# martellab-sri/ModalTune

Hardware: AMD Instinct MI355X
Metric: slides/sec (train step) at 10k patches x 1536-d (higher is better)
Workload: dtype f16; 1 GPU; Prov-GigaPath ModalAdapter train step, 10000 patches x 1536-d, 6 pathways -> 64 gene tokens + 1 task token, 3 task passes, fp16 operands / fp32 accumulate, 1 slide per GPU per step, task passes as two concurrent groups (B = 2 | 1 on two HIP streams), train mode: Dropout(0.25) on the embedded input and both backbone branches, DropPath(0..0.1) per layer and on the Extractor FFN (Philox masks regener; patches=10000, parallelism=dp1, dropout=True

## Files before the change

include/modaltune_hip.h:

```cpp
#ifndef MODALTUNE_HIP_H
#define MODALTUNE_HIP_H

#include <stdint.h>

#ifdef __cplusplus
extern "C" {
#endif

typedef void* mt_stream_t;
typedef uint16_t mt_half;

typedef enum {
  MT_OK = 0,
  MT_ERR_BAD_ARG = -1,
  MT_ERR_LAUNCH = -2,
  MT_ERR_UNSUPPORTED = -3
} MtStatus;

typedef struct { int seg_rows, seg_stride, row0; } MtRowMap;

int mt_version(void);
const char* mt_status_string(int status);
const char* mt_build_id(void);

// ... 8 lines not shown
  const unsigned* rng;
  unsigned site;
  float p;
  unsigned path_site;
  float path_p;
  int rows_per_pass;
} MtDropout;
int mt_rng_advance(unsigned* rng, mt_stream_t stream);
int mt_dropout_f32(const float* x, long ldx, const MtRowMap* xmap, float* y, int M, int D, const MtDropout* drop,
                   mt_stream_t stream);
int mt_droppath_rows_f32(float* x, int M, int D, const MtDropout* drop, mt_stream_t stream);

typedef struct {
  const float* bias;
  const float* resid;
  long ldr;
  MtRowMap rmap;
  const float* colscale;
  const float* pos_table;
  const int* pos_row;
  const int* pos_col;
  MtDropout drop;
} MtGemmEpilogue;

int mt_gemm_nt_f16(const mt_half* A, long lda, const MtRowMap* amap, const mt_half* W, int M, int N, int K,
                   int epilogue, const MtGemmEpilogue* epi, void* C, long ldc, const MtRowMap* cmap, int out_dtype,
                   mt_stream_t stream);

int mt_gemm_tn_f16(const mt_half* A, long lda, const MtRowMap* amap, const mt_half* B, long ldb, const MtRowMap* bmap,
                   int M, int N1, int N2, float* C, long ldc, float* colsum, mt_stream_t stream);

int mt_colsum_f16(const mt_half* A, long lda, const MtRowMap* amap, int M, int N, float* out, mt_stream_t stream);

enum { MT_ACT_NONE = 0, MT_ACT_RELU = 1, MT_ACT_GELU = 2, MT_ACT_ELU = 3 };
int mt_sgemm_small(const float* A, long as0, long as1, long a_bs, const float* B, long bs0, long bs1, long b_bs,
                   const float* bias, int bias_on_m, float* C, long cs0, long cs1, long c_bs, int M, int N, int K,
                   int batch, int act, int accumulate, float* rowsum, mt_stream_t stream);

#define MT_SGEMM_MAX 3
typedef struct {
  const float* A; long as0, as1, a_bs;
  const float* B; long bs0, bs1, b_bs;
  const float* bias; int bias_on_m;
  float* C; long cs0, cs1, c_bs;
  int M, N, K, batch, act, accumulate;
  float* rowsum;
  float* pre_out;
  const float* resid;
  MtDropout c_drop;
  const float* a_aux; int a_act;
  MtDropout a_drop;
  float resid_scale; int a_ld;
} MtSgemm;
int mt_sgemm_multi(const MtSgemm* probs, int n, mt_stream_t stream);

int mt_layernorm_fwd(const void* x, long ldx, const MtRowMap* xmap, int in_dtype, int gelu_in, const float* w,
                     const float* b, const float* add_rows, int add_period, void* y, long ldy, const MtRowMap* ymap,
                     int out_dtype, float* stats, int M, int D, mt_stream_t stream);
int mt_add_layernorm_fwd(const float* x, const mt_half* branch, const MtDropout* drop, const float* w, const float* b,
                         float* h, mt_half* y, float* stats, int M, int D, mt_stream_t stream);

int mt_layernorm_fwd_eps(const void* x, long ldx, const MtRowMap* xmap, int in_dtype, int gelu_in, const float* w,
                         const float* b, const float* add_rows, int add_period, void* y, long ldy, const MtRowMap* ymap,
                         int out_dtype, float* stats, int M, int D, float eps, mt_stream_t stream);
int mt_add_layernorm_fwd_eps(const float* x, const mt_half* branch, const MtDropout* drop, const float* w, const float* b,
                             float* h, mt_half* y, float* stats, int M, int D, float eps, mt_stream_t stream);

int mt_layernorm_bwd(const void* dy, long lddy, const MtRowMap* dymap, int dy_dtype, const void* x, long ldx,
                     const MtRowMap* xmap, int in_dtype, int gelu_in, const float* w, const float* stats, void* dx,
                     long lddx, const MtRowMap* dxmap, int dx_dtype, int accumulate, float* dw, float* db,
                     mt_half* dx_f16, const MtDropout* dx_f16_drop, int M, int D, mt_stream_t stream);

#define MT_MAX_BRANCHES 8
#define MT_QK_SCALE_LOG2 0.20823509396846288f
typedef struct {
  int nbranch;
  int N;
  int B;
  int seg[MT_MAX_BRANCHES];
  int ratio[MT_MAX_BRANCHES];
  int nseg[MT_MAX_BRANCHES];
  int n[MT_MAX_BRANCHES];
  int qlimit[MT_MAX_BRANCHES];
} MtDilatedPlan;

int mt_dilated_attn_fwd(const mt_half* qkv, const MtDilatedPlan* plan, mt_half* o_br, float* lse_br,
                        mt_stream_t stream);

int mt_dilated_mix_ln_fwd(const mt_half* o_br, const float* lse_br, const MtDilatedPlan* plan, const float* ln_w,
                          const float* ln_b, mt_half* y, float* stats, float* lse_tot, mt_stream_t stream);

int mt_dilated_mix_ln_bwd(const mt_half* dy, const mt_half* o_br, const float* lse_br, const float* lse_tot,
                          const MtDilatedPlan* plan, const float* ln_w, const float* stats, mt_half* dmixed,
                          float* delta_br, mt_stream_t stream);

long mt_dilated_attn_bwd_workspace_bytes(const MtDilatedPlan* plan);
enum { MT_ATTN_BWD_KV = 1, MT_ATTN_BWD_Q = 2, MT_ATTN_BWD_COMBINE = 4, MT_ATTN_BWD_ALL = 7 };
int mt_dilated_attn_bwd(const mt_half* qkv, const mt_half* dmixed, const float* lse_tot, const float* delta_br,
                        const MtDilatedPlan* plan, void* workspace, mt_half* dqkv, int phases, mt_stream_t stream);

#define MT_DENSE_QK_SCALE_LOG2 0.18033688011112042f
typedef struct {
  int N;
  int B;
  int H;
  const mt_half* dist;
  const float* nslope;
} MtDensePlan;
long mt_alibi_dist_halves(int N);
int mt_alibi_dist(const int* cells, int N, mt_half* table, mt_stream_t stream);
int mt_dense_attn_fwd(const mt_half* qkv, const MtDensePlan* plan, mt_half* o, float* lse, mt_stream_t stream);
enum { MT_DENSE_BWD_DELTA = 1, MT_DENSE_BWD_KV = 2, MT_DENSE_BWD_Q = 4, MT_DENSE_BWD_ALL = 7 };
int mt_dense_attn_bwd(const mt_half* qkv, const mt_half* o, const mt_half* d_o, const float* lse, const MtDensePlan* plan,
                      float* delta, mt_half* dqkv, int phases, mt_stream_t stream);

int mt_gelu_f16_fwd(const mt_half* x, mt_half* y, long n, mt_stream_t stream);
int mt_gelu_f16_bwd(const mt_half* x, const mt_half* dy, mt_half* dx, long n, mt_stream_t stream);

long mt_pool_attn_workspace_floats(int B, int N, int heads, int nq);
int mt_pool_attn_fwd(const float* q, const mt_half* kv, int B, int N, int E, int heads, int nq, float* out, float* scores,
                     float* lse, float* workspace, mt_stream_t stream);
int mt_pool_attn_bwd(const float* q, const mt_half* kv, const float* scores, const float* lse, const float* out,
                     const float* dout, int B, int N, int E, int heads, int nq, mt_half* dkv, mt_stream_t stream);

typedef struct {
  const float *ln1_w, *ln1_b, *inner_ln_w, *inner_ln_b, *ln2_w, *ln2_b, *ffn_ln_w, *ffn_ln_b;
  const float *b_qkv, *b_out, *b_fc1, *b_fc2;
  const mt_half *w_qkv, *w_out, *w_fc1, *w_fc2;
  const mt_half *wt_qkv, *wt_out, *wt_fc1, *wt_fc2;
} MtLongNetLayerWeights;
typedef struct {
  float *hin, *hmid; mt_half *qkv, *o_br; float *lse_br, *lse_tot; mt_half* a1; float *st1, *stin, *st2, *stf;
  mt_half *u16, *br16, *t16;
  float* dh; mt_half *dy16, *dh16, *dt16, *da1, *dmixed, *dqkv16; float* delta; void* attn_ws;
} MtLongNetLayerBuffers;
int mt_longnet_layer_fwd(const MtLongNetLayerWeights* w, const MtLongNetLayerBuffers* b, const MtDilatedPlan* plan, int M, int D, int F,
                         const float* pend_x, const mt_half* pend_branch, const MtDropout* pend_drop, int defer, float* out,
                         const MtDropout* drop_attn, const MtDropout* drop_ffn, mt_stream_t stream);
int mt_longnet_layer_bwd(const MtLongNetLayerWeights* w, const MtLongNetLayerBuffers* b, const MtDilatedPlan* plan, int M, int D, int F,
                         int dh16_valid, int feeds_lower, const MtDropout* drop_attn, const MtDropout* drop_ffn,
                         const MtDropout* drop_lower_ffn, mt_stream_t stream);
typedef struct {
  const float *n1_w, *n1_b, *n2_w, *n2_b; float n1_eps, n2_eps;
  const float *b_qkv, *b_proj, *b_fc1, *b_fc2;
  const mt_half *w_qkv, *w_proj, *w_fc1, *w_fc2;
  const mt_half *wt_qkv, *wt_proj, *wt_fc1, *wt_fc2;
} MtVitBlockWeights;
typedef struct {
  float *hin, *hmid; mt_half *qkv, *o16; float* lse; mt_half* a1; float *st1, *st2;
  mt_half *u16, *br16, *t16;
  float* dh; mt_half *dy16, *dh16, *dt16, *da1, *dqkv16; float* delta;
} MtVitBlockBuffers;
int mt_vit_block_fwd(const MtVitBlockWeights* w, const MtVitBlockBuffers* b, const MtDensePlan* plan, int M, int D, int F,
                     const float* pend_x, const mt_half* pend_branch, int defer, float* out, mt_stream_t stream);
int mt_vit_block_bwd(const MtVitBlockWeights* w, const MtVitBlockBuffers* b, const MtDensePlan* plan, int M, int D, int F,
                     int dh16_valid, int feeds_lower, mt_stream_t stream);

int mt_inject_attn_fwd(const mt_half* q, int M, int rows_per_pass, const float* k, const float* v, int T,
                       mt_half* a, float* lse, mt_stream_t stream);
int mt_inject_attn_bwd(const mt_half* q, const mt_half* a, const float* lse, const mt_half* da, int M,
                       int rows_per_pass, const float* k, const float* v, int T, mt_half* dq, float* dk, float* dv,
                       mt_stream_t stream);

int mt_extract_attn_fwd(const float* q, const mt_half* kv, int B, int T, int L, float* out, float* lse,
                        float* part_acc, float* part_ml, int nsplit, mt_stream_t stream);
int mt_extract_attn_bwd(const float* q, const mt_half* kv, const float* out, const float* lse, const float* dout,
                        int B, int T, int L, float* dq, mt_half* dkv, mt_stream_t stream);

int mt_gene_snn_fwd(const float* params, const long* offs, const int* sizes, const long* goff, const float* genes, int G,
                    int latent, int passes, float* a1, float* a2, float* z, const MtDropout* alpha_drop, mt_stream_t stream);
int mt_gene_snn_bwd(const float* params, float* grads, const long* offs, const int* sizes, const long* goff,
                    const float* genes, int G, int latent, int passes, const float* a1, const float* a2, const float* dz,
                    const MtDropout* alpha_drop, mt_stream_t stream);

int mt_token_mha_fwd(const float* q, const float* k, const float* v, int B, int T, int E, int heads, float* out,
                     float* probs, mt_stream_t stream);
int mt_token_mha_bwd(const float* q, const float* k, const float* v, const float* probs, const float* dout, int B,
                     int T, int E, int heads, float* dq, float* dk, float* dv, mt_stream_t stream);

int mt_cast_f32_to_f16(const float* x, mt_half* y, long n, const MtDropout* drop, int D, mt_stream_t stream);
int mt_cast_f16_to_f32(const mt_half* x, float* y, long n, mt_stream_t stream);
int mt_pack_weight_f16(const float* src, int R, int C, mt_half* dst, int transpose, mt_stream_t stream);
int mt_pack_weights_f16(const long long* items, int n_items, mt_stream_t stream);
int mt_act_fwd(const float* x, float* y, long n, int act, mt_stream_t stream);
int mt_act_bwd(const float* x, const float* dy, float* dx, long n, int act, mt_stream_t stream);
int mt_axpy(const float* a, const float* b, float alpha, float* y, long n, mt_stream_t stream);
int mt_axpy_bcast(const float* a, const float* b, float alpha, float* y, long n, long period, mt_stream_t stream);
int mt_fold_rows(const float* x, int reps, long period, float* out, mt_stream_t stream);
int mt_copy_rows_f32(const float* src, long lds, const MtRowMap* smap, float* dst, long ldd, const MtRowMap* dmap,
                     int M, int D, int accumulate, mt_stream_t stream);
int mt_inject_resid_bwd(const float* dy, long lddy, const MtRowMap* dymap, const float* x, long ldx,
                        const MtRowMap* xmap, const mt_half* proj, const float* gamma, float* dx, long lddx,
                        const MtRowMap* dxmap, int dx_accumulate, mt_half* dproj, float* dgamma, int M, int D,
                        mt_stream_t stream);

int mt_l2norm_rows(const float* x, float* y, int R, int O, mt_stream_t stream);
int mt_distill_loss(const float* logits, const float* target, int R, int O, float loss_scale,
                    const float* scale_dev , float* loss,
                    float* dlogits, mt_stream_t stream);

int mt_adamw_step(float* p, const float* g, float* m, float* v, long n, double lr, double beta1, double beta2,
                  double eps, double weight_decay , int step_count, const int* step_dev , float grad_mult ,
                  const float* scale, int* found_inf, const float* lr_dev , mt_stream_t stream);
int mt_scaler_update(float* scale, int* growth_tracker, int* found_inf, int* step_dev ,
                     float growth, float backoff, int interval, mt_stream_t stream);
int mt_check_finite(const float* g, long n, int* found_inf, mt_stream_t stream);

int mt_mfma_probe(float* sink, int workgroups, int iters, mt_stream_t stream);

int mt_absmax_scale(const float* x, long n, float target, float* s, mt_stream_t stream);
int mt_axpy_dev(const float* a, const float* b, const float* alpha, float* y, long n, mt_stream_t stream);
int mt_coords_to_grid(const float* coords, int L, float tile, int ngrids, int* prow, int* pcol, int* err,
                      mt_stream_t stream);
int mt_titan_grid(const float* coords, int L, float patch, int* cells, int* dims, int* err, mt_stream_t stream);
int mt_titan_cell_sums(const float* feat, long ldf, const int* cells, int L, int C, int* first, int* next, float* sums, int* nz,
                       mt_stream_t stream);
int mt_titan_token_order(const int* cells, const int* first, const int* nz, int L, int* pos, int* cells_tok, int* count,
                         mt_stream_t stream);
int mt_titan_gather_tokens(const float* sums, const int* pos, int L, int C, mt_half* x16, mt_stream_t stream);
int mt_scatter_rows_f32(const float* src, const int* src_idx, const int* idx, float* dst, int M, int D, int accumulate,
                        mt_stream_t stream);
int mt_row_absmax_f32(const float* x, float* out, int M, int D, mt_stream_t stream);

#ifdef __cplusplus
// ... 4 lines not shown
```

modaltune_amd/_lib.py:

```python
from __future__ import annotations

import ctypes as C
import os

_HERE = os.path.dirname(os.path.abspath(__file__))
LIB_PATH = os.environ.get("MODALTUNE_HIP_LIB", os.path.join(_HERE, "_C", "libmodaltune_hip.so"))

P, I, L, F, D = C.c_void_p, C.c_int, C.c_long, C.c_float, C.c_double


class MtRowMap(C.Structure):
    _fields_ = [("seg_rows", I), ("seg_stride", I), ("row0", I)]


class MtDropout(C.Structure):
    _fields_ = [("rng", P), ("site", C.c_uint), ("p", F), ("path_site", C.c_uint), ("path_p", F), ("rows_per_pass", I)]


class MtGemmEpilogue(C.Structure):
    _fields_ = [("bias", P), ("resid", P), ("ldr", L), ("rmap", MtRowMap), ("colscale", P),
                ("pos_table", P), ("pos_row", P), ("pos_col", P), ("drop", MtDropout)]


MT_SGEMM_MAX = 3


class MtSgemm(C.Structure):
    _fields_ = [("A", P), ("as0", L), ("as1", L), ("a_bs", L), ("B", P), ("bs0", L), ("bs1", L), ("b_bs", L),
                ("bias", P), ("bias_on_m", I), ("C", P), ("cs0", L), ("cs1", L), ("c_bs", L),
                ("M", I), ("N", I), ("K", I), ("batch", I), ("act", I), ("accumulate", I),
                ("rowsum", P), ("pre_out", P), ("resid", P), ("c_drop", MtDropout),
                ("a_aux", P), ("a_act", I), ("a_drop", MtDropout), ("resid_scale", F), ("a_ld", I)]


MT_MAX_BRANCHES = 8


class MtDilatedPlan(C.Structure):
    _fields_ = [("nbranch", I), ("N", I), ("B", I), ("seg", I * MT_MAX_BRANCHES), ("ratio", I * MT_MAX_BRANCHES),
                ("nseg", I * MT_MAX_BRANCHES), ("n", I * MT_MAX_BRANCHES), ("qlimit", I * MT_MAX_BRANCHES)]


class MtDensePlan(C.Structure):
    _fields_ = [("N", I), ("B", I), ("H", I), ("dist", P), ("nslope", P)]


class MtLongNetLayerWeights(C.Structure):
    _fields_ = [(n, P) for n in ("ln1_w", "ln1_b", "inner_ln_w", "inner_ln_b", "ln2_w", "ln2_b", "ffn_ln_w", "ffn_ln_b", "b_qkv", "b_out",
                                 "b_fc1", "b_fc2", "w_qkv", "w_out", "w_fc1", "w_fc2", "wt_qkv", "wt_out", "wt_fc1", "wt_fc2")]


class MtLongNetLayerBuffers(C.Structure):
    _fields_ = [(n, P) for n in ("hin", "hmid", "qkv", "o_br", "lse_br", "lse_tot", "a1", "st1", "stin", "st2", "stf", "u16", "br16", "t16",
                                 "dh", "dy16", "dh16", "dt16", "da1", "dmixed", "dqkv16", "delta", "attn_ws")]


class MtVitBlockWeights(C.Structure):
    _fields_ = [(n, P) for n in ("n1_w", "n1_b", "n2_w", "n2_b")] + [("n1_eps", F), ("n2_eps", F)] + \
               [(n, P) for n in ("b_qkv", "b_proj", "b_fc1", "b_fc2", "w_qkv", "w_proj", "w_fc1", "w_fc2", "wt_qkv", "wt_proj", "wt_fc1", "wt_fc2")]


class MtVitBlockBuffers(C.Structure):
    _fields_ = [(n, P) for n in ("hin", "hmid", "qkv", "o16", "lse", "a1", "st1", "st2", "u16", "br16", "t16", "dh", "dy16", "dh16", "dt16",
                                 "da1", "dqkv16", "delta")]


RM = C.POINTER(MtRowMap)
DR = C.POINTER(MtDropout)
EP = C.POINTER(MtGemmEpilogue)
PL = C.POINTER(MtDilatedPlan)
DP = C.POINTER(MtDensePlan)

SIGNATURES = {
    "mt_version": [],
    "mt_status_string": [I],
    "mt_build_id": [],
    "mt_gemm_nt_f16": [P, L, RM, P, I, I, I, I, EP, P, L, RM, I, P],
    "mt_gemm_tn_f16": [P, L, RM, P, L, RM, I, I, I, P, L, P, P],
    "mt_colsum_f16": [P, L, RM, I, I, P, P],
    "mt_sgemm_small": [P, L, L, L, P, L, L, L, P, I, P, L, L, L, I, I, I, I, I, I, P, P],
    "mt_sgemm_multi": [C.POINTER(MtSgemm), I, P],
    "mt_layernorm_fwd": [P, L, RM, I, I, P, P, P, I, P, L, RM, I, P, I, I, P],
    "mt_add_layernorm_fwd": [P, P, DR, P, P, P, P, P, I, I, P],
    "mt_layernorm_fwd_eps": [P, L, RM, I, I, P, P, P, I, P, L, RM, I, P, I, I, F, P],
    "mt_add_layernorm_fwd_eps": [P, P, DR, P, P, P, P, P, I, I, F, P],
    "mt_layernorm_bwd": [P, L, RM, I, P, L, RM, I, I, P, P, P, L, RM, I, I, P, P, P, DR, I, I, P],
    "mt_dilated_attn_fwd": [P, PL, P, P, P],
    "mt_dilated_mix_ln_fwd": [P, P, PL, P, P, P, P, P, P],
    "mt_dilated_mix_ln_bwd": [P, P, P, P, PL, P, P, P, P, P],
    "mt_dilated_attn_bwd_workspace_bytes": [PL],
    "mt_dilated_attn_bwd": [P, P, P, P, PL, P, P, I, P],
    "mt_gene_snn_fwd": [P, P, P, P, P, I, I, I, P, P, P, DR, P],
    "mt_gene_snn_bwd": [P, P, P, P, P, P, I, I, I, P, P, P, DR, P],
    "mt_inject_attn_fwd": [P, I, I, P, P, I, P, P, P],
    "mt_inject_attn_bwd": [P, P, P, P, I, I, P, P, I, P, P, P, P],
    "mt_extract_attn_fwd": [P, P, I, I, I, P, P, P, P, I, P],
    "mt_extract_attn_bwd": [P, P, P, P, P, I, I, I, P, P, P],
    "mt_token_mha_fwd": [P, P, P, I, I, I, I, P, P, P],
    "mt_token_mha_bwd": [P, P, P, P, P, I, I, I, I, P, P, P, P],
    "mt_cast_f32_to_f16": [P, P, L, DR, I, P],
    "mt_rng_advance": [P, P],
    "mt_dropout_f32": [P, L, RM, P, I, I, DR, P],
    "mt_droppath_rows_f32": [P, I, I, DR, P],
    "mt_cast_f16_to_f32": [P, P, L, P],
    "mt_pack_weight_f16": [P, I, I, P, I, P],
    "mt_pack_weights_f16": [P, I, P],
    "mt_act_fwd": [P, P, L, I, P],
    "mt_act_bwd": [P, P, P, L, I, P],
    "mt_axpy": [P, P, F, P, L, P],
    "mt_axpy_bcast": [P, P, F, P, L, L, P],
    "mt_fold_rows": [P, I, L, P, P],
    "mt_copy_rows_f32": [P, L, RM, P, L, RM, I, I, I, P],
    "mt_inject_resid_bwd": [P, L, RM, P, L, RM, P, P, P, L, RM, I, P, P, I, I, P],
    "mt_l2norm_rows": [P, P, I, I, P],
    "mt_distill_loss": [P, P, I, I, F, P, P, P, P],
    "mt_adamw_step": [P, P, P, P, L, D, D, D, D, D, I, P, F, P, P, P, P],
    "mt_scaler_update": [P, P, P, P, F, F, I, P],
    "mt_check_finite": [P, L, P, P],
    "mt_absmax_scale": [P, L, F, P, P],
    "mt_axpy_dev": [P, P, P, P, L, P],
    "mt_coords_to_grid": [P, I, F, I, P, P, P, P],
    "mt_mfma_probe": [P, I, I, P],
    "mt_longnet_layer_fwd": [P, P, PL, I, I, I, P, P, DR, I, P, DR, DR, P],
    "mt_longnet_layer_bwd": [P, P, PL, I, I, I, I, I, DR, DR, DR, P],
    "mt_vit_block_fwd": [P, P, DP, I, I, I, P, P, I, P, P],
    "mt_vit_block_bwd": [P, P, DP, I, I, I, I, I, P],
    "mt_alibi_dist": [P, I, P, P],
    "mt_alibi_dist_halves": [I],
    "mt_dense_attn_fwd": [P, DP, P, P, P],
    "mt_dense_attn_bwd": [P, P, P, P, DP, P, P, I, P],
    "mt_gelu_f16_fwd": [P, P, L, P],
    "mt_gelu_f16_bwd": [P, P, P, L, P],
    "mt_pool_attn_workspace_floats": [I, I, I, I],
    "mt_pool_attn_fwd": [P, P, I, I, I, I, I, P, P, P, P, P],
    "mt_pool_attn_bwd": [P, P, P, P, P, P, I, I, I, I, I, P, P],
    "mt_titan_grid": [P, I, F, P, P, P, P],
    "mt_titan_cell_sums": [P, L, P, I, I, P, P, P, P, P],
    "mt_titan_token_order": [P, P, P, I, P, P, P, P],
    "mt_titan_gather_tokens": [P, P, I, I, P, P],
    "mt_scatter_rows_f32": [P, P, P, P, I, I, I, P],
    "mt_row_absmax_f32": [P, P, I, I, P],
}
_RESTYPE = {"mt_status_string": C.c_char_p, "mt_build_id": C.c_char_p, "mt_dilated_attn_bwd_workspace_bytes": C.c_long, "mt_pool_attn_workspace_floats": C.c_long,
             "mt_alibi_dist_halves": C.c_long}

_lib = None


def load():
    global _lib
    if _lib is not None:
        return _lib
    import torch
    if not os.path.exists(LIB_PATH):
        raise RuntimeError(
            f"modaltune_amd: {LIB_PATH} is missing -- run `python __graft_entry__.py` (hipcc, gfx950) first; "
            "there is no CPU/PyTorch fallback for the hot path")
    lib = C.CDLL(LIB_PATH)
    for name, args in SIGNATURES.items():
        fn = getattr(lib, name)
        fn.argtypes = args
        fn.restype = _RESTYPE.get(name, I)
    _lib = lib
    return lib


def build_info() -> dict:
    from ._build_id import tree_build_id
    bid = load().mt_build_id().decode()
    try:
        ok = bid == tree_build_id()
    except Exception:
        ok = None
    return {"build_id": bid, "build_id_matches_tree": ok, "lib": os.path.relpath(LIB_PATH, os.path.dirname(_HERE))}


def check(status: int, what: str = ""):
    if status != 0:
        msg = load().mt_status_string(status).decode()
        raise RuntimeError(f"modaltune_hip {what} failed: {msg} ({status})")


def rowmap(seg_rows=0, seg_stride=0, row0=0):
    return MtRowMap(seg_rows, seg_stride, row0)
```

modaltune_amd/csrc/attn.hip:

```cpp
#include "attn_common.h"

namespace {

__global__ __launch_bounds__(256) void dilated_attn_fwd_kernel(const h16* __restrict__ qkv, Plan p, h16* __restrict__ o_br,
                                                               float* __restrict__ lse_br) {
  __shared__ __attribute__((aligned(16))) h16 smem[4 * IMG_HALVES];
  h16* const Ks = smem;
  h16* const Vs = smem + 2 * IMG_HALVES;
  const int tid = threadIdx.x, lane = tid & 63, wave = tid >> 6;
  const int hh = lane >> 5, l31 = lane & 31;
  const WorkItem w = decode(p, blockIdx.x);
  const Seq sq = make_seq(p, w);
  const long M = (long)p.B * p.N;
  const int nv = __builtin_amdgcn_readfirstlane(sq.nvalid());
  const int nvq = min(nv, p.qlimit[w.br]);
  if (w.qt * 128 >= nvq) return;

  {
    const int buf = tid >> 7, row = (tid >> 1) & 63, which = 6 + (tid & 1);
    const h16x8 one = {(h16)1.f, 0, 0, 0, (h16)1.f, 0, 0, 0}, zero = {0, 0, 0, 0, 0, 0, 0, 0};
    *reinterpret_cast<h16x8*>(&Vs[buf * IMG_HALVES + img_off(row, which)]) = which == 6 ? one : zero;
  }

  const int iq = w.qt * 128 + wave * 32 + l31;
  const bool qvalid = sq.valid(iq) && iq < nvq;
  const long qrow = sq.row_clamped(iq);
  h16x8 qf[3];
#pragma unroll
  for (int ks = 0; ks < 3; ++ks)
    qf[ks] = sel8(qvalid, ldg8(hm_ptr(qkv, M, w.h, qrow) + ks * 16 + hh * 8));

  const int ntile = (sq.n + 63) / 64;
  const int nproc = (nv + 63) >> 6;
  const int row_bytes = sq.dr * HD * 2;
  const long valid_bytes = (long)(nv - 1) * row_bytes + HD * 2;
  const long tile_bytes = 64L * row_bytes;
  const h16* const kseq = hm_ptr(qkv, M, H + w.h, sq.row(0));
  const h16* const vseq = hm_ptr(qkv, M, 2 * H + w.h, sq.row(0));
  const DmaLane dl(tid, row_bytes);
  auto dma = [&](int t) {
    dma_tile(Ks + (t & 1) * IMG_HALVES, tile_rsrc(kseq, t * tile_bytes, valid_bytes), dl);
    dma_tile(Vs + (t & 1) * IMG_HALVES, tile_rsrc(vseq, t * tile_bytes, valid_bytes), dl);
  };
  const int grp = lane >> 4, li = lane & 15, tq = li >> 2, tp = li & 3;
  int krd[3];
#pragma unroll
  for (int ks = 0; ks < 3; ++ks) krd[ks] = img_off(l31, 2 * ks + hh);
  const int vc = 2 * (grp & 1) + (tp >> 1), vo = 4 * (tp & 1);
  const int va0 = img_off(4 * hh + tq, vc) + vo, va1 = img_off(4 * hh + tq, vc + 4) + vo;
  const int vb0 = img_off(4 * hh + tq + 8, vc) + vo, vb1 = img_off(4 * hh + tq + 8, vc + 4) + vo;

  auto qk = [&](const h16* Kb, f32x16 (&s)[2], const f32x16& init) {
#pragma unroll
    for (int sub = 0; sub < 2; ++sub) {
#pragma unroll
      for (int ks = 0; ks < 3; ++ks) {
        const h16x8 kf = *reinterpret_cast<const h16x8*>(&Kb[sub * 32 * IMG_ROW + krd[ks]]);
        s[sub] = __builtin_amdgcn_mfma_f32_32x32x16_f16(kf, qf[ks], ks == 0 ? init : s[sub], 0, 0, 0);
      }
    }
  };

  f32x16 o0, o1;
#pragma unroll
  for (int i = 0; i < 16; ++i) { o0[i] = 0.f; o1[i] = 0.f; }

  dma(0);
  dma_wait_all();
  __syncthreads();
  float m2;
  f32x16 minit;
  {
    f32x16 s0[2], zero;
#pragma unroll
    for (int i = 0; i < 16; ++i) zero[i] = 0.f;
    qk(Ks, s0, zero);
    float mx = NEG_BIG;
#pragma unroll
    for (int sub = 0; sub < 2; ++sub)
#pragma unroll
      for (int i = 0; i < 16; ++i) {
        const int kidx = sub * 32 + (i & 3) + 8 * (i >> 2) + 4 * hh;
        mx = fmaxf(mx, kidx < sq.n ? s0[sub][i] : NEG_BIG);
      }
    m2 = max_halves(mx);
#pragma unroll
    for (int i = 0; i < 16; ++i) minit[i] = -m2;
  }

  auto tile = [&](int t, auto tail_tag) {
    constexpr bool TAIL = decltype(tail_tag)::value;
    const int kb = t * 64;
    const h16* Kb = Ks + (t & 1) * IMG_HALVES;
    const h16* Vb = Vs + (t & 1) * IMG_HALVES;
    if (t + 1 < nproc) dma(t + 1);
    f32x16 s_cur[2];
    qk(Kb, s_cur, minit);
    float mx = NEG_BIG;
#pragma unroll
// ... 41 lines not shown
  if (tail_last) tile(nproc - 1, std::true_type{});
  const int rest = sq.n - nproc * 64;
  if (rest > 0) {
    if (__any(-m2 > RESCALE_LOG2)) {
      const float up = fmaxf(-m2, 0.f);
      const float alpha = __builtin_amdgcn_exp2f(-up);
#pragma unroll
      for (int i = 0; i < 16; ++i) { o0[i] *= alpha; o1[i] *= alpha; }
      m2 += up;
    }
    o1[8] += (float)rest * __builtin_amdgcn_exp2f(-m2);
  }

  if (qvalid) {
    const float l = o1[8];
    const float inv = 1.0f / l;
    h16* orow = o_br + ((long)w.br * M + qrow) * DM + w.h * HD;
#pragma unroll
    for (int gq = 0; gq < 4; ++gq) {
      h16x4 v = {(h16)(o0[4 * gq] * inv), (h16)(o0[4 * gq + 1] * inv), (h16)(o0[4 * gq + 2] * inv), (h16)(o0[4 * gq + 3] * inv)};
      *reinterpret_cast<h16x4*>(orow + 8 * gq + 4 * hh) = v;
    }
#pragma unroll
    for (int gq = 0; gq < 2; ++gq) {
      h16x4 v = {(h16)(o1[4 * gq] * inv), (h16)(o1[4 * gq + 1] * inv), (h16)(o1[4 * gq + 2] * inv), (h16)(o1[4 * gq + 3] * inv)};
      *reinterpret_cast<h16x4*>(orow + 32 + 8 * gq + 4 * hh) = v;
    }
    if (hh == 0) lse_br[((long)w.br * M + qrow) * H + w.h] = (m2 + __log2f(l)) * LN2;
  }
}

struct MixGeom {
  int grp[MT_MAX_BRANCHES];
  MT_DEVINL MixGeom(const Plan& p, int h) {
#pragma unroll
    for (int b = 0; b < MT_MAX_BRANCHES; ++b) grp[b] = b < p.nbranch ? h / (H / p.ratio[b]) : -1;
  }
};
MT_DEVINL void seg_split(const Plan& p, int b, int pos, int& j, int& loc) {
  const int sg = p.seg[b];
  if (sg >= p.N) { j = 0; loc = pos; return; }
  j = (int)((float)pos * p.inv_seg[b]);
  loc = pos - j * sg;
  if (loc < 0) { loc += sg; --j; }
  if (loc >= sg) { loc -= sg; ++j; }
}
MT_DEVINL int residue(const Plan& p, int b, int pos) {
  int j, loc;
  seg_split(p, b, pos, j, loc);
  const int dr = p.ratio[b];
  return (dr & (dr - 1)) == 0 ? (loc & (dr - 1)) : loc % dr;
}
MT_DEVINL int dense_branch(const Plan& p) {
  int d = 0;
#pragma unroll
  for (int b = 0; b < MT_MAX_BRANCHES; ++b) if (b < p.nbranch && p.ratio[b] == 1) d = b;
  return d;
}
constexpr int MIX_CPL = 24;
struct H24 { h16x8 a, b, c; };
MT_DEVINL H24 ld24(const h16* p) {
  return H24{*reinterpret_cast<const h16x8*>(p), *reinterpret_cast<const h16x8*>(p + 8), *reinterpret_cast<const h16x8*>(p + 16)};
}
MT_DEVINL float h24(const H24& v, int e) { return (float)(e < 8 ? v.a[e & 7] : e < 16 ? v.b[e & 7] : v.c[e & 7]); }
MT_DEVINL float half_sum(float v) {
#pragma unroll
  for (int o = 16; o > 0; o >>= 1) v += __shfl_xor(v, o, 64);
  return v;
}

template <int NB>
__global__ __launch_bounds__(256) void mix_ln_fwd_kernel(const h16* __restrict__ o_br, const float* __restrict__ lse_br, Plan p,
                                                         const float* __restrict__ ln_w, const float* __restrict__ ln_b,
                                                         h16* __restrict__ y, float* __restrict__ stats, float* __restrict__ lse_tot) {
  const int lane = threadIdx.x & 63, wave = threadIdx.x >> 6, sub = lane >> 5, l5 = lane & 31;
  const long M = (long)p.B * p.N;
  const int h = l5 >> 1, c0 = l5 * MIX_CPL;
  const MixGeom geo(p, h);
  const int db = dense_branch(p);
  float w[MIX_CPL], bb[MIX_CPL];
#pragma unroll
  for (int e = 0; e < MIX_CPL; ++e) { w[e] = ln_w[c0 + e]; bb[e] = ln_b[c0 + e]; }
  for (long m2 = ((long)blockIdx.x * 4 + wave) * 2; m2 < M; m2 += (long)gridDim.x * 8) {
    const bool live = m2 + sub < M;
    const long m = live ? m2 + sub : M - 1;
    const int pos = (int)(m % p.N);
    bool cov[NB];
    float lse[NB];
    H24 ob[NB];
#pragma unroll
    for (int b = 0; b < NB; ++b) {
      cov[b] = b < p.nbranch && geo.grp[b] == residue(p, b, pos);
      const int sb = cov[b] ? b : db;
      lse[b] = lse_br[((long)sb * M + m) * H + h];
      ob[b] = ld24(o_br + ((long)sb * M + m) * DM + c0);
    }
    float mx = NEG_BIG;
#pragma unroll
    for (int b = 0; b < NB; ++b) { lse[b] = cov[b] ? lse[b] : NEG_BIG; mx = fmaxf(mx, lse[b]); }
    float den = 0.f;
#pragma unroll
    for (int b = 0; b < NB; ++b) den += cov[b] ? __expf(lse[b] - mx) : 0.f;
    const float tot = mx + __logf(den);
    float v[MIX_CPL];
#pragma unroll
    for (int e = 0; e < MIX_CPL; ++e) v[e] = 0.f;
#pragma unroll
    for (int b = 0; b < NB; ++b) {
      const float wgt = cov[b] ? __expf(lse[b] - tot) : 0.f;
#pragma unroll
      for (int e = 0; e < MIX_CPL; ++e) v[e] = fmaf(wgt, cov[b] ? h24(ob[b], e) : 0.f, v[e]);
    }
    float s = 0.f;
#pragma unroll
    for (int e = 0; e < MIX_CPL; ++e) s += v[e];
    const float mean = half_sum(s) * (1.0f / DM);
    float q = 0.f;
#pragma unroll
    for (int e = 0; e < MIX_CPL; ++e) { const float d = v[e] - mean; q += d * d; }
    const float rstd = rsqrtf(half_sum(q) * (1.0f / DM) + 1e-5f);
    if (live) {
      h16* dst = y + m * DM + c0;
#pragma unroll
      for (int k = 0; k < 3; ++k) {
        h16x8 o;
#pragma unroll
        for (int e = 0; e < 8; ++e) o[e] = (h16)((v[8 * k + e] - mean) * rstd * w[8 * k + e] + bb[8 * k + e]);
        *reinterpret_cast<h16x8*>(dst + 8 * k) = o;
      }
      if (l5 == 0) { stats[2 * m] = mean; stats[2 * m + 1] = rstd; }
      if ((l5 & 1) == 0) lse_tot[m * H + h] = tot;
    }
  }
}

template <int NB>
__global__ __launch_bounds__(256) void mix_ln_bwd_kernel(const h16* __restrict__ dy, const h16* __restrict__ o_br,
                                                         const float* __restrict__ lse_br, const float* __restrict__ lse_tot, Plan p,
                                                         const float* __restrict__ ln_w, const float* __restrict__ stats,
                                                         h16* __restrict__ dmixed, float* __restrict__ delta_br) {
  const int lane = threadIdx.x & 63, wave = threadIdx.x >> 6, sub = lane >> 5, l5 = lane & 31;
  const long M = (long)p.B * p.N;
  const int h = l5 >> 1, c0 = l5 * MIX_CPL;
  const MixGeom geo(p, h);
  const int db = dense_branch(p);
  float w[MIX_CPL];
#pragma unroll
  for (int e = 0; e < MIX_CPL; ++e) w[e] = ln_w[c0 + e];
  for (long m2 = ((long)blockIdx.x * 4 + wave) * 2; m2 < M; m2 += (long)gridDim.x * 8) {
    const bool live = m2 + sub < M;
    const long m = live ? m2 + sub : M - 1;
    const int pos = (int)(m % p.N);
    const float tot = lse_tot[m * H + h];
    const float mean = stats[2 * m], rstd = stats[2 * m + 1];
    const H24 dyv = ld24(dy + m * DM + c0);
    bool cov[NB];
    float lse[NB];
    H24 ob[NB];
#pragma unroll
    for (int b = 0; b < NB; ++b) {
      cov[b] = b < p.nbranch && geo.grp[b] == residue(p, b, pos);
      const int sb = cov[b] ? b : db;
      lse[b] = lse_br[((long)sb * M + m) * H + h];
      ob[b] = ld24(o_br + ((long)sb * M + m) * DM + c0);
    }
    float v[MIX_CPL];
#pragma unroll
    for (int e = 0; e < MIX_CPL; ++e) v[e] = 0.f;
#pragma unroll
    for (int b = 0; b < NB; ++b) {
      const float wgt = cov[b] ? __expf(lse[b] - tot) : 0.f;
#pragma unroll
      for (int e = 0; e < MIX_CPL; ++e) v[e] = fmaf(wgt, cov[b] ? h24(ob[b], e) : 0.f, v[e]);
    }
    float g[MIX_CPL], xh[MIX_CPL];
    float s1 = 0.f, s2 = 0.f;
#pragma unroll
    for (int i = 0; i < MIX_CPL; ++i) {
      xh[i] = (v[i] - mean) * rstd;
      g[i] = h24(dyv, i) * w[i];
      s1 += g[i]; s2 = fmaf(g[i], xh[i], s2);
    }
    const float c1 = half_sum(s1) * (1.0f / DM), c2 = half_sum(s2) * (1.0f / DM);
    float dm[MIX_CPL];
    h16* dst = dmixed + ((long)h * M + m) * HD + (c0 - h * HD);
#pragma unroll
    for (int k = 0; k < 3; ++k) {
      h16x8 o;
#pragma unroll
      for (int e = 0; e < 8; ++e) {
        const int i = 8 * k + e;
        o[e] = (h16)(rstd * (g[i] - c1 - xh[i] * c2));
        dm[i] = (float)o[e];
      }
      if (live) *reinterpret_cast<h16x8*>(dst + 8 * k) = o;
    }
#pragma unroll
    for (int b = 0; b < NB; ++b) {
      float d = 0.f;
#pragma unroll
      for (int e = 0; e < MIX_CPL; ++e) d = fmaf(dm[e], h24(ob[b], e), d);
      d += __shfl_xor(d, 1, 64);
      if (live && (l5 & 1) == 0 && cov[b]) delta_br[((long)b * M + m) * H + h] = d;
    }
  }
}


}

extern "C" int mt_dilated_attn_fwd(const mt_half* qkv, const MtDilatedPlan* plan, mt_half* o_br, float* lse_br,
                                   mt_stream_t stream) {
  if (!qkv || !o_br || !lse_br || !plan_ok(plan)) return MT_ERR_BAD_ARG;
  const Plan p = make_plan(plan, 128);
  const int nblk = p.blk_off[p.nbranch];
  hipLaunchKernelGGL(dilated_attn_fwd_kernel, dim3(nblk), dim3(256), 0, (hipStream_t)stream, (const h16*)qkv, p,
                     (h16*)o_br, lse_br);
  MT_CHECK_LAUNCH();
  return MT_OK;
}

extern "C" int mt_dilated_mix_ln_fwd(const mt_half* o_br, const float* lse_br, const MtDilatedPlan* plan,
                                     const float* ln_w, const float* ln_b, mt_half* y, float* stats, float* lse_tot,
                                     mt_stream_t stream) {
  if (!o_br || !lse_br || !ln_w || !ln_b || !y || !stats || !lse_tot || !plan_ok(plan)) return MT_ERR_BAD_ARG;
  const Plan p = make_plan(plan, 128);
  const long M = (long)p.B * p.N;
  const dim3 grid((int)min((M + 7) / 8, 8192L));
  if (p.nbranch <= 5)
    hipLaunchKernelGGL(mix_ln_fwd_kernel<5>, grid, dim3(256), 0, (hipStream_t)stream, (const h16*)o_br, lse_br, p, ln_w, ln_b,
                       (h16*)y, stats, lse_tot);
  else
    hipLaunchKernelGGL(mix_ln_fwd_kernel<MT_MAX_BRANCHES>, grid, dim3(256), 0, (hipStream_t)stream, (const h16*)o_br, lse_br, p,
                       ln_w, ln_b, (h16*)y, stats, lse_tot);
// ... 39 lines not shown
```

modaltune_amd/csrc/attn_bwd_kv.hip:

```cpp
#include "attn_common.h"

namespace {

__global__ __launch_bounds__(256, 3) void dilated_attn_bwd_kv_kernel(const h16* __restrict__ qkv, const h16* __restrict__ dmixed,
                                                                  const float* __restrict__ lse_tot, const float* __restrict__ delta_br,
                                                                  Plan p, h16* __restrict__ ws) {
  __shared__ __attribute__((aligned(16))) h16 smem[4 * IMG_HALVES];
  __shared__ __attribute__((aligned(16))) float L2s[2][64];
  __shared__ __attribute__((aligned(16))) float Dls[2][64];
  h16* const Qx = smem;
  h16* const Dx = smem + 2 * IMG_HALVES;
  const int tid = threadIdx.x, lane = tid & 63, wave = tid >> 6;
  const int hh = lane >> 5, l31 = lane & 31;
  const WorkItem w = decode(p, blockIdx.x);
  const Seq sq = make_seq(p, w);
  const long M = (long)p.B * p.N;
  const h16x8 zero8 = {0, 0, 0, 0, 0, 0, 0, 0};
  const int nv = __builtin_amdgcn_readfirstlane(sq.nvalid());
  if (w.qt * 128 >= nv) return;

  {
    const int img = tid >> 6, row = tid & 63;
    *reinterpret_cast<h16x8*>(&smem[img * IMG_HALVES + img_off(row, 6)]) = zero8;
    *reinterpret_cast<h16x8*>(&smem[img * IMG_HALVES + img_off(row, 7)]) = zero8;
  }

  const int ik = w.qt * 128 + wave * 32 + l31;
  const bool kvalid = sq.valid(ik);
  const long krow = sq.row_clamped(ik);
  h16x8 kf[3], vf[3];
#pragma unroll
  for (int ks = 0; ks < 3; ++ks) {
    kf[ks] = sel8(kvalid, ldg8(hm_ptr(qkv, M, H + w.h, krow) + ks * 16 + hh * 8));
    vf[ks] = sel8(kvalid, ldg8(hm_ptr(qkv, M, 2 * H + w.h, krow) + ks * 16 + hh * 8));
  }

  const int nvq = min(nv, p.qlimit[w.br]);
  const int ntile = (nvq + 63) >> 6;
  const int row_bytes = sq.dr * HD * 2;
  const long valid_bytes = (long)(nvq - 1) * row_bytes + HD * 2;
  const long tile_bytes = 64L * row_bytes;
  const h16* const qseq = hm_ptr(qkv, M, w.h, sq.row(0));
  const h16* const dseq = hm_ptr(dmixed, M, w.h, sq.row(0));
  const DmaLane dl(tid, row_bytes);
  const float* const lbase = lse_tot + sq.row(0) * H + w.h;
  const float* const dbase = delta_br + ((long)w.br * M + sq.row(0)) * H + w.h;
  float rl2 = 0.f, rdl = 0.f;
  auto issue = [&](int t) {
    dma_tile(Qx + (t & 1) * IMG_HALVES, tile_rsrc(qseq, t * tile_bytes, valid_bytes), dl);
    dma_tile(Dx + (t & 1) * IMG_HALVES, tile_rsrc(dseq, t * tile_bytes, valid_bytes), dl);
    if (tid < 64) {
      const long off = (long)min(t * 64 + lane, nvq - 1) * sq.dr * H;
      rl2 = lbase[off];
      rdl = dbase[off];
    }
  };
  auto publish = [&](int t) {
    if (tid < 64) {
      const bool ok = t * 64 + lane < nvq;
      L2s[t & 1][tid] = ok ? fmaf(-rl2, LOG2E, LOG2_LN2) : 0.f;
      Dls[t & 1][tid] = ok ? -rdl : 0.f;
    }
  };

  f32x16 dk0, dk1, dv0, dv1;
#pragma unroll
  for (int i = 0; i < 16; ++i) { dk0[i] = 0.f; dk1[i] = 0.f; dv0[i] = 0.f; dv1[i] = 0.f; }
  const int grp = lane >> 4, li = lane & 15, tq = li >> 2, tp = li & 3;
  int rrd[3];
#pragma unroll
  for (int ks = 0; ks < 3; ++ks) rrd[ks] = img_off(l31, 2 * ks + hh);
  const int trc = 2 * (grp & 1) + (tp >> 1), tro = 4 * (tp & 1);
  const int tr_a0 = img_off(4 * hh + tq, trc) + tro, tr_a1 = img_off(4 * hh + tq, trc + 4) + tro;
  const int tr_b0 = img_off(4 * hh + tq + 8, trc) + tro, tr_b1 = img_off(4 * hh + tq + 8, trc + 4) + tro;

  issue(0);
  publish(0);
  dma_wait_all();
  __syncthreads();
  for (int t = 0; t < ntile; ++t) {
    const h16* Qb = Qx + (t & 1) * IMG_HALVES;
    const h16* Db = Dx + (t & 1) * IMG_HALVES;
    const float* L2b = L2s[t & 1];
    const float* Dlb = Dls[t & 1];
    if (t + 1 < ntile) issue(t + 1);
#pragma unroll
    for (int sub = 0; sub < 2; ++sub) {
      f32x16 s, dp;
#pragma unroll
      for (int g4 = 0; g4 < 4; ++g4) {
        const f32x4 a = *reinterpret_cast<const f32x4*>(&L2b[sub * 32 + 8 * g4 + 4 * hh]);
        const f32x4 b = *reinterpret_cast<const f32x4*>(&Dlb[sub * 32 + 8 * g4 + 4 * hh]);
#pragma unroll
        for (int e = 0; e < 4; ++e) { s[4 * g4 + e] = a[e]; dp[4 * g4 + e] = b[e]; }
      }
      __builtin_amdgcn_sched_barrier(0);
      h16x8 qa[3], da[3];
#pragma unroll
      for (int ks = 0; ks < 3; ++ks) {
        qa[ks] = *reinterpret_cast<const h16x8*>(&Qb[sub * 32 * IMG_ROW + rrd[ks]]);
        da[ks] = *reinterpret_cast<const h16x8*>(&Db[sub * 32 * IMG_ROW + rrd[ks]]);
      }
// ... 66 lines not shown
```

modaltune_amd/csrc/attn_bwd_q.hip:

```cpp
#include "attn_common.h"

namespace {

__global__ __launch_bounds__(256) void dilated_attn_bwd_q_kernel(const h16* __restrict__ qkv, const h16* __restrict__ dmixed,
                                                                 const float* __restrict__ lse_tot, const float* __restrict__ delta_br,
                                                                 Plan p, h16* __restrict__ ws) {
  __shared__ __attribute__((aligned(16))) h16 smem[4 * IMG_HALVES];
  h16* const Ks = smem;
  h16* const Vs = smem + 2 * IMG_HALVES;
  const int tid = threadIdx.x, lane = tid & 63, wave = tid >> 6;
  const int hh = lane >> 5, l31 = lane & 31;
  const WorkItem w = decode(p, blockIdx.x);
  const Seq sq = make_seq(p, w);
  const long M = (long)p.B * p.N;
  const h16x8 zero8 = {0, 0, 0, 0, 0, 0, 0, 0};
  const int nv = __builtin_amdgcn_readfirstlane(sq.nvalid());
  const int nvq = min(nv, p.qlimit[w.br]);
  if (w.qt * 128 >= nvq) return;

  {
    const int buf = tid >> 7, row = (tid >> 1) & 63, which = 6 + (tid & 1);
    *reinterpret_cast<h16x8*>(&Ks[buf * IMG_HALVES + img_off(row, which)]) = zero8;
  }

  const int iq = w.qt * 128 + wave * 32 + l31;
  const bool qvalid = sq.valid(iq) && iq < nvq;
  const long qrow = sq.row_clamped(iq);
  h16x8 qf[3], dof[3];
#pragma unroll
  for (int ks = 0; ks < 3; ++ks) {
    qf[ks] = sel8(qvalid, ldg8(hm_ptr(qkv, M, w.h, qrow) + ks * 16 + hh * 8));
    dof[ks] = sel8(qvalid, ldg8(hm_ptr(dmixed, M, w.h, qrow) + ks * 16 + hh * 8));
  }
  const float L2raw = lse_tot[qrow * H + w.h], dlraw = delta_br[((long)w.br * M + qrow) * H + w.h];
  const float nl2 = qvalid ? fmaf(-L2raw, LOG2E, LOG2_LN2) : -1.0e30f;
  const float ndl = qvalid ? -dlraw : 0.f;
  f32x16 nl2i, ndli;
#pragma unroll
  for (int i = 0; i < 16; ++i) { nl2i[i] = nl2; ndli[i] = ndl; }

  const int ntile = (nv + 63) >> 6;
  const int row_bytes = sq.dr * HD * 2;
  const long valid_bytes = (long)(nv - 1) * row_bytes + HD * 2;
  const long tile_bytes = 64L * row_bytes;
  const h16* const kseq = hm_ptr(qkv, M, H + w.h, sq.row(0));
  const h16* const vseq = hm_ptr(qkv, M, 2 * H + w.h, sq.row(0));
  const DmaLane dl(tid, row_bytes);
  auto dma = [&](int t) {
    dma_tile_pair(Ks + (t & 1) * IMG_HALVES, tile_rsrc(kseq, t * tile_bytes, valid_bytes), Vs + (t & 1) * IMG_HALVES,
                  tile_rsrc(vseq, t * tile_bytes, valid_bytes), dl, __builtin_amdgcn_readfirstlane(tid >> 6));
  };
  const int grp = lane >> 4, li = lane & 15, tq = li >> 2, tp = li & 3;
  int rrd[3];
#pragma unroll
  for (int ks = 0; ks < 3; ++ks) rrd[ks] = img_off(l31, 2 * ks + hh);
  const int kc = 2 * (grp & 1) + (tp >> 1), ko = 4 * (tp & 1);
  const int ka0 = img_off(4 * hh + tq, kc) + ko, ka1 = img_off(4 * hh + tq, kc + 4) + ko;
  const int kb0 = img_off(4 * hh + tq + 8, kc) + ko, kb1 = img_off(4 * hh + tq + 8, kc + 4) + ko;

  f32x16 dq0, dq1;
#pragma unroll
  for (int i = 0; i < 16; ++i) { dq0[i] = 0.f; dq1[i] = 0.f; }
  dma(0);
  dma_wait_all();
  __syncthreads();
  auto tile = [&](int t, auto tail_tag) {
    constexpr bool TAIL = decltype(tail_tag)::value;
    const int kb = t * 64;
    const h16* Kb = Ks + (t & 1) * IMG_HALVES;
    const h16* Vb = Vs + (t & 1) * IMG_HALVES;
    if (t + 1 < ntile) dma(t + 1);
#pragma unroll
    for (int sub = 0; sub < 2; ++sub) {
      f32x16 s, dp;
      h16x8 ka[3], va[3];
#pragma unroll
      for (int ks = 0; ks < 3; ++ks) {
        ka[ks] = *reinterpret_cast<const h16x8*>(&Kb[sub * 32 * IMG_ROW + rrd[ks]]);
        va[ks] = *reinterpret_cast<const h16x8*>(&Vb[sub * 32 * IMG_ROW + rrd[ks]]);
      }
#pragma unroll
      for (int ks = 0; ks < 3; ++ks) {
        s = __builtin_amdgcn_mfma_f32_32x32x16_f16(ka[ks], qf[ks], ks == 0 ? nl2i : s, 0, 0, 0);
        dp = __builtin_amdgcn_mfma_f32_32x32x16_f16(va[ks], dof[ks], ks == 0 ? ndli : dp, 0, 0, 0);
      }
      __builtin_amdgcn_sched_group_barrier(0x100, 3, 0);
#pragma unroll
      for (int i = 0; i < 3; ++i) {
        __builtin_amdgcn_sched_group_barrier(0x8, 1, 0);
        __builtin_amdgcn_sched_group_barrier(0x100, 1, 0);
      }
      __builtin_amdgcn_sched_group_barrier(0x8, 3, 0);
      h16x8 dsf[2];
#pragma unroll
      for (int i = 0; i < 16; i += 2) {
        f32x2 pt = pk_exp2((f32x2){s[i], s[i + 1]});
        if (TAIL) {
          const int kidx = kb + sub * 32 + (i & 3) + 8 * (i >> 2) + 4 * hh;
          if (kidx >= sq.n) pt[0] = 0.f;
          if (kidx + 1 >= sq.n) pt[1] = 0.f;
        }
// ... 42 lines not shown
```

modaltune_amd/csrc/attn_combine.hip:

```cpp
#include "attn_common.h"

namespace {

__global__ __launch_bounds__(192) void dilated_attn_bwd_combine_kernel(const h16* __restrict__ ws, Plan p, h16* __restrict__ dqkv) {
  const long M = (long)p.B * p.N;
  const int t = threadIdx.x;
  const int col = t * 12, which = col / DM, h = (col % DM) / HD, d0 = col % HD;
  for (long m = blockIdx.x; m < M; m += gridDim.x) {
    const int pos = (int)(m % p.N);
    float acc[12];
#pragma unroll
    for (int e = 0; e < 12; ++e) acc[e] = 0.f;
#pragma unroll
    for (int br = 0; br < MT_MAX_BRANCHES; ++br) {
      if (br < p.nbranch) {
        const int dr = p.ratio[br], sg = p.seg[br], hb = H / dr;
        const int j = pos / sg, loc = pos - j * sg;
        if (loc % dr == h / hb) {
          const h16* src = ws + p.ws_off[br] + ((m * 3 + which) * hb + (h % hb)) * HD + d0;
          const h16x4 a0 = *reinterpret_cast<const h16x4*>(src), a1 = *reinterpret_cast<const h16x4*>(src + 4),
                      a2 = *reinterpret_cast<const h16x4*>(src + 8);
#pragma unroll
          for (int e = 0; e < 4; ++e) { acc[e] += (float)a0[e]; acc[4 + e] += (float)a1[e]; acc[8 + e] += (float)a2[e]; }
        }
      }
    }
    h16* dst = dqkv + m * QKV_LD + col;
#pragma unroll
    for (int k = 0; k < 3; ++k) {
      const h16x4 o = {(h16)acc[4 * k], (h16)acc[4 * k + 1], (h16)acc[4 * k + 2], (h16)acc[4 * k + 3]};
      *reinterpret_cast<h16x4*>(dst + 4 * k) = o;
    }
  }
}

}

void mt_attn::launch_bwd_combine(const void* ws, const MtDilatedPlan* plan, mt_half* dqkv, hipStream_t s) {
  const Plan p = make_plan(plan, 128);
  const long M = (long)p.B * p.N;
  hipLaunchKernelGGL(dilated_attn_bwd_combine_kernel, dim3((int)min(M, 16384L)), dim3(192), 0, s, (const h16*)ws, p, (h16*)dqkv);
}
```

modaltune_amd/csrc/attn_common.h:

```cpp
#pragma once
#include <stdlib.h>
#include <type_traits>

#include "common.h"

namespace {

constexpr int H = 16, HD = 48, DM = 768, QKV_LD = 2304;
constexpr int KSTR = 56;
constexpr int VSTR = 96;
constexpr float LOG2E = 1.4426950408889634f, LN2 = 0.6931471805599453f;
constexpr float NEG_BIG = -1.0e30f;
constexpr float RESCALE_LOG2 = 8.0f;
constexpr float QK_SCALE_LOG2 = 0.14433756729740643f * 1.4426950408889634f;
constexpr float LOG2_LN2 = -0.52876637294489768f;
constexpr float INV_LN2 = 1.4426950408889634f;

struct Plan {
  int nbranch, N, B;
  int seg[MT_MAX_BRANCHES], ratio[MT_MAX_BRANCHES], nseg[MT_MAX_BRANCHES], n[MT_MAX_BRANCHES];
  int order[MT_MAX_BRANCHES], qtiles[MT_MAX_BRANCHES], blk_off[MT_MAX_BRANCHES + 1];
  long ws_off[MT_MAX_BRANCHES + 1];
  float inv_seg[MT_MAX_BRANCHES];
  int qlimit[MT_MAX_BRANCHES];
};

Plan make_plan(const MtDilatedPlan* p, int qtile) {
  Plan d;
  d.nbranch = p->nbranch; d.N = p->N; d.B = p->B;
  for (int i = 0; i < p->nbranch; ++i) {
    d.seg[i] = p->seg[i]; d.ratio[i] = p->ratio[i]; d.nseg[i] = p->nseg[i]; d.n[i] = p->n[i];
    d.order[i] = i;
    d.qtiles[i] = cdiv(p->n[i], qtile);
    d.inv_seg[i] = 1.0f / (float)p->seg[i];
    d.qlimit[i] = p->qlimit[i] > 0 ? p->qlimit[i] : p->n[i];
  }
  for (int i = 0; i < d.nbranch; ++i)
    for (int j = i + 1; j < d.nbranch; ++j)
      if (d.n[d.order[j]] > d.n[d.order[i]]) { int t = d.order[i]; d.order[i] = d.order[j]; d.order[j] = t; }
  d.blk_off[0] = 0;
  for (int i = 0; i < d.nbranch; ++i) {
    const int b = d.order[i];
    d.blk_off[i + 1] = d.blk_off[i] + d.B * d.nseg[b] * H * d.qtiles[b];
  }
  d.ws_off[0] = 0;
  for (int b = 0; b < d.nbranch; ++b) d.ws_off[b + 1] = d.ws_off[b] + (long)d.B * d.N * 3 * (H / d.ratio[b]) * HD;
  return d;
}

bool plan_ok(const MtDilatedPlan* p) {
  if (!p || p->nbranch < 1 || p->nbranch > MT_MAX_BRANCHES || p->N < 1 || p->B < 1) return false;
  for (int i = 0; i < p->nbranch; ++i) {
    const int r = p->ratio[i], s = p->seg[i];
    if (r < 1 || r > H || (H % r) != 0 || s < 1 || s > p->N) return false;
    if (p->nseg[i] != cdiv(p->N, s) || p->n[i] != cdiv(s, r)) return false;
    if (p->qlimit[i] < 0 || p->qlimit[i] > p->n[i]) return false;
  }
  return true;
}

struct WorkItem { int br, b, j, h, qt; };

MT_DEVINL WorkItem decode(const Plan& p, int bid) {
  const int x = bid & 7, j = bid >> 3;
  int oi = 0;
#pragma unroll
  for (int i = 1; i < MT_MAX_BRANCHES; ++i)
    if (i < p.nbranch && j >= (p.blk_off[i] >> 3)) oi = i;
  WorkItem w;
  w.br = p.order[oi];
  int local = j - (p.blk_off[oi] >> 3);
  w.qt = local % p.qtiles[w.br];
  const int gid = (local / p.qtiles[w.br]) * 8 + x;
  w.h = gid % H;
  const int r = gid / H;
  w.j = r % p.nseg[w.br];
  w.b = r / p.nseg[w.br];
  w.br = __builtin_amdgcn_readfirstlane(w.br); w.qt = __builtin_amdgcn_readfirstlane(w.qt);
  w.h = __builtin_amdgcn_readfirstlane(w.h); w.j = __builtin_amdgcn_readfirstlane(w.j);
  w.b = __builtin_amdgcn_readfirstlane(w.b);
  return w;
}

MT_DEVINL WorkItem decode_branch(const Plan& p, int br, int bid) {
  const int x = bid & 7, j = bid >> 3;
  WorkItem w;
  w.br = br;
  w.qt = j % p.qtiles[br];
  const int gid = (j / p.qtiles[br]) * 8 + x;
  w.h = gid % H;
  const int r = gid / H;
  w.j = r % p.nseg[br];
  w.b = r / p.nseg[br];
  return w;
}

MT_DEVINL int swz(int row, int chunk) { return row * VSTR + ((chunk ^ ((row >> 2) & 3)) << 3); }

MT_DEVINL h16x4 lds_tr4(const h16* p) {
  s16x4 r = __builtin_amdgcn_ds_read_tr16_b64_v4i16(
      (__attribute__((address_space(3))) s16x4*)(__attribute__((address_space(3))) void*)p);
  return __builtin_bit_cast(h16x4, r);
}
MT_DEVINL h16x8 cat8(h16x4 lo, h16x4 hi) { return (h16x8){lo[0], lo[1], lo[2], lo[3], hi[0], hi[1], hi[2], hi[3]}; }

struct Seq {
  int n, s, dr, r, seg_base, N;
  long row_base;
  MT_DEVINL bool valid(int i) const {
    const int loc = r + i * dr;
    return i < n && loc < s && seg_base + loc < N;
  }
  MT_DEVINL long row(int i) const { return row_base + seg_base + r + (long)i * dr; }
  MT_DEVINL long row_clamped(int i) const { return min(row(i), row_base + (long)N - 1); }
  MT_DEVINL int nvalid() const {
    const int lim = min(s, N - seg_base) - r;
    return lim <= 0 ? 0 : min(n, (lim + dr - 1) / dr);
  }
};
// ... 115 lines not shown
```

modaltune_amd/csrc/common.h:

```cpp
#pragma once
#include <hip/hip_runtime.h>
#include <stdint.h>

#include "../../include/modaltune_hip.h"

typedef _Float16 h16;
typedef _Float16 h16x2 __attribute__((ext_vector_type(2)));
typedef _Float16 h16x4 __attribute__((ext_vector_type(4)));
typedef _Float16 h16x8 __attribute__((ext_vector_type(8)));
typedef short s16x4 __attribute__((ext_vector_type(4)));
typedef float f32x2 __attribute__((ext_vector_type(2)));
typedef float f32x4 __attribute__((ext_vector_type(4)));
typedef float f32x16 __attribute__((ext_vector_type(16)));

#define MT_WAVE 64
#define MT_DEVINL __device__ __forceinline__
MT_DEVINL float lds_f32(const float* p) { return *reinterpret_cast<const volatile float*>(p); }
MT_DEVINL f32x4 lds_f32x4_by_dword(const float* p) {
  const volatile float* q = reinterpret_cast<const volatile float*>(p);
  return (f32x4){q[0], q[1], q[2], q[3]};
}
#define MT_LDS_DRAIN_V1(a) asm volatile("s_waitcnt lgkmcnt(0)" : "+v"(a) : : "memory")
#define MT_LDS_DRAIN_V2(a, b) asm volatile("s_waitcnt lgkmcnt(0)" : "+v"(a), "+v"(b) : : "memory")
#define MT_LDS_DRAIN_V3(a, b, c) asm volatile("s_waitcnt lgkmcnt(0)" : "+v"(a), "+v"(b), "+v"(c) : : "memory")
#define MT_LDS_DRAIN_V4(a) asm volatile("s_waitcnt lgkmcnt(0)" : "+v"((a)[0]), "+v"((a)[1]), "+v"((a)[2]), "+v"((a)[3]) : : "memory")
#define MT_LDS_DRAIN_V8(a)                                                                                                       \
  asm volatile("s_waitcnt lgkmcnt(0)"                                                                                            \
               : "+v"((a)[0]), "+v"((a)[1]), "+v"((a)[2]), "+v"((a)[3]), "+v"((a)[4]), "+v"((a)[5]), "+v"((a)[6]), "+v"((a)[7]) \
               :                                                                                                                  \
               : "memory")

struct RowMap {
  int seg_rows, seg_stride, row0;
  MT_DEVINL long map(int m) const {
    if (seg_rows <= 0) return m;
    int s = m / seg_rows;
    return (long)s * seg_stride + row0 + (m - s * seg_rows);
  }
};
static inline RowMap make_rowmap(const MtRowMap* r) {
  RowMap m;
  if (r) { m.seg_rows = r->seg_rows; m.seg_stride = r->seg_stride; m.row0 = r->row0; }
  else { m.seg_rows = 0; m.seg_stride = 0; m.row0 = 0; }
  return m;
}

MT_DEVINL float wave_sum(float v) {
#pragma unroll
  for (int o = 32; o > 0; o >>= 1) v += __shfl_xor(v, o, 64);
  return v;
}
MT_DEVINL float wave_max(float v) {
#pragma unroll
  for (int o = 32; o > 0; o >>= 1) v = fmaxf(v, __shfl_xor(v, o, 64));
  return v;
}

MT_DEVINL float erf_rsqrt2(float x, float& e) {
  const float z = fabsf(x) * 0.70710678118654752440f;
  const float t = __builtin_amdgcn_rcpf(fmaf(0.3275911f, z, 1.0f));
  float poly = fmaf(t, 1.061405429f, -1.453152027f);
  poly = fmaf(poly, t, 1.421413741f);
  poly = fmaf(poly, t, -0.284496736f);
  poly = fmaf(poly, t, 0.254829592f);
  poly *= t;
  e = __builtin_amdgcn_exp2f(-z * z * 1.4426950408889634f);
  const float r = fmaf(-poly, e, 1.0f);
  return copysignf(r, x);
}
MT_DEVINL float gelu_erf(float x) { float e; return 0.5f * x * (1.0f + erf_rsqrt2(x, e)); }
MT_DEVINL float gelu_erf_grad(float x) {
  float e;
  const float er = erf_rsqrt2(x, e);
  return fmaf(x * 0.39894228040143267794f, e, 0.5f * (1.0f + er));
}

struct DropArgs {
  const uint32_t* rng; uint32_t site; float p; uint32_t path_site; float path_p; int rows_per_pass;
  __host__ __device__ __forceinline__ bool active() const { return rng != nullptr && (p > 0.f || path_p > 0.f); }
};
static inline DropArgs make_drop(const MtDropout* d) {
  DropArgs a;
  if (d && d->rng && (d->p > 0.f || d->path_p > 0.f)) {
    a.rng = d->rng; a.site = d->site; a.p = d->p; a.path_site = d->path_site; a.path_p = d->path_p;
    a.rows_per_pass = d->rows_per_pass > 0 ? d->rows_per_pass : 1;
  } else {
    a.rng = nullptr; a.site = 0; a.p = 0.f; a.path_site = 0; a.path_p = 0.f; a.rows_per_pass = 1;
  }
  return a;
}
MT_DEVINL void philox4x32_7(uint32_t c0, uint32_t c1, uint32_t c2, uint32_t c3, uint32_t k0, uint32_t k1, uint32_t (&out)[4]) {
#pragma unroll
  for (int r = 0; r < 7; ++r) {
    const uint32_t hi0 = __umulhi(0xD2511F53u, c0), lo0 = 0xD2511F53u * c0;
    const uint32_t hi1 = __umulhi(0xCD9E8D57u, c2), lo1 = 0xCD9E8D57u * c2;
    c0 = hi1 ^ c1 ^ k0; c1 = lo1; c2 = hi0 ^ c3 ^ k1; c3 = lo0;
    k0 += 0x9E3779B9u; k1 += 0xBB67AE85u;
  }
  out[0] = c0; out[1] = c1; out[2] = c2; out[3] = c3;
}
MT_DEVINL uint32_t drop_threshold(float p) { return (uint32_t)fminf(p * 4294967296.0f, 4294967040.0f); }
MT_DEVINL float drop_path_factor(const DropArgs& d, int pass) {
  if (!(d.path_p > 0.f)) return 1.f;
  uint32_t r[4];
  philox4x32_7((uint32_t)pass, 0x9E3779B9u, d.path_site, d.rng[2], d.rng[0], d.rng[1], r);
  return r[0] >= drop_threshold(d.path_p) ? 1.f / (1.f - d.path_p) : 0.f;
}
MT_DEVINL f32x4 drop_elem4(const DropArgs& d, uint64_t idx4, float pf) {
  f32x4 s = {pf, pf, pf, pf};
  if (d.p > 0.f) {
    uint32_t r[4];
    philox4x32_7((uint32_t)idx4, (uint32_t)(idx4 >> 32), d.site, d.rng[2], d.rng[0], d.rng[1], r);
    const uint32_t thr = drop_threshold(d.p);
    const float keep = pf / (1.f - d.p);
#pragma unroll
    for (int e = 0; e < 4; ++e) s[e] = r[e] >= thr ? keep : 0.f;
  }
  return s;
}
MT_DEVINL f32x4 drop_scale4(const DropArgs& d, uint64_t idx4, int m) {
  return drop_elem4(d, idx4, drop_path_factor(d, m / d.rows_per_pass));
}

MT_DEVINL bool drop_keep1(const DropArgs& d, uint32_t site, uint64_t idx) {
  uint32_t r[4];
  philox4x32_7((uint32_t)(idx >> 2), (uint32_t)(idx >> 34), site, d.rng[2], d.rng[0], d.rng[1], r);
  return r[idx & 3] >= drop_threshold(d.p);
}

MT_DEVINL h16x8 ldg8(const h16* p) { return *reinterpret_cast<const h16x8*>(p); }
MT_DEVINL void stg8(h16* p, h16x8 v) { *reinterpret_cast<h16x8*>(p) = v; }

#define MT_CHECK_LAUNCH()                                   \
  do {                                                      \
    hipError_t e__ = hipGetLastError();                     \
    if (e__ != hipSuccess) return MT_ERR_LAUNCH;            \
  } while (0)

static inline int cdiv(long a, long b) { return (int)((a + b - 1) / b); }
```

modaltune_amd/csrc/gemm.hip:

```cpp
#include <stdlib.h>
#include <string.h>

#include "common.h"

int mt_gemm_ps_launch(const void* A, long lda, const void* W, int M, int N, int K, int epilogue, const float* bias, void* C, long ldc, hipStream_t s);

namespace {

constexpr int BK = 64;

#ifdef MT_GEMM_STAMP
MT_DEVINL unsigned long long stamp_now() { unsigned long long t; asm volatile("s_memtime %0\n\ts_waitcnt lgkmcnt(0)" : "=s"(t) :: "memory"); return t; }
#define MT_STAMP(var) const unsigned long long var = stamp_now()
#define MT_STAMP_ADD(g, slot, a, b) do { if (threadIdx.x == 0) atomicAdd(reinterpret_cast<unsigned long long*>(const_cast<float*>((g).pos_table)) + (slot), (b) - (a)); } while (0)
#else
#define MT_STAMP(var)
#define MT_STAMP_ADD(g, slot, a, b)
#endif

struct GemmNtArgs {
  const h16* A; long lda; RowMap amap;
  const h16* W;
  int M, N, K;
  int m_begin, m_end;
  const float* bias;
  const float* resid; long ldr; RowMap rmap;
  const float* colscale;
  const float* pos_table; const int* pos_row; const int* pos_col;
  void* C; long ldc; RowMap cmap;
  DropArgs drop;
};

constexpr int erows_for(int bm, int cs, int lds_bytes) {
  int e = bm;
  while (e * cs * 4 > lds_bytes) e /= 2;
  return e;
}

typedef uint32_t u32x2_t __attribute__((ext_vector_type(2)));
constexpr int erows_h16(int bm, int csh, int lds_bytes) {
  int e = bm;
  while (e * csh * 2 > lds_bytes) e /= 2;
  return e;
}
template <int BM, int BN, int WM, int WN, int EPI, int LDS_BYTES>
MT_DEVINL void gemm_epilogue_h16(const GemmNtArgs& g, f32x4 (&acc)[BM / WM / 16][BN / WN / 16], h16* smem, int m0, int n0) {
  constexpr int NT = WM * WN * 64;
  constexpr int TM = BM / WM, TN = BN / WN, MI = TM / 16, NI = TN / 16;
  constexpr int CSH = BN + 4;
  constexpr int EROWS = erows_h16(BM, CSH, LDS_BYTES);
  const int tid = threadIdx.x, lane = tid & 63, wave = tid >> 6;
  const int wm = wave / WN, wn = wave % WN;
  const int fr = lane & 15, fq = lane >> 4;
  h16* C = reinterpret_cast<h16*>(g.C);
  f32x4 b4[NI];
#pragma unroll
  for (int j = 0; j < NI; ++j) {
    const int n = n0 + wn * TN + j * 16 + fq * 4;
    b4[j] = (g.bias && n < g.N) ? *reinterpret_cast<const f32x4*>(g.bias + n) : (f32x4){0.f, 0.f, 0.f, 0.f};
  }
  constexpr int CPR = BN / 8;
  constexpr int RPP = NT / CPR;
  const int cc = (tid % CPR) * 8, r0 = tid / CPR;
  const int n = n0 + cc;
#pragma unroll
  for (int pass = 0; pass < BM / EROWS; ++pass) {
    const int rbase = pass * EROWS;
    MT_STAMP(e0);
    if (pass > 0) __syncthreads();
#pragma unroll
    for (int i = 0; i < MI; ++i) {
      const int row = wm * TM + i * 16 + fr - rbase;
      if (row >= 0 && row < EROWS) {
#pragma unroll
        for (int j = 0; j < NI; ++j) {
          const f32x4 v = acc[i][j] + b4[j];
          *reinterpret_cast<h16x4*>(&smem[row * CSH + wn * TN + j * 16 + fq * 4]) = (h16x4){(h16)v[0], (h16)v[1], (h16)v[2], (h16)v[3]};
        }
      }
    }
    __syncthreads();
    MT_STAMP(e1);
#pragma unroll 4
    for (int rr = r0; rr < EROWS; rr += RPP) {
      const int m = m0 + rbase + rr;
      if (m >= g.m_end || n >= g.N) continue;
      const h16x4 lo = *reinterpret_cast<const h16x4*>(&smem[rr * CSH + cc]), hi = *reinterpret_cast<const h16x4*>(&smem[rr * CSH + cc + 4]);
      h16* dst = EPI == MT_EPI_QKV_HM ? C + ((long)(n / 48) * g.M + m) * 48 + (n % 48)
// ... 619 lines not shown
      for (int j = 0; j < 4; ++j) a[j] = sg_xform4<AK>(g, a[j], x[j], arow + (long)(k0 + 16 * j + 4 * kq) * g.as1);
    }
#pragma unroll
    for (int j = 0; j < 4; ++j) {
#pragma unroll
      for (int e = 0; e < 4; ++e) acc = __builtin_amdgcn_mfma_f32_16x16x4f32(a[j][e], b[j][e], acc, 0, 0, 0);
      if (want_rs) rs += (a[j][0] + a[j][1]) + (a[j][2] + a[j][3]);
    }
  }
  for (; k0 + 16 <= ke; k0 += 16) {
    const int k = k0 + 4 * kq;
    f32x4 a = sg_load4<AK>(ap, k, g.as1), x = {0.f, 0.f, 0.f, 0.f};
    const f32x4 b = sg_load4<BK_>(bp, k, g.bs1);
    if (xp) x = sg_load4<AK>(xp, k, g.as1);
    if (xf) a = sg_xform4<AK>(g, a, x, arow + (long)k * g.as1);
#pragma unroll
    for (int e = 0; e < 4; ++e) acc = __builtin_amdgcn_mfma_f32_16x16x4f32(a[e], b[e], acc, 0, 0, 0);
    if (want_rs) rs += (a[0] + a[1]) + (a[2] + a[3]);
  }
  for (; k0 < ke; k0 += 16) {
    float a[4], b[4];
#pragma unroll
    for (int e = 0; e < 4; ++e) {
      const int k = k0 + 4 * kq + e;
      const bool ok = k < ke;
      const int kc = ok ? k : kb;
      float av = ap[(long)kc * g.as1];
      const float bv = bp[(long)kc * g.bs1];
      if (g.adrop.rng && g.adrop.p > 0.f) av *= sg_drop1(g.adrop, arow + (long)kc * g.as1);
      if (g.adrop.rng && g.adrop.path_p > 0.f) av *= drop_path_factor(g.adrop, (int)((arow + (long)kc * g.as1) / g.a_ld) / g.adrop.rows_per_pass);
      if (xp) av *= act_grad(xp[(long)kc * g.as1], g.a_act);
      a[e] = ok ? av : 0.f; b[e] = ok ? bv : 0.f;
    }
#pragma unroll
    for (int e = 0; e < 4; ++e) acc = __builtin_amdgcn_mfma_f32_16x16x4f32(a[e], b[e], acc, 0, 0, 0);
    if (want_rs) rs += (a[0] + a[1]) + (a[2] + a[3]);
  }
#pragma unroll
  for (int e = 0; e < 4; ++e) part[wave][4 * kq + e][r] = acc[e];
  if (want_rs) {
    rs += __shfl_xor(rs, 16, 64);
    rs += __shfl_xor(rs, 32, 64);
    if (kq == 0) rsum[wave][r] = rs;
  }
  __syncthreads();
  const int tm = tid >> 4, tn = tid & 15;
  const int m = m0 + tm, n = n0 + tn;
  if (want_rs && tid < 16 && m0 + tid < g.M)
    g.rowsum[m0 + tid] += (rsum[0][tid] + rsum[1][tid]) + (rsum[2][tid] + rsum[3][tid]);
  if (m < g.M && n < g.N) {
    float v = (part[0][tm][tn] + part[1][tm][tn]) + (part[2][tm][tn] + part[3][tm][tn]);
    if (g.bias) v += g.bias[g.bias_on_m ? m : n];
    const long off = (long)bz * g.c_bs + m * g.cs0 + n * g.cs1;
    if (g.pre_out) g.pre_out[off] = v;
    v = apply_act(v, g.act);
    if (g.cdrop.rng && g.cdrop.p > 0.f) v *= sg_drop1(g.cdrop, off);
    if (g.cdrop.rng && g.cdrop.path_p > 0.f) v *= drop_path_factor(g.cdrop, m / g.cdrop.rows_per_pass);
    if (g.resid) v += g.resid_scale * g.resid[off];
    float* c = &g.C[off];
    *c = g.accumulate ? *c + v : v;
  }
}

__global__ __launch_bounds__(256) void sgemm_multi_kernel(SgemmMulti mm) {
  __shared__ float part[4][16][17];
  __shared__ float rsum[4][16];
  int blk = blockIdx.x, pi = 0;
#pragma unroll
  for (int i = 0; i + 1 < MT_SGEMM_MAX; ++i)
    if (pi == i && i + 1 < mm.n && blk >= mm.p[i].nblk) { blk -= mm.p[i].nblk; pi = i + 1; }
  const SgemmArgs& g = mm.p[pi];
  const int bx = blk % g.nx, by = (blk / g.nx) % g.ny, bz = blk / (g.nx * g.ny);
  if (g.ak && g.bk) sgemm_tile<true, true>(g, bx, by, bz, part, rsum);
  else if (g.ak) sgemm_tile<true, false>(g, bx, by, bz, part, rsum);
  else if (g.bk) sgemm_tile<false, true>(g, bx, by, bz, part, rsum);
  else sgemm_tile<false, false>(g, bx, by, bz, part, rsum);
}

}

extern "C" int mt_gemm_nt_f16(const mt_half* A, long lda, const MtRowMap* amap, const mt_half* W, int M, int N, int K,
                              int epilogue, const MtGemmEpilogue* epi, void* C, long ldc, const MtRowMap* cmap,
                              int out_dtype, mt_stream_t stream) {
  if (!A || !W || !C || M <= 0 || N <= 0 || K <= 0) return MT_ERR_BAD_ARG;
  if (K % BK != 0 || lda % 8 != 0 || (N % 64) != 0 || (ldc % 4) != 0) return MT_ERR_BAD_ARG;
  if (((uintptr_t)A & 15) || ((uintptr_t)W & 15) || ((uintptr_t)C & 7)) return MT_ERR_BAD_ARG;
  if (epi && epi->resid && (((uintptr_t)epi->resid & 15) || (epi->ldr % 4))) return MT_ERR_BAD_ARG;
  GemmNtArgs a;
  a.A = (const h16*)A; a.lda = lda; a.amap = make_rowmap(amap);
  a.W = (const h16*)W; a.M = M; a.N = N; a.K = K;
  a.m_begin = 0; a.m_end = M;
  a.bias = epi ? epi->bias : nullptr;
  a.resid = epi ? epi->resid : nullptr; a.ldr = epi ? epi->ldr : 0;
  a.rmap = make_rowmap(epi ? &epi->rmap : nullptr);
  a.colscale = epi ? epi->colscale : nullptr;
  a.pos_table = epi ? epi->pos_table : nullptr;
  a.pos_row = epi ? epi->pos_row : nullptr; a.pos_col = epi ? epi->pos_col : nullptr;
  a.drop = make_drop(epi ? &epi->drop : nullptr);
  if (a.drop.active() && epilogue != MT_EPI_BIAS_RESID) return MT_ERR_UNSUPPORTED;
  a.C = C; a.ldc = ldc; a.cmap = make_rowmap(cmap);
  hipStream_t s = (hipStream_t)stream;
  const bool f32 = out_dtype == MT_OUT_F32;
  const char* ps_env = getenv("MT_GEMM_PS");
  if (!(ps_env && ps_env[0] == '0') && !f32 && (epilogue == MT_EPI_BIAS || epilogue == MT_EPI_QKV_HM) && a.amap.seg_rows <= 0 &&
      a.cmap.seg_rows <= 0 && (ldc % 8) == 0 && !((uintptr_t)C & 15) && (epilogue != MT_EPI_QKV_HM || a.bias) && !a.drop.active()) {
    const int rc = mt_gemm_ps_launch(A, lda, W, M, N, K, epilogue, a.bias, C, ldc, s);
    if (rc != MT_ERR_UNSUPPORTED) return rc;
  }
  switch (epilogue) {
    case MT_EPI_BIAS:
      return f32 ? launch_nt_bn<MT_EPI_BIAS, float>(a, s) : launch_nt_bn<MT_EPI_BIAS, h16>(a, s);
    case MT_EPI_BIAS_RESID:
      if (!a.resid) return MT_ERR_BAD_ARG;
      return f32 ? launch_nt_bn<MT_EPI_BIAS_RESID, float>(a, s) : launch_nt_bn<MT_EPI_BIAS_RESID, h16>(a, s);
    case MT_EPI_INJECT:
      if (!a.resid || !a.colscale || !f32) return MT_ERR_BAD_ARG;
      return launch_nt_bn<MT_EPI_INJECT, float>(a, s);
    case MT_EPI_POSEMB:
      if (!a.pos_table || !a.pos_row || !a.pos_col || !f32) return MT_ERR_BAD_ARG;
      return launch_nt_bn<MT_EPI_POSEMB, float>(a, s);
    case MT_EPI_QKV_HM:
      if (f32 || (N % 48) != 0 || cmap) return MT_ERR_BAD_ARG;
      return launch_nt_bn<MT_EPI_QKV_HM, h16>(a, s);
    default:
      return MT_ERR_BAD_ARG;
  }
}

extern "C" int mt_gemm_tn_f16(const mt_half* A, long lda, const MtRowMap* amap, const mt_half* B, long ldb,
                              const MtRowMap* bmap, int M, int N1, int N2, float* C, long ldc, float* colsum,
                              mt_stream_t stream) {
  if (!A || !B || !C || M <= 0 || N1 % 64 || N2 % 64 || lda % 8 || ldb % 8) return MT_ERR_BAD_ARG;
  GemmTnArgs g;
  g.A = (const h16*)A; g.lda = lda; g.amap = make_rowmap(amap);
  g.B = (const h16*)B; g.ldb = ldb; g.bmap = make_rowmap(bmap);
  g.M = M; g.N1 = N1; g.N2 = N2; g.C = C; g.ldc = ldc; g.colsum = colsum;
  const int tiles = (N1 / 64) * (N2 / 64);
  int split = max(1, min(cdiv(M, 256), cdiv(tiles >= 16 ? 1024 : 512, tiles)));
  split = cdiv(split, 8) * 8;
  g.rows_per_split = cdiv(cdiv(M, split), 32) * 32;
  hipLaunchKernelGGL((gemm_tn_kernel<64, 64>), dim3(tiles * split), dim3(256), 0, (hipStream_t)stream, g);
  MT_CHECK_LAUNCH();
  return MT_OK;
}

extern "C" int mt_colsum_f16(const mt_half* A, long lda, const MtRowMap* amap, int M, int N, float* out,
                             mt_stream_t stream) {
  if (!A || !out || M <= 0 || N <= 0 || (N & 7) || (lda & 7)) return MT_ERR_BAD_ARG;
  const int rows_per_block = 256;
  hipLaunchKernelGGL(colsum_kernel, dim3(cdiv(N, 256), cdiv(M, rows_per_block)), dim3(256), 0, (hipStream_t)stream,
                     (const h16*)A, lda, make_rowmap(amap), M, N, rows_per_block, out);
  MT_CHECK_LAUNCH();
  return MT_OK;
}

static int sgemm_fill(const MtSgemm& q, SgemmArgs& g) {
  if (!q.A || !q.B || !q.C || q.M <= 0 || q.N <= 0 || q.K <= 0 || q.batch <= 0 || (q.rowsum && q.batch != 1)) return MT_ERR_BAD_ARG;
  g.A = q.A; g.as0 = q.as0; g.as1 = q.as1; g.a_bs = q.a_bs;
  g.B = q.B; g.bs0 = q.bs0; g.bs1 = q.bs1; g.b_bs = q.b_bs;
  g.bias = q.bias; g.bias_on_m = q.bias_on_m;
  g.C = q.C; g.cs0 = q.cs0; g.cs1 = q.cs1; g.c_bs = q.c_bs;
  g.M = q.M; g.N = q.N; g.K = q.K; g.act = q.act; g.accumulate = q.accumulate;
  g.rowsum = q.rowsum; g.pre_out = q.pre_out; g.resid = q.resid;
  g.cdrop = make_drop(&q.c_drop); g.a_aux = q.a_aux; g.a_act = q.a_act; g.adrop = make_drop(&q.a_drop);
  g.resid_scale = q.resid_scale != 0.f ? q.resid_scale : 1.f;
  g.a_ld = q.a_ld;
  if (g.adrop.rng && g.adrop.path_p > 0.f && q.a_ld < 1) return MT_ERR_BAD_ARG;
  if (g.cdrop.rng && g.cdrop.path_p > 0.f && q.batch != 1) return MT_ERR_UNSUPPORTED;
  if (!(g.cdrop.p > 0.f || g.cdrop.path_p > 0.f)) g.cdrop.rng = nullptr;
  if (!(g.adrop.p > 0.f || g.adrop.path_p > 0.f)) g.adrop.rng = nullptr;
  g.ak = q.as1 == 1 && (q.as0 % 4) == 0 && (q.a_bs % 4) == 0 && ((uintptr_t)q.A & 15) == 0 && ((uintptr_t)q.a_aux & 15) == 0;
  g.bk = q.bs1 == 1 && (q.bs0 % 4) == 0 && (q.b_bs % 4) == 0 && ((uintptr_t)q.B & 15) == 0;
  g.nx = cdiv(q.N, 16); g.ny = cdiv(q.M, 16); g.nblk = g.nx * g.ny * q.batch;
  return MT_OK;
}

extern "C" int mt_sgemm_multi(const MtSgemm* probs, int n, mt_stream_t stream) {
  if (!probs || n < 1 || n > MT_SGEMM_MAX) return MT_ERR_BAD_ARG;
  SgemmMulti mm;
  mm.n = n;
  long blocks = 0;
  for (int i = 0; i < MT_SGEMM_MAX; ++i) {
    const int rc = sgemm_fill(probs[i < n ? i : 0], mm.p[i]);
    if (rc != MT_OK) return rc;
    if (i < n) blocks += mm.p[i].nblk;
  }
  if (blocks > 0x7fffffffL) return MT_ERR_BAD_ARG;
  hipLaunchKernelGGL(sgemm_multi_kernel, dim3((unsigned)blocks), dim3(256), 0, (hipStream_t)stream, mm);
  MT_CHECK_LAUNCH();
// ... 14 lines not shown
```

modaltune_amd/csrc/gemm_ps.hip:

```cpp
#include <stdlib.h>
#include <string.h>

#include <type_traits>

#include "common.h"

namespace {

constexpr int PS_BM = 192, PS_BN = 256;
constexpr int PS_AREG = PS_BM * 64;
constexpr int PS_SLOT = PS_AREG + PS_BN * 64;
constexpr int PS_STAGE = 4 * PS_SLOT;
constexpr int PS_STAGE_ROW = 272;
constexpr int PS_STAGE_WAVE = 16 * PS_STAGE_ROW;
constexpr int PS_BIAS = PS_STAGE + 4 * PS_STAGE_WAVE;
constexpr int PS_LDS = PS_BIAS + 2 * 1024;

struct GemmPsArgs {
  const h16* A; long lda;
  const h16* W;
  const float* bias;
  h16* C; long ldc;
  int M, N, K;
  int nbm, nbn;
  int gc;
};

#ifdef PS_STAMP
__device__ unsigned long long* ps_stamp_buf;
MT_DEVINL unsigned long long ps_now() {
  unsigned long long t;
  __builtin_amdgcn_sched_barrier(0);
  asm volatile("s_memtime %0\n\ts_waitcnt lgkmcnt(0)" : "=s"(t)::"memory");
  __builtin_amdgcn_sched_barrier(0);
  return t;
}
#define PS_T(var) const unsigned long long var = ps_now()
#define PS_ACC(slot, a, b) stamp_acc[slot] += (b) - (a)
#else
#define PS_T(var)
#define PS_ACC(slot, a, b)
#endif

#ifdef PS_GELU_EPI
#define PS_OUT(x) gelu_erf(x)
#else
#define PS_OUT(x) (x)
#endif

template <int N> MT_DEVINL void ps_wait_vmcnt() { asm volatile("s_waitcnt vmcnt(%0)" ::"n"(N) : "memory"); }
MT_DEVINL void ps_barrier() { asm volatile("s_barrier" ::: "memory"); }
MT_DEVINL void ps_dma16(__amdgpu_buffer_rsrc_t rs, unsigned voff, unsigned soff, unsigned lds_byte_off, char* smem) {
  __builtin_amdgcn_raw_ptr_buffer_load_lds(rs, (__attribute__((address_space(3))) void*)(smem + lds_byte_off), 16, voff, soff, 0, 0);
}
MT_DEVINL __amdgpu_buffer_rsrc_t ps_rsrc(const void* base, unsigned bytes) {
  return __builtin_amdgcn_make_buffer_rsrc(const_cast<void*>(base), 0, bytes, 0x00020000);
}

template <typename Args>
MT_DEVINL void tile_of(const Args& g, int idx, int& mt, int& nt) {
  const int per = g.nbm * g.gc;
  const int cg = idx / per, rem = idx - cg * per;
  const int w = min(g.gc, g.nbn - cg * g.gc);
  mt = rem / w;
  nt = cg * g.gc + (rem - mt * w);
}

template <int EPI, bool HAS_BIAS>
__global__ __launch_bounds__(256) __attribute__((amdgpu_waves_per_eu(1, 1))) void gemm_nt_ps_kernel(GemmPsArgs g) {
  __shared__ __attribute__((aligned(16))) char smem[PS_LDS];
  const int tid = threadIdx.x, lane = tid & 63;
  const int wave = __builtin_amdgcn_readfirstlane(tid >> 6);
  const int wr = wave >> 1, wc = wave & 1;
  const int fr = lane & 15, fq = lane >> 4;

  const int ntiles = g.nbm * g.nbn;
  const int xcd = blockIdx.x & 7, slot_id = blockIdx.x >> 3, nslot = gridDim.x >> 3;
  const int tq = ntiles / 8, trm = ntiles % 8;
  const int t_begin = xcd * tq + min(xcd, trm), t_count = tq + (xcd < trm ? 1 : 0);
  const int my_tiles = t_count > slot_id ? (t_count - slot_id + nslot - 1) / nslot : 0;
  if (my_tiles == 0) return;
  const int S = g.K >> 5;

  const int prow = lane >> 2, lchunk = (lane & 3) ^ ((0 - (lane >> 4)) & 3);
  const unsigned lda2 = (unsigned)g.lda * 2u, K2 = (unsigned)g.K * 2u;
  const __amdgpu_buffer_rsrc_t rsA = ps_rsrc(g.A, (unsigned)g.M * lda2), rsW = ps_rsrc(g.W, (unsigned)g.N * K2),
                               rsB = ps_rsrc(HAS_BIAS ? (const void*)g.bias : (const void*)g.W, (unsigned)g.N * 4u),
                               rsC = ps_rsrc(g.C, (unsigned)g.M * (unsigned)g.N * 2u);
  unsigned voffA[3];
  const unsigned voffW = (unsigned)prow * K2 + lchunk * 16, voffB = lane * 16;
  unsigned soffW = 0, soffB = 0;
  int d_tile = 0, d_ks = 0;
  auto dma_tile_setup = [&](int t) {
    const int idx = t_begin + slot_id + min(t, my_tiles - 1) * nslot;
    int mt, nt; tile_of(g, idx, mt, nt);
#pragma unroll
    for (int p = 0; p < 3; ++p) voffA[p] = (unsigned)min(mt * PS_BM + wave * 48 + p * 16 + prow, g.M - 1) * lda2 + lchunk * 16;
    soffW = (unsigned)(nt * PS_BN + wave * 64) * K2;
    soffB = (unsigned)(nt * PS_BN) * 4u;
  };
  auto dma_piece = [&](auto p_c, int qslice) {
    constexpr int p = decltype(p_c)::value;

    const unsigned sb = (unsigned)(qslice & 3) * PS_SLOT, k0 = (unsigned)d_ks * 64;
    if constexpr (p < 3) ps_dma16(rsA, voffA[p], k0, sb + (unsigned)wave * 3072 + p * 1024, smem);
    else if constexpr (p < 7) ps_dma16(rsW, voffW, soffW + (p - 3) * 16 * K2 + k0, sb + PS_AREG + (unsigned)wave * 4096 + (p - 3) * 1024, smem);
    else ps_dma16(rsB, voffB, soffB, PS_BIAS + (unsigned)(d_tile & 1) * 1024, smem);
  };
  auto dma_advance = [&]() { if (++d_ks == S) { d_ks = 0; ++d_tile; dma_tile_setup(d_tile); } };
  using std::integral_constant;
  auto dma_group_all = [&](int qslice) {
    dma_piece(integral_constant<int, 0>{}, qslice); dma_piece(integral_constant<int, 1>{}, qslice);
    dma_piece(integral_constant<int, 2>{}, qslice); dma_piece(integral_constant<int, 3>{}, qslice);
    dma_piece(integral_constant<int, 4>{}, qslice); dma_piece(integral_constant<int, 5>{}, qslice);
    dma_piece(integral_constant<int, 6>{}, qslice);
    if (HAS_BIAS && d_ks == 0) dma_piece(integral_constant<int, 7>{}, qslice);
    dma_advance();
  };

  const unsigned swz = (unsigned)((fq ^ (0 - (fr >> 2))) & 3) * 16;
  const unsigned a_lane = (unsigned)(wr * 96 + fr) * 64 + swz;
  const unsigned b_lane = PS_AREG + (unsigned)(wc * 128 + fr) * 64 + swz;
  auto ld_frag = [&](unsigned off) -> h16x8 { return *reinterpret_cast<const h16x8*>(smem + off); };

  f32x4 acc[6][8];
  h16x4 held[6][8];
#pragma unroll
  for (int i = 0; i < 6; ++i)
#pragma unroll
    for (int j = 0; j < 8; ++j) held[i][j] = (h16x4){(h16)0.f, (h16)0.f, (h16)0.f, (h16)0.f};
  h16x8 bf[8], afA[2], afB[2], afC[2];
  f32x4 cinit[8];

  const unsigned st_w = PS_STAGE + wave * PS_STAGE_WAVE + fr * PS_STAGE_ROW + fq * 8;
  const unsigned st_r = PS_STAGE + wave * PS_STAGE_WAVE + fq * PS_STAGE_ROW + fr * 16;
  const unsigned row_bytes = EPI == MT_EPI_QKV_HM ? 96u : (unsigned)(g.ldc * 2);
  unsigned held_off = 0;
  int held_rows_left = 0;
  h16x8 dr[4];
  auto drain_write1 = [&](auto c_c, auto j_c) {
    constexpr int c = decltype(c_c)::value, j = decltype(j_c)::value;
    *reinterpret_cast<h16x4*>(smem + st_w + j * 32) = held[c][j];
  };
  auto drain_read1 = [&](auto t_c) {
    constexpr int t = decltype(t_c)::value;
    dr[t] = *reinterpret_cast<const h16x8*>(smem + st_r + t * 4 * PS_STAGE_ROW);
  };
  auto drain_store1 = [&](auto c_c, auto t_c) {
    constexpr int c = decltype(c_c)::value, t = decltype(t_c)::value;
    const unsigned vo = (c * 16 + t * 4 < held_rows_left) ? held_off : 0xffffff00u;
    __builtin_amdgcn_raw_buffer_store_b128(__builtin_bit_cast(__attribute__((__vector_size__(4 * sizeof(unsigned)))) unsigned, dr[t]), rsC, vo,
                                           (unsigned)(c * 16 + t * 4) * row_bytes, 0);
  };
  auto convert_pair = [&](auto i0_c) {
    constexpr int i0 = decltype(i0_c)::value;
#pragma unroll
    for (int r = 0; r < 2; ++r)
#pragma unroll
      for (int j = 0; j < 8; ++j)
        held[i0 + r][j] = (h16x4){(h16)PS_OUT(acc[i0 + r][j][0]), (h16)PS_OUT(acc[i0 + r][j][1]), (h16)PS_OUT(acc[i0 + r][j][2]), (h16)PS_OUT(acc[i0 + r][j][3])};
  };

  dma_tile_setup(0);
  dma_group_all(0);
  dma_group_all(1);
  dma_group_all(2);
  ps_wait_vmcnt<0>();
  ps_barrier();
#pragma unroll
  for (int j = 0; j < 7; ++j) bf[j] = ld_frag(b_lane + j * 1024);
  afA[0] = ld_frag(a_lane); afA[1] = ld_frag(a_lane + 1024);

#ifdef PS_STAMP
  unsigned long long stamp_acc[6] = {0, 0, 0, 0, 0, 0};
  const unsigned long long k_begin = ps_now();
#endif
  int q = 0;
  for (int t = 0; t < my_tiles; ++t) {
// ... 7 lines not shown
      ps_wait_vmcnt<NWAIT>();
      PS_T(s1);
      ps_barrier();
      __builtin_amdgcn_sched_barrier(0);
      PS_T(s2);
#pragma unroll
      for (int n = 0; n < 48; ++n) {
        const int pr = n >> 4, k = (n & 15) >> 1, r = n & 1, i = 2 * pr + r;
        const h16x8& af = pr == 0 ? afA[r] : pr == 1 ? afB[r] : afC[r];
        acc[i][k] = __builtin_amdgcn_mfma_f32_16x16x32_f16(bf[k], af, MODE == 0 ? (HAS_BIAS ? cinit[k] : (f32x4){0.f, 0.f, 0.f, 0.f}) : acc[i][k], 0, 0, 0);
        if (n == 0) bf[7] = ld_frag(sa + b_lane + 7 * 1024);
        if (n == 1) afB[0] = ld_frag(sa + a_lane + 2 * 1024);
        if (n == 2) afB[1] = ld_frag(sa + a_lane + 3 * 1024);
        if (n == 8) afC[0] = ld_frag(sa + a_lane + 4 * 1024);
        if (n == 9) afC[1] = ld_frag(sa + a_lane + 5 * 1024);
        if (n == 16) afA[0] = ld_frag(sn + a_lane);
        if (n == 17) afA[1] = ld_frag(sn + a_lane + 1024);
        if (n >= 33 && n <= 45 && (n & 1)) bf[(n - 33) >> 1] = ld_frag(sn + b_lane + ((n - 33) >> 1) * 1024);
#ifndef PS_NO_DMA
        if (n == 3) dma_piece(integral_constant<int, 0>{}, q + 3);
        if (n == 10) dma_piece(integral_constant<int, 1>{}, q + 3);
        if (n == 18) dma_piece(integral_constant<int, 2>{}, q + 3);
        if (n == 24) dma_piece(integral_constant<int, 3>{}, q + 3);
        if (n == 30) dma_piece(integral_constant<int, 4>{}, q + 3);
        if (n == 36) dma_piece(integral_constant<int, 5>{}, q + 3);
        if (n == 42) dma_piece(integral_constant<int, 6>{}, q + 3);
        if constexpr (HAS_BIAS && BIASGRP) { if (n == 46) dma_piece(integral_constant<int, 7>{}, q + 3); }
#endif
        if constexpr (DRAIN >= 0) {
          if (n == 4) drain_write1(integral_constant<int, DC>{}, integral_constant<int, 0>{});
          if (n == 5) drain_write1(integral_constant<int, DC>{}, integral_constant<int, 1>{});
          if (n == 6) drain_write1(integral_constant<int, DC>{}, integral_constant<int, 2>{});
          if (n == 7) drain_write1(integral_constant<int, DC>{}, integral_constant<int, 3>{});
          if (n == 11) drain_write1(integral_constant<int, DC>{}, integral_constant<int, 4>{});
          if (n == 12) drain_write1(integral_constant<int, DC>{}, integral_constant<int, 5>{});
          if (n == 13) drain_write1(integral_constant<int, DC>{}, integral_constant<int, 6>{});
          if (n == 14) drain_write1(integral_constant<int, DC>{}, integral_constant<int, 7>{});
          if (n == 19) drain_read1(integral_constant<int, 0>{});
          if (n == 20) drain_read1(integral_constant<int, 1>{});
          if (n == 21) drain_read1(integral_constant<int, 2>{});
          if (n == 22) drain_read1(integral_constant<int, 3>{});
          if (n == 26) drain_store1(integral_constant<int, DC>{}, integral_constant<int, 0>{});
          if (n == 27) drain_store1(integral_constant<int, DC>{}, integral_constant<int, 1>{});
          if (n == 28) drain_store1(integral_constant<int, DC>{}, integral_constant<int, 2>{});
          if (n == 29) drain_store1(integral_constant<int, DC>{}, integral_constant<int, 3>{});
        }
        if constexpr (MODE == 2) {
          if (n >= 16) {
            const int ci = (n - 16) >> 3, cj = (n - 16) & 7;
            held[ci][cj] = (h16x4){(h16)PS_OUT(acc[ci][cj][0]), (h16)PS_OUT(acc[ci][cj][1]), (h16)PS_OUT(acc[ci][cj][2]), (h16)PS_OUT(acc[ci][cj][3])};
          }
        }
        __builtin_amdgcn_sched_barrier(0);
      }
      dma_advance();
      if constexpr (MODE == 2) convert_pair(integral_constant<int, 4>{});
      PS_T(s3);
      if (MODE == 1 && DRAIN < 0 && !BIASGRP) { PS_ACC(0, s0, s1); PS_ACC(1, s1, s2); PS_ACC(2, s2, s3); PS_ACC(5, s3 - 1, s3); }
      ++q;
    };
    using I0 = integral_constant<int, 0>; using I1 = integral_constant<int, 1>; using I2 = integral_constant<int, 2>;
    using NoDrain = integral_constant<int, -1>;
    constexpr int G = 7, GB = HAS_BIAS ? 8 : 7;
    if constexpr (HAS_BIAS) {
#pragma unroll
      for (int j = 0; j < 8; ++j) cinit[j] = *reinterpret_cast<const f32x4*>(smem + PS_BIAS + (t & 1) * 1024 + (wc * 128 + j * 16 + fq * 4) * 4);
    }
    slice(I0{}, NoDrain{}, integral_constant<int, G>{}, I0{});
    slice(I1{}, integral_constant<int, 0>{}, integral_constant<int, G>{}, I0{});
    slice(I1{}, integral_constant<int, 1>{}, integral_constant<int, G + 4>{}, I0{});
    slice(I1{}, integral_constant<int, 2>{}, integral_constant<int, G + 4>{}, I0{});
    slice(I1{}, integral_constant<int, 3>{}, integral_constant<int, G + 4>{}, I0{});
    slice(I1{}, integral_constant<int, 4>{}, integral_constant<int, G + 4>{}, I0{});
    slice(I1{}, integral_constant<int, 5>{}, integral_constant<int, G + 4>{}, I0{});
    slice(I1{}, NoDrain{}, integral_constant<int, G + 4>{}, I0{});
    for (int ks = 8; ks < S - 3; ++ks) slice(I1{}, NoDrain{}, integral_constant<int, G>{}, I0{});
    slice(I1{}, NoDrain{}, integral_constant<int, G>{}, I1{});
    slice(I1{}, NoDrain{}, integral_constant<int, GB>{}, I0{});
    __builtin_amdgcn_sched_barrier(0);
    slice(I2{}, NoDrain{}, integral_constant<int, G>{}, I0{});
    {
      const int idx = t_begin + slot_id + t * nslot;
      int mt, nt; tile_of(g, idx, mt, nt);
      const int m = mt * PS_BM + wr * 96 + fq, n = nt * PS_BN + wc * 128 + fr * 8;
      held_rows_left = g.M - m;
      held_off = EPI == MT_EPI_QKV_HM ? (unsigned)(((n / 48) * g.M + m) * 48 + n % 48) * 2u
                                       : (unsigned)m * (unsigned)(g.ldc * 2) + (unsigned)n * 2u;
    }
    __builtin_amdgcn_sched_barrier(0);
  }
#ifdef PS_STAMP
  if (tid == 0) {
    const unsigned long long k_end = ps_now();
    unsigned long long* o = ps_stamp_buf + blockIdx.x * 8;
    for (int i = 0; i < 6; ++i) o[i] = stamp_acc[i];
    o[6] = k_end - k_begin; o[7] = my_tiles;
  }
#endif
#define PS_DRAIN_OPEN(c)                                                                                                      \
  drain_write1(integral_constant<int, c>{}, integral_constant<int, 0>{}); drain_write1(integral_constant<int, c>{}, integral_constant<int, 1>{}); \
  drain_write1(integral_constant<int, c>{}, integral_constant<int, 2>{}); drain_write1(integral_constant<int, c>{}, integral_constant<int, 3>{}); \
  drain_write1(integral_constant<int, c>{}, integral_constant<int, 4>{}); drain_write1(integral_constant<int, c>{}, integral_constant<int, 5>{}); \
  drain_write1(integral_constant<int, c>{}, integral_constant<int, 6>{}); drain_write1(integral_constant<int, c>{}, integral_constant<int, 7>{}); \
  drain_read1(integral_constant<int, 0>{}); drain_read1(integral_constant<int, 1>{}); drain_read1(integral_constant<int, 2>{});       \
  drain_read1(integral_constant<int, 3>{});                                                                                            \
  drain_store1(integral_constant<int, c>{}, integral_constant<int, 0>{}); drain_store1(integral_constant<int, c>{}, integral_constant<int, 1>{}); \
  drain_store1(integral_constant<int, c>{}, integral_constant<int, 2>{}); drain_store1(integral_constant<int, c>{}, integral_constant<int, 3>{});
  PS_DRAIN_OPEN(0) PS_DRAIN_OPEN(1) PS_DRAIN_OPEN(2) PS_DRAIN_OPEN(3) PS_DRAIN_OPEN(4) PS_DRAIN_OPEN(5)
#undef PS_DRAIN_OPEN
  ps_wait_vmcnt<0>();
}

}

int mt_gemm_ps_launch(const void* A, long lda, const void* W, int M, int N, int K, int epilogue, const float* bias, void* C, long ldc, hipStream_t s);
#ifdef PS_STAMP
extern "C" int mt_gemm_ps_set_stamps(void* buf) { return hipMemcpyToSymbol(HIP_SYMBOL(ps_stamp_buf), &buf, sizeof(buf)) == hipSuccess ? 0 : -1; }
extern "C" int mt_gemm_ps_stamp_launch(const void* A, long lda, const void* W, int M, int N, int K, const float* bias, void* C, long ldc) {
  return mt_gemm_ps_launch(A, lda, W, M, N, K, MT_EPI_BIAS, bias, C, ldc, nullptr);
}
#endif

int mt_gemm_ps_launch(const void* A, long lda, const void* W, int M, int N, int K, int epilogue, const float* bias, void* C, long ldc,
                      hipStream_t s) {
  if (N % 256 != 0 || K % 64 != 0 || K < 768 || M < 256) return MT_ERR_UNSUPPORTED;
  static int ncu = 0;
  if (!ncu) {
    int dev = 0;
    if (hipGetDevice(&dev) != hipSuccess || hipDeviceGetAttribute(&ncu, hipDeviceAttributeMultiprocessorCount, dev) != hipSuccess || ncu <= 0)
      ncu = 256;
  }
  GemmPsArgs g;
  g.A = (const h16*)A; g.lda = lda; g.W = (const h16*)W; g.bias = bias; g.C = (h16*)C; g.ldc = ldc;
  g.M = M; g.N = N; g.K = K;
  g.nbm = cdiv(M, PS_BM); g.nbn = N / PS_BN;
  {
    const char* e = getenv("MT_GEMM_GC");
    const int want = e ? atoi(e) : 0;
    g.gc = want > 0 ? min(want, g.nbn) : (g.nbn <= 4 ? g.nbn : max(2, min(g.nbn, 3072 / K)));
  }
  const int ntiles = g.nbm * g.nbn;
  const int rounds = cdiv(ntiles, ncu);
  static const char* force = getenv("MT_GEMM_FORCE");
  if (force && force[0] && strcmp(force, "ps") != 0) return MT_ERR_UNSUPPORTED;
  if (!(force && force[0]) && (2 * ntiles < 3 * ncu || 4L * ntiles < 3L * rounds * ncu)) return MT_ERR_UNSUPPORTED;
  if (ldc != N && epilogue != MT_EPI_QKV_HM) return MT_ERR_UNSUPPORTED;
  if (K > 2304 && !(force && force[0])) return MT_ERR_UNSUPPORTED;
  int grid = min(ncu, ntiles);
  grid = max(8, grid / 8 * 8);
  if (lda < K || (long)M * lda * 2 >= (1L << 32) || (long)M * N * 2 >= (1L << 32) || (long)N * K * 2 >= (1L << 32)) return MT_ERR_UNSUPPORTED;
  if (epilogue == MT_EPI_QKV_HM) {
    if (!bias || N % 48 != 0) return MT_ERR_UNSUPPORTED;
    hipLaunchKernelGGL((gemm_nt_ps_kernel<MT_EPI_QKV_HM, true>), dim3(grid), dim3(256), 0, s, g);
  } else if (bias) {
    hipLaunchKernelGGL((gemm_nt_ps_kernel<MT_EPI_BIAS, true>), dim3(grid), dim3(256), 0, s, g);
  } else {
    hipLaunchKernelGGL((gemm_nt_ps_kernel<MT_EPI_BIAS, false>), dim3(grid), dim3(256), 0, s, g);
  }
  MT_CHECK_LAUNCH();
  return MT_OK;
}
```

modaltune_amd/csrc/layer.hip:

```cpp
#include "common.h"

namespace {

MtGemmEpilogue epi_bias(const float* bias) {
  MtGemmEpilogue e{};
  e.bias = bias;
  return e;
}
#define MT_TRY(call)              \
  do {                            \
    const int st__ = (call);      \
    if (st__ != MT_OK) return st__; \
  } while (0)

}

extern "C" int mt_longnet_layer_fwd(const MtLongNetLayerWeights* w, const MtLongNetLayerBuffers* b, const MtDilatedPlan* plan, int M,
                                    int D, int F, const float* pend_x, const mt_half* pend_branch, const MtDropout* pend_drop, int defer,
                                    float* out, const MtDropout* drop_attn, const MtDropout* drop_ffn, mt_stream_t s) {
  if (!w || !b || !plan || M < 1 || D != 768 || (!defer && !out)) return MT_ERR_BAD_ARG;
  if (!pend_x)
    MT_TRY(mt_layernorm_fwd(b->hin, D, nullptr, MT_OUT_F32, 0, w->ln1_w, w->ln1_b, nullptr, 0, b->u16, D, nullptr, MT_OUT_F16, b->st1, M, D, s));
  else
    MT_TRY(mt_add_layernorm_fwd(pend_x, pend_branch, pend_drop, w->ln1_w, w->ln1_b, b->hin, b->u16, b->st1, M, D, s));
  MtGemmEpilogue e = epi_bias(w->b_qkv);
  MT_TRY(mt_gemm_nt_f16(b->u16, D, nullptr, w->w_qkv, M, 3 * D, D, MT_EPI_QKV_HM, &e, b->qkv, 3 * D, nullptr, MT_OUT_F16, s));
  MT_TRY(mt_dilated_attn_fwd(b->qkv, plan, b->o_br, b->lse_br, s));
  MT_TRY(mt_dilated_mix_ln_fwd(b->o_br, b->lse_br, plan, w->inner_ln_w, w->inner_ln_b, b->u16, b->stin, b->lse_tot, s));
  e = epi_bias(w->b_out);
  MT_TRY(mt_gemm_nt_f16(b->u16, D, nullptr, w->w_out, M, D, D, MT_EPI_BIAS, &e, b->br16, D, nullptr, MT_OUT_F16, s));
  MT_TRY(mt_add_layernorm_fwd(b->hin, b->br16, drop_attn, w->ln2_w, w->ln2_b, b->hmid, b->u16, b->st2, M, D, s));
  e = epi_bias(w->b_fc1);
  MT_TRY(mt_gemm_nt_f16(b->u16, D, nullptr, w->w_fc1, M, F, D, MT_EPI_BIAS, &e, b->a1, F, nullptr, MT_OUT_F16, s));
  MT_TRY(mt_layernorm_fwd(b->a1, F, nullptr, MT_OUT_F16, 1, w->ffn_ln_w, w->ffn_ln_b, nullptr, 0, b->t16, F, nullptr, MT_OUT_F16, b->stf, M, F, s));
  e = epi_bias(w->b_fc2);
  if (defer) return mt_gemm_nt_f16(b->t16, F, nullptr, w->w_fc2, M, D, F, MT_EPI_BIAS, &e, b->br16, D, nullptr, MT_OUT_F16, s);
  e.resid = b->hmid; e.ldr = D;
  if (drop_ffn) e.drop = *drop_ffn;
  return mt_gemm_nt_f16(b->t16, F, nullptr, w->w_fc2, M, D, F, MT_EPI_BIAS_RESID, &e, out, D, nullptr, MT_OUT_F32, s);
}

extern "C" int mt_longnet_layer_bwd(const MtLongNetLayerWeights* w, const MtLongNetLayerBuffers* b, const MtDilatedPlan* plan, int M,
                                    int D, int F, int dh16_valid, int feeds_lower, const MtDropout* drop_attn, const MtDropout* drop_ffn,
                                    const MtDropout* drop_lower_ffn, mt_stream_t s) {
  if (!w || !b || !plan || M < 1 || D != 768) return MT_ERR_BAD_ARG;
  const MtGemmEpilogue none{};
  const mt_half* src16 = b->dh16;
  if (!dh16_valid) {
    MT_TRY(mt_cast_f32_to_f16(b->dh, b->dy16, (long)M * D, drop_ffn, D, s));
    src16 = b->dy16;
  }
  MT_TRY(mt_gemm_nt_f16(src16, D, nullptr, w->wt_fc2, M, F, D, MT_EPI_BIAS, &none, b->dt16, F, nullptr, MT_OUT_F16, s));
  MT_TRY(mt_layernorm_bwd(b->dt16, F, nullptr, MT_OUT_F16, b->a1, F, nullptr, MT_OUT_F16, 1, w->ffn_ln_w, b->stf, b->da1, F, nullptr,
                          MT_OUT_F16, 0, nullptr, nullptr, nullptr, nullptr, M, F, s));
  MT_TRY(mt_gemm_nt_f16(b->da1, F, nullptr, w->wt_fc1, M, D, F, MT_EPI_BIAS, &none, b->dy16, D, nullptr, MT_OUT_F16, s));
  MT_TRY(mt_layernorm_bwd(b->dy16, D, nullptr, MT_OUT_F16, b->hmid, D, nullptr, MT_OUT_F32, 0, w->ln2_w, b->st2, b->dh, D, nullptr, MT_OUT_F32,
                          1, nullptr, nullptr, b->dh16, drop_attn, M, D, s));
  MT_TRY(mt_gemm_nt_f16(b->dh16, D, nullptr, w->wt_out, M, D, D, MT_EPI_BIAS, &none, b->u16, D, nullptr, MT_OUT_F16, s));
  MT_TRY(mt_dilated_mix_ln_bwd(b->u16, b->o_br, b->lse_br, b->lse_tot, plan, w->inner_ln_w, b->stin, b->dmixed, b->delta, s));
  MT_TRY(mt_dilated_attn_bwd(b->qkv, b->dmixed, b->lse_tot, b->delta, plan, b->attn_ws, b->dqkv16, MT_ATTN_BWD_ALL, s));
  MT_TRY(mt_gemm_nt_f16(b->dqkv16, 3 * D, nullptr, w->wt_qkv, M, D, 3 * D, MT_EPI_BIAS, &none, b->dy16, D, nullptr, MT_OUT_F16, s));
  return mt_layernorm_bwd(b->dy16, D, nullptr, MT_OUT_F16, b->hin, D, nullptr, MT_OUT_F32, 0, w->ln1_w, b->st1, b->dh, D, nullptr, MT_OUT_F32, 1,
                          nullptr, nullptr, feeds_lower ? b->dh16 : nullptr, feeds_lower ? drop_lower_ffn : nullptr, M, D, s);
}

extern "C" int mt_vit_block_fwd(const MtVitBlockWeights* w, const MtVitBlockBuffers* b, const MtDensePlan* plan, int M, int D, int F,
                                const float* pend_x, const mt_half* pend_branch, int defer, float* out, mt_stream_t s) {
  if (!w || !b || !plan || M < 1 || D != 768 || (!defer && !out)) return MT_ERR_BAD_ARG;
  if (!pend_x)
    MT_TRY(mt_layernorm_fwd_eps(b->hin, D, nullptr, MT_OUT_F32, 0, w->n1_w, w->n1_b, nullptr, 0, b->u16, D, nullptr, MT_OUT_F16, b->st1, M, D,
                                w->n1_eps, s));
  else
    MT_TRY(mt_add_layernorm_fwd_eps(pend_x, pend_branch, nullptr, w->n1_w, w->n1_b, b->hin, b->u16, b->st1, M, D, w->n1_eps, s));
  MtGemmEpilogue e = epi_bias(w->b_qkv);
  MT_TRY(mt_gemm_nt_f16(b->u16, D, nullptr, w->w_qkv, M, 3 * D, D, MT_EPI_BIAS, &e, b->qkv, 3 * D, nullptr, MT_OUT_F16, s));
  MT_TRY(mt_dense_attn_fwd(b->qkv, plan, b->o16, b->lse, s));
  e = epi_bias(w->b_proj);
  MT_TRY(mt_gemm_nt_f16(b->o16, D, nullptr, w->w_proj, M, D, D, MT_EPI_BIAS, &e, b->br16, D, nullptr, MT_OUT_F16, s));
  MT_TRY(mt_add_layernorm_fwd_eps(b->hin, b->br16, nullptr, w->n2_w, w->n2_b, b->hmid, b->u16, b->st2, M, D, w->n2_eps, s));
  e = epi_bias(w->b_fc1);
  MT_TRY(mt_gemm_nt_f16(b->u16, D, nullptr, w->w_fc1, M, F, D, MT_EPI_BIAS, &e, b->a1, F, nullptr, MT_OUT_F16, s));
  MT_TRY(mt_gelu_f16_fwd(b->a1, b->t16, (long)M * F, s));
  e = epi_bias(w->b_fc2);
  if (defer) return mt_gemm_nt_f16(b->t16, F, nullptr, w->w_fc2, M, D, F, MT_EPI_BIAS, &e, b->br16, D, nullptr, MT_OUT_F16, s);
  e.resid = b->hmid; e.ldr = D;
  return mt_gemm_nt_f16(b->t16, F, nullptr, w->w_fc2, M, D, F, MT_EPI_BIAS_RESID, &e, out, D, nullptr, MT_OUT_F32, s);
}

extern "C" int mt_vit_block_bwd(const MtVitBlockWeights* w, const MtVitBlockBuffers* b, const MtDensePlan* plan, int M, int D, int F,
                                int dh16_valid, int feeds_lower, mt_stream_t s) {
  if (!w || !b || !plan || M < 1 || D != 768) return MT_ERR_BAD_ARG;
  const MtGemmEpilogue none{};
  const mt_half* src16 = b->dh16;
  if (!dh16_valid) {
    MT_TRY(mt_cast_f32_to_f16(b->dh, b->dy16, (long)M * D, nullptr, 0, s));
    src16 = b->dy16;
  }
  MT_TRY(mt_gemm_nt_f16(src16, D, nullptr, w->wt_fc2, M, F, D, MT_EPI_BIAS, &none, b->dt16, F, nullptr, MT_OUT_F16, s));
  MT_TRY(mt_gelu_f16_bwd(b->a1, b->dt16, b->da1, (long)M * F, s));
  MT_TRY(mt_gemm_nt_f16(b->da1, F, nullptr, w->wt_fc1, M, D, F, MT_EPI_BIAS, &none, b->dy16, D, nullptr, MT_OUT_F16, s));
  MT_TRY(mt_layernorm_bwd(b->dy16, D, nullptr, MT_OUT_F16, b->hmid, D, nullptr, MT_OUT_F32, 0, w->n2_w, b->st2, b->dh, D, nullptr, MT_OUT_F32, 1,
                          nullptr, nullptr, b->dh16, nullptr, M, D, s));
  MT_TRY(mt_gemm_nt_f16(b->dh16, D, nullptr, w->wt_proj, M, D, D, MT_EPI_BIAS, &none, b->u16, D, nullptr, MT_OUT_F16, s));
  MT_TRY(mt_dense_attn_bwd(b->qkv, b->o16, b->u16, b->lse, plan, b->delta, b->dqkv16, MT_DENSE_BWD_ALL, s));
  MT_TRY(mt_gemm_nt_f16(b->dqkv16, 3 * D, nullptr, w->wt_qkv, M, D, 3 * D, MT_EPI_BIAS, &none, b->dy16, D, nullptr, MT_OUT_F16, s));
  return mt_layernorm_bwd(b->dy16, D, nullptr, MT_OUT_F16, b->hin, D, nullptr, MT_OUT_F32, 0, w->n1_w, b->st1, b->dh, D, nullptr, MT_OUT_F32, 1,
                          nullptr, nullptr, feeds_lower ? b->dh16 : nullptr, nullptr, M, D, s);
}
```

modaltune_amd/csrc/norm.hip:

```cpp
#include "common.h"

namespace {

template <typename T> struct Vec4;
template <> struct Vec4<float> {
  static MT_DEVINL f32x4 load(const float* p) { return *reinterpret_cast<const f32x4*>(p); }
  static MT_DEVINL void store(float* p, f32x4 v) { *reinterpret_cast<f32x4*>(p) = v; }
};
template <> struct Vec4<h16> {
  static MT_DEVINL f32x4 load(const h16* p) {
    h16x4 v = *reinterpret_cast<const h16x4*>(p);
    return (f32x4){(float)v[0], (float)v[1], (float)v[2], (float)v[3]};
  }
  static MT_DEVINL void store(h16* p, f32x4 v) {
    *reinterpret_cast<h16x4*>(p) = (h16x4){(h16)v[0], (h16)v[1], (h16)v[2], (h16)v[3]};
  }
};

struct LnFwdArgs {
  const void* x; long ldx; RowMap xmap;
  const float* w; const float* b; const float* add_rows; int add_period;
  void* y; long ldy; RowMap ymap;
  float* stats; int M;
  float eps;
};

template <int D, typename InT, typename OutT, bool GELU>
__global__ __launch_bounds__(256) void ln_fwd_kernel(LnFwdArgs a) {
  constexpr int NC = D / 256;
  const int lane = threadIdx.x & 63, wave = threadIdx.x >> 6;
  f32x4 wr[NC], br[NC];
#pragma unroll
  for (int c = 0; c < NC; ++c) {
    wr[c] = Vec4<float>::load(a.w + c * 256 + lane * 4);
    br[c] = Vec4<float>::load(a.b + c * 256 + lane * 4);
  }
  for (int m = blockIdx.x * 4 + wave; m < a.M; m += gridDim.x * 4) {
    const InT* x = reinterpret_cast<const InT*>(a.x) + a.xmap.map(m) * a.ldx;
    f32x4 v[NC];
    float s = 0.f;
#pragma unroll
    for (int c = 0; c < NC; ++c) {
      v[c] = Vec4<InT>::load(x + c * 256 + lane * 4);
      if (GELU) {
#pragma unroll
        for (int e = 0; e < 4; ++e) v[c][e] = gelu_erf(v[c][e]);
      }
      s += v[c][0] + v[c][1] + v[c][2] + v[c][3];
    }
    const float mean = wave_sum(s) * (1.0f / D);
    float q = 0.f;
#pragma unroll
    for (int c = 0; c < NC; ++c)
#pragma unroll
      for (int e = 0; e < 4; ++e) { const float d = v[c][e] - mean; q += d * d; }
    const float rstd = rsqrtf(wave_sum(q) * (1.0f / D) + a.eps);
    OutT* y = reinterpret_cast<OutT*>(a.y) + a.ymap.map(m) * a.ldy;
    const float* add = a.add_rows ? a.add_rows + (long)(m % a.add_period) * D : nullptr;
#pragma unroll
    for (int c = 0; c < NC; ++c) {
      const int col = c * 256 + lane * 4;
      f32x4 o;
#pragma unroll
      for (int e = 0; e < 4; ++e) o[e] = (v[c][e] - mean) * rstd * wr[c][e] + br[c][e];
      if (add) { const f32x4 p = Vec4<float>::load(add + col); o += p; }
      Vec4<OutT>::store(y + col, o);
    }
    if (a.stats && lane == 0) { a.stats[2 * (long)m] = mean; a.stats[2 * (long)m + 1] = rstd; }
  }
}

struct AddLnArgs {
  const float* x; const h16* branch; DropArgs drop;
  const float* w; const float* b;
  float* h; h16* y; float* stats; int M;
  float eps;
};

template <int D>
__global__ __launch_bounds__(256) void add_ln_fwd_kernel(AddLnArgs a) {
  constexpr int NC = D / 256;
  const int lane = threadIdx.x & 63, wave = threadIdx.x >> 6;
  f32x4 wr[NC], br[NC];
#pragma unroll
  for (int c = 0; c < NC; ++c) {
    wr[c] = Vec4<float>::load(a.w + c * 256 + lane * 4);
    br[c] = Vec4<float>::load(a.b + c * 256 + lane * 4);
  }
  const bool dropping = a.drop.active();
  for (int m = blockIdx.x * 4 + wave; m < a.M; m += gridDim.x * 4) {
    const float* x = a.x + (long)m * D;
    const h16* bp = a.branch + (long)m * D;
    f32x4 v[NC], bv[NC];
#pragma unroll
    for (int c = 0; c < NC; ++c) {
      v[c] = Vec4<float>::load(x + c * 256 + lane * 4);
      bv[c] = Vec4<h16>::load(bp + c * 256 + lane * 4);
    }
    const float pf = dropping ? drop_path_factor(a.drop, m / a.drop.rows_per_pass) : 1.f;
    float s = 0.f;
    float* hrow = a.h + (long)m * D;
#pragma unroll
    for (int c = 0; c < NC; ++c) {
      const int col = c * 256 + lane * 4;
      if (dropping) bv[c] *= drop_elem4(a.drop, ((uint64_t)m * D + col) >> 2, pf);
      v[c] += bv[c];
      Vec4<float>::store(hrow + col, v[c]);
      s += v[c][0] + v[c][1] + v[c][2] + v[c][3];
    }
    const float mean = wave_sum(s) * (1.0f / D);
    float q = 0.f;
#pragma unroll
    for (int c = 0; c < NC; ++c)
#pragma unroll
      for (int e = 0; e < 4; ++e) { const float d = v[c][e] - mean; q += d * d; }
    const float rstd = rsqrtf(wave_sum(q) * (1.0f / D) + a.eps);
    h16* y = a.y + (long)m * D;
#pragma unroll
    for (int c = 0; c < NC; ++c) {
      f32x4 o;
#pragma unroll
      for (int e = 0; e < 4; ++e) o[e] = (v[c][e] - mean) * rstd * wr[c][e] + br[c][e];
      Vec4<h16>::store(y + c * 256 + lane * 4, o);
    }
    if (lane == 0) { a.stats[2 * (long)m] = mean; a.stats[2 * (long)m + 1] = rstd; }
  }
}

struct LnBwdArgs {
  const void* dy; long lddy; RowMap dymap;
  const void* x; long ldx; RowMap xmap;
  const float* w; const float* stats;
  void* dx; long lddx; RowMap dxmap; int accumulate;
  float* dw; float* db; h16* dx16; DropArgs drop16; int M;
};

template <int D, typename DyT, typename InT, typename DxT, bool GELU, bool PARAM>
__global__ __launch_bounds__(256) void ln_bwd_kernel(LnBwdArgs a) {
  constexpr int NC = D / 256;
  constexpr int NP = PARAM ? NC : 1;
  const int lane = threadIdx.x & 63, wave = threadIdx.x >> 6;
  f32x4 gw[NP], gb[NP];
#pragma unroll
  for (int c = 0; c < NP; ++c) { gw[c] = (f32x4){0.f, 0.f, 0.f, 0.f}; gb[c] = gw[c]; }
  f32x4 wr[NC];
#pragma unroll
  for (int c = 0; c < NC; ++c) wr[c] = Vec4<float>::load(a.w + c * 256 + lane * 4);
  for (int m = blockIdx.x * 4 + wave; m < a.M; m += gridDim.x * 4) {
    const DyT* dy = reinterpret_cast<const DyT*>(a.dy) + a.dymap.map(m) * a.lddy;
    const InT* x = reinterpret_cast<const InT*>(a.x) + a.xmap.map(m) * a.ldx;
    const float mean = a.stats[2 * (long)m], rstd = a.stats[2 * (long)m + 1];
    f32x4 xh[NC], g[NC], raw[GELU ? NC : 1];
    float s1 = 0.f, s2 = 0.f;
#pragma unroll
    for (int c = 0; c < NC; ++c) {
      const int col = c * 256 + lane * 4;
      f32x4 xv = Vec4<InT>::load(x + col);
      if (GELU) {
        raw[c] = xv;
#pragma unroll
        for (int e = 0; e < 4; ++e) xv[e] = gelu_erf(xv[e]);
      }
      const f32x4 d = Vec4<DyT>::load(dy + col);
#pragma unroll
      for (int e = 0; e < 4; ++e) {
        xh[c][e] = (xv[e] - mean) * rstd;
        g[c][e] = d[e] * wr[c][e];
        s1 += g[c][e];
        s2 += g[c][e] * xh[c][e];
      }
      if (PARAM) {
#pragma unroll
        for (int e = 0; e < 4; ++e) { gw[c][e] += d[e] * xh[c][e]; gb[c][e] += d[e]; }
      }
    }
    const float c1 = wave_sum(s1) * (1.0f / D), c2 = wave_sum(s2) * (1.0f / D);
    DxT* dx = reinterpret_cast<DxT*>(a.dx) + a.dxmap.map(m) * a.lddx;
#pragma unroll
    for (int c = 0; c < NC; ++c) {
      const int col = c * 256 + lane * 4;
      f32x4 o;
#pragma unroll
      for (int e = 0; e < 4; ++e) {
        o[e] = rstd * (g[c][e] - c1 - xh[c][e] * c2);
        if (GELU) o[e] *= gelu_erf_grad(raw[c][e]);
      }
      if (a.accumulate) { const f32x4 old = Vec4<DxT>::load(dx + col); o += old; }
      Vec4<DxT>::store(dx + col, o);
      if (a.dx16) {
        if (a.drop16.active()) o *= drop_scale4(a.drop16, ((uint64_t)m * D + col) >> 2, m);
        Vec4<h16>::store(a.dx16 + (long)m * D + col, o);
      }
    }
  }
  if (PARAM) {
    __shared__ float red[2][4][D];
#pragma unroll
    for (int c = 0; c < NP; ++c)
#pragma unroll
      for (int e = 0; e < 4; ++e) {
        red[0][wave][c * 256 + lane * 4 + e] = gw[c][e];
        red[1][wave][c * 256 + lane * 4 + e] = gb[c][e];
      }
    __syncthreads();
    for (int i = threadIdx.x; i < D; i += 256) {
      atomicAdd(&a.dw[i], red[0][0][i] + red[0][1][i] + red[0][2][i] + red[0][3][i]);
      atomicAdd(&a.db[i], red[1][0][i] + red[1][1][i] + red[1][2][i] + red[1][3][i]);
    }
  }
}


MT_DEVINL f32x2 pk_fma2(f32x2 a, f32x2 b, f32x2 c) { return __builtin_elementwise_fma(a, b, c); }
MT_DEVINL f32x2 splat2(float v) { return (f32x2){v, v}; }

template <bool WANT_GRAD>
MT_DEVINL void gelu_pair(f32x2 x, f32x2& g, f32x2& dg) {
  const f32x2 ax = {fabsf(x[0]), fabsf(x[1])};
  const f32x2 z = ax * splat2(0.70710678118654752440f);
  const f32x2 den = pk_fma2(z, splat2(0.3275911f), splat2(1.0f));
  const f32x2 t = {__builtin_amdgcn_rcpf(den[0]), __builtin_amdgcn_rcpf(den[1])};
  f32x2 poly = pk_fma2(t, splat2(1.061405429f), splat2(-1.453152027f));
  poly = pk_fma2(poly, t, splat2(1.421413741f));
  poly = pk_fma2(poly, t, splat2(-0.284496736f));
  poly = pk_fma2(poly, t, splat2(0.254829592f));
  poly = poly * t;
  const f32x2 ea = z * z * splat2(-1.4426950408889634f);
  const f32x2 e = {__builtin_amdgcn_exp2f(ea[0]), __builtin_amdgcn_exp2f(ea[1])};
  const f32x2 r = pk_fma2(-poly, e, splat2(1.0f));
  const f32x2 er = {copysignf(r[0], x[0]), copysignf(r[1], x[1])};
  const f32x2 h = pk_fma2(er, splat2(0.5f), splat2(0.5f));
// ... 343 lines not shown
    for (int i = 0; i < 4; ++i) {
      const int r = r0 + ty + 8 * i, c = c0 + tx;
      const float v = (r < R && c < C) ? src[(long)r * C + c] : 0.f;
      tile[ty + 8 * i][tx] = v;
      if (dst && r < R && c < C) dst[(long)(roff + r) * ld + c] = (h16)v;
    }
    __syncthreads();
    if (dst_t) {
#pragma unroll
      for (int i = 0; i < 4; ++i) {
        const int c = c0 + ty + 8 * i, r = r0 + tx;
        if (r < R && c < C) dst_t[(long)c * ld_t + roff + r] = (h16)tile[tx][ty + 8 * i];
      }
    }
    __syncthreads();
  }
}

int ew_grid(long n) { return (int)max(1L, min((n + 1023) / 1024, 4096L)); }

}

extern "C" int mt_layernorm_fwd_eps(const void* x, long ldx, const MtRowMap* xmap, int in_dtype, int gelu_in,
                                    const float* w, const float* b, const float* add_rows, int add_period, void* y,
                                    long ldy, const MtRowMap* ymap, int out_dtype, float* stats, int M, int D, float eps,
                                    mt_stream_t stream) {
  if (!x || !y || !w || !b || M <= 0 || (ldx & 3) || (ldy & 3) || !(eps > 0.f)) return MT_ERR_BAD_ARG;
  LnFwdArgs a{x, ldx, make_rowmap(xmap), w, b, add_rows, add_period > 0 ? add_period : 1, y, ldy, make_rowmap(ymap), stats, M, eps};
  hipStream_t s = (hipStream_t)stream;
  switch (D) {
    case 256: return ln_fwd_types<256>(a, in_dtype, out_dtype, gelu_in, s);
    case 768: return ln_fwd_types<768>(a, in_dtype, out_dtype, gelu_in, s);
    case 2304: return ln_fwd_types<2304>(a, in_dtype, out_dtype, gelu_in, s);
    case 3072: return ln_fwd_types<3072>(a, in_dtype, out_dtype, gelu_in, s);
    default: return MT_ERR_UNSUPPORTED;
  }
}

extern "C" int mt_layernorm_fwd(const void* x, long ldx, const MtRowMap* xmap, int in_dtype, int gelu_in,
                                const float* w, const float* b, const float* add_rows, int add_period, void* y,
                                long ldy, const MtRowMap* ymap, int out_dtype, float* stats, int M, int D,
                                mt_stream_t stream) {
  return mt_layernorm_fwd_eps(x, ldx, xmap, in_dtype, gelu_in, w, b, add_rows, add_period, y, ldy, ymap, out_dtype, stats, M, D, 1e-5f,
                              stream);
}

extern "C" int mt_add_layernorm_fwd_eps(const float* x, const mt_half* branch, const MtDropout* drop, const float* w,
                                        const float* b, float* h, mt_half* y, float* stats, int M, int D, float eps,
                                        mt_stream_t stream) {
  if (!x || !branch || !w || !b || !h || !y || !stats || M <= 0 || h == x || !(eps > 0.f)) return MT_ERR_BAD_ARG;
  if (D != 768) return MT_ERR_UNSUPPORTED;
  AddLnArgs a{x, (const h16*)branch, make_drop(drop), w, b, h, (h16*)y, stats, M, eps};
  hipLaunchKernelGGL((add_ln_fwd_kernel<768>), dim3(ln_grid(M)), dim3(256), 0, (hipStream_t)stream, a);
  MT_CHECK_LAUNCH();
  return MT_OK;
}

extern "C" int mt_add_layernorm_fwd(const float* x, const mt_half* branch, const MtDropout* drop, const float* w,
                                    const float* b, float* h, mt_half* y, float* stats, int M, int D, mt_stream_t stream) {
  return mt_add_layernorm_fwd_eps(x, branch, drop, w, b, h, y, stats, M, D, 1e-5f, stream);
}

template <int D>
static int ln_bwd_types(const LnBwdArgs& a, int dy_dt, int in_dt, int dx_dt, int gelu, hipStream_t s) {
  const bool dyh = dy_dt == MT_OUT_F16, inh = in_dt == MT_OUT_F16, dxh = dx_dt == MT_OUT_F16;
  if (gelu) {
    if constexpr (D % 1024 == 0) {
      if (dyh && inh && dxh && !a.dw && !(a.lddy & 7) && !(a.ldx & 7) && !(a.lddx & 7)) {
        constexpr int WPR = (D % 1536 == 0) ? 3 : 2;
        hipLaunchKernelGGL((ln_gelu_bwd_kernel<D, WPR>), dim3(min(a.M, 16384)), dim3(64 * WPR), 0, s, a);
        MT_CHECK_LAUNCH();
        return MT_OK;
      }
    }
    if (dyh && inh && dxh) return ln_bwd_launch<D, h16, h16, h16, true>(a, s);
    return MT_ERR_UNSUPPORTED;
  }
  if (dyh && !inh && !dxh) return ln_bwd_launch<D, h16, float, float, false>(a, s);
  if (dyh && !inh && dxh) return ln_bwd_launch<D, h16, float, h16, false>(a, s);
  if (!dyh && !inh && !dxh) return ln_bwd_launch<D, float, float, float, false>(a, s);
  return MT_ERR_UNSUPPORTED;
}

extern "C" int mt_layernorm_bwd(const void* dy, long lddy, const MtRowMap* dymap, int dy_dtype, const void* x,
                                long ldx, const MtRowMap* xmap, int in_dtype, int gelu_in, const float* w,
                                const float* stats, void* dx, long lddx, const MtRowMap* dxmap, int dx_dtype,
                                int accumulate, float* dw, float* db, mt_half* dx_f16, const MtDropout* dx_f16_drop, int M,
                                int D, mt_stream_t stream) {
  if (!dy || !x || !w || !stats || !dx || M <= 0 || (!dw) != (!db)) return MT_ERR_BAD_ARG;
  if (dx_f16 && gelu_in) return MT_ERR_UNSUPPORTED;
  LnBwdArgs a{dy, lddy, make_rowmap(dymap), x, ldx, make_rowmap(xmap), w, stats, dx, lddx, make_rowmap(dxmap), accumulate, dw, db,
              (h16*)dx_f16, make_drop(dx_f16 ? dx_f16_drop : nullptr), M};
  hipStream_t s = (hipStream_t)stream;
  switch (D) {
    case 256: return ln_bwd_types<256>(a, dy_dtype, in_dtype, dx_dtype, gelu_in, s);
    case 768: return ln_bwd_types<768>(a, dy_dtype, in_dtype, dx_dtype, gelu_in, s);
    case 2304: return ln_bwd_types<2304>(a, dy_dtype, in_dtype, dx_dtype, gelu_in, s);
    case 3072: return ln_bwd_types<3072>(a, dy_dtype, in_dtype, dx_dtype, gelu_in, s);
    default: return MT_ERR_UNSUPPORTED;
  }
}

extern "C" int mt_cast_f32_to_f16(const float* x, mt_half* y, long n, const MtDropout* drop, int D, mt_stream_t stream) {
  if (!x || !y || n <= 0) return MT_ERR_BAD_ARG;
  const DropArgs d = make_drop(drop);
  if (d.active()) {
    if ((n & 3) || D <= 0 || (D & 3)) return MT_ERR_BAD_ARG;
    hipLaunchKernelGGL(cast_drop_f32_f16_kernel, dim3(ew_grid(n / 4 + 1)), dim3(256), 0, (hipStream_t)stream, x, (h16*)y, n, d, D);
  } else {
    hipLaunchKernelGGL(cast_f32_f16_kernel, dim3(ew_grid(n / 4 + 1)), dim3(256), 0, (hipStream_t)stream, x, (h16*)y, n);
  }
  MT_CHECK_LAUNCH();
  return MT_OK;
}
extern "C" int mt_rng_advance(unsigned* rng, mt_stream_t stream) {
  if (!rng) return MT_ERR_BAD_ARG;
  hipLaunchKernelGGL(rng_advance_kernel, dim3(1), dim3(64), 0, (hipStream_t)stream, rng);
  MT_CHECK_LAUNCH();
  return MT_OK;
}
extern "C" int mt_dropout_f32(const float* x, long ldx, const MtRowMap* xmap, float* y, int M, int D, const MtDropout* drop,
                              mt_stream_t stream) {
  if (!x || !y || M <= 0 || D <= 0 || (D & 3) || (ldx & 3)) return MT_ERR_BAD_ARG;
  hipLaunchKernelGGL(dropout_f32_kernel, dim3(ew_grid((long)M * D / 4 + 1)), dim3(256), 0, (hipStream_t)stream, x, ldx,
                     make_rowmap(xmap), y, M, D, make_drop(drop));
  MT_CHECK_LAUNCH();
  return MT_OK;
}
extern "C" int mt_droppath_rows_f32(float* x, int M, int D, const MtDropout* drop, mt_stream_t stream) {
  if (!x || M <= 0 || D <= 0 || (D & 3)) return MT_ERR_BAD_ARG;
  const DropArgs d = make_drop(drop);
  if (!d.active() || d.path_p <= 0.f) return MT_OK;
  hipLaunchKernelGGL(droppath_rows_kernel, dim3(ew_grid((long)M * D / 4 + 1)), dim3(256), 0, (hipStream_t)stream, x, M, D, d);
  MT_CHECK_LAUNCH();
  return MT_OK;
}
extern "C" int mt_cast_f16_to_f32(const mt_half* x, float* y, long n, mt_stream_t stream) {
  if (!x || !y || n <= 0) return MT_ERR_BAD_ARG;
  hipLaunchKernelGGL(cast_f16_f32_kernel, dim3(ew_grid(n / 4 + 1)), dim3(256), 0, (hipStream_t)stream, (const h16*)x, y, n);
  MT_CHECK_LAUNCH();
  return MT_OK;
}
extern "C" int mt_pack_weight_f16(const float* src, int R, int C, mt_half* dst, int transpose, mt_stream_t stream) {
  if (!src || !dst || R <= 0 || C <= 0) return MT_ERR_BAD_ARG;
  hipLaunchKernelGGL(pack_f16_kernel, dim3(cdiv(C, 32), cdiv(R, 32)), dim3(256), 0, (hipStream_t)stream, src, R, C, (h16*)dst, transpose);
  MT_CHECK_LAUNCH();
  return MT_OK;
}
extern "C" int mt_pack_weights_f16(const long long* items, int n_items, mt_stream_t stream) {
  if (!items || n_items <= 0) return MT_ERR_BAD_ARG;
  hipLaunchKernelGGL(pack_group_kernel, dim3(n_items, 48), dim3(256), 0, (hipStream_t)stream, items);
  MT_CHECK_LAUNCH();
  return MT_OK;
}
extern "C" int mt_act_fwd(const float* x, float* y, long n, int act, mt_stream_t stream) {
  if (!x || !y || n <= 0) return MT_ERR_BAD_ARG;
  hipLaunchKernelGGL(act_fwd_kernel, dim3(ew_grid(n)), dim3(256), 0, (hipStream_t)stream, x, y, n, act);
  MT_CHECK_LAUNCH();
  return MT_OK;
}
extern "C" int mt_act_bwd(const float* x, const float* dy, float* dx, long n, int act, mt_stream_t stream) {
  if (!x || !dy || !dx || n <= 0) return MT_ERR_BAD_ARG;
  hipLaunchKernelGGL(act_bwd_kernel, dim3(ew_grid(n)), dim3(256), 0, (hipStream_t)stream, x, dy, dx, n, act);
  MT_CHECK_LAUNCH();
  return MT_OK;
}
extern "C" int mt_axpy(const float* a, const float* b, float alpha, float* y, long n, mt_stream_t stream) {
  if (!a || !b || !y || n <= 0) return MT_ERR_BAD_ARG;
  hipLaunchKernelGGL(axpy_kernel, dim3(ew_grid(n)), dim3(256), 0, (hipStream_t)stream, a, b, alpha, y, n);
  MT_CHECK_LAUNCH();
  return MT_OK;
}
extern "C" int mt_axpy_bcast(const float* a, const float* b, float alpha, float* y, long n, long period, mt_stream_t stream) {
  if (!a || !b || !y || n <= 0 || period <= 0) return MT_ERR_BAD_ARG;
  hipLaunchKernelGGL(axpy_bcast_kernel, dim3(ew_grid(n)), dim3(256), 0, (hipStream_t)stream, a, b, alpha, y, n, period);
  MT_CHECK_LAUNCH();
  return MT_OK;
}
extern "C" int mt_fold_rows(const float* x, int reps, long period, float* out, mt_stream_t stream) {
  if (!x || !out || reps < 1 || period <= 0 || (period & 3) || ((uintptr_t)x & 15) || ((uintptr_t)out & 15)) return MT_ERR_BAD_ARG;
  hipLaunchKernelGGL(fold_rows_kernel, dim3(ew_grid(period / 4)), dim3(256), 0, (hipStream_t)stream, x, reps, period, out);
  MT_CHECK_LAUNCH();
  return MT_OK;
// ... 21 lines not shown
```

modaltune_amd/engine.py:

```python
from __future__ import annotations


import os
from typing import Dict, List, Optional, Sequence

import numpy as np
import torch

from . import ops
from ._lib import rowmap
from .config import ModelConfig, branch_table, coords_to_rowcol, segment_lengths, sincos_1d_table, DILATED_RATIOS
from .synth import param_specs
from .tape import Param, Tape, Var

H16 = torch.float16
F32 = torch.float32


class ParamStore:

    def __init__(self, cfg: ModelConfig, group_sizes: Sequence[int], device):
        self.cfg, self.group_sizes, self.device = cfg, list(group_sizes), device
        self.specs = param_specs(cfg, group_sizes)
        off = 0
# ... 65 lines not shown
QK_SCALE_LOG2 = 0.14433756729740643 * 1.4426950408889634


def _scaled_copy(t: torch.Tensor, alpha: float) -> torch.Tensor:
    out = torch.empty_like(t)
    a = torch.full((1,), float(alpha), dtype=F32, device=t.device)
    ops.axpy_dev(None, t.contiguous(), a, out)
    return out


class _W16:

    def __init__(self, srcs: Sequence[torch.Tensor], device, need_t: bool = True):
        self.srcs = list(srcs)
        self.N = sum(s.shape[0] for s in srcs)
        self.K = srcs[0].shape[1]
        self.w = torch.empty(self.N, self.K, dtype=H16, device=device)
        self.wt = torch.empty(self.K, self.N, dtype=H16, device=device) if need_t else None
        self.refresh()

    def refresh(self):
        r = 0
        for s in self.srcs:
            n = s.shape[0]
            ops.pack_weight(s, self.w[r:r + n], n, self.K, transpose=False)
            r += n
        if self.wt is not None:
            if len(self.srcs) == 1:
                ops.pack_weight(self.srcs[0], self.wt, self.N, self.K, transpose=True)
            else:
                full = torch.empty(self.N, self.K, dtype=F32, device=self.w.device)
                r = 0
                for s in self.srcs:
                    full[r:r + s.shape[0]].copy_(s)
                    r += s.shape[0]
                ops.pack_weight(full, self.wt, self.N, self.K, transpose=True)


class Engine:
    def __init__(self, cfg: ModelConfig, group_sizes: Sequence[int], device="cuda"):
        cfg.validate()
        self.cfg, self.device = cfg, torch.device(device)
        self.group_sizes = list(group_sizes)
        self.store = ParamStore(cfg, group_sizes, self.device)
        self.tape = Tape(self.device)
        self._fresh_arenas = {"need": 0, "pool": []}
        self.tape.on_realloc = self._bump_generation
        self._main_tape = self.tape
        self.seg_lengths = segment_lengths(cfg.max_wsi_size, cfg.tile_size)
        self.pos_table = torch.from_numpy(sincos_1d_table(cfg.slide_ngrids, cfg.embed_dim // 2)).to(self.device)
        self._frozen16: Dict[str, _W16] = {}
        self._train16: Dict[str, _W16] = {}
        self._ws: Dict[tuple, Dict[str, torch.Tensor]] = {}
        self._ws_store: Dict[tuple, dict] = {}
        self._caches_ready = False
        self.generation = 0
        self.grad_ready_hook = None
        self.record_markers = False
        self._coord_err = torch.zeros(1, dtype=torch.int32, device=self.device)
        self._coord_err_host = None
        self._coord_err_event = None
        self._pin_ring: List[tuple] = []
        self._pin_next = 0
        self.collect_taps = False
        self.taps: Dict[str, torch.Tensor] = {}
        self.T = cfg.num_tokens
        self._mean_w = torch.full((max(self.T, 2),), 1.0 / max(1, cfg.gene.final_groups), device=self.device)
        sl, G = self.store.slots, len(self.group_sizes)
        offs = [[sl[f"gene_encoder.gene_networks.{i}.{a}.0.{w}"][0] for a, w in ((0, "weight"), (0, "bias"), (1, "weight"), (1, "bias"))]
                for i in range(G)]
        goff = np.concatenate([[0], np.cumsum(self.group_sizes)[:-1]]).astype(np.int64)
        self._gene_offs = torch.tensor(offs, dtype=torch.int64, device=self.device)
        self._gene_sizes = torch.tensor(self.group_sizes, dtype=torch.int32, device=self.device)
        self._gene_goff = torch.from_numpy(goff).to(self.device)
        self._gene_total = int(sum(self.group_sizes))
        self.stochastic = False
        self.rng = torch.zeros(4, dtype=torch.int32, device=self.device)
        self._drop_now = False
        self._fresh_calls, self._site_base = 0, 0
        self._fresh_tick = 0
        self._fresh_pool: Dict[int, list] = {}
        dpr = np.linspace(0.0, float(cfg.drop_path_rate), cfg.depth) if cfg.depth > 1 else np.zeros(1)
        self._layer_path_p = [float(v) for v in dpr]
        self.leaf_stream = os.environ.get("MT_LEAF_STREAM", "0") == "1"
        self._side, self._side_refs, self._side_busy = None, [], False

    def _bump_generation(self):
        self.generation += 1

    def _leaf(self, fn, *keep):
        if not self.leaf_stream:
            fn()
            return
        if self._side is None:
            self._side = torch.cuda.Stream(device=self.device)
        self._side.wait_stream(torch.cuda.current_stream(self.device))
        with torch.cuda.stream(self._side):
            fn()
        self._side_refs.extend(keep)
        self._side_busy = True

    def _leaf_join(self):
        if self._side_busy:
            torch.cuda.current_stream(self.device).wait_stream(self._side)
            self._side_refs.clear()
            self._side_busy = False

    def set_stochastic(self, on: bool, seed: int = 0):
        if bool(on) != self.stochastic:
            self.generation += 1
        self.stochastic = bool(on)
        self.rng.copy_(torch.tensor([seed & 0x7FFFFFFF, (seed >> 31) & 0x7FFFFFFF, 0, 0], dtype=torch.int32))

    def _drop(self, site: int, p: float, path_site: int = 0, path_p: float = 0.0, rows_per_pass: int = 1):
        if not self._drop_now or (p <= 0.0 and path_p <= 0.0):
            return None
        off = self._site_base
        return ops.dropout_spec(self.rng, site + off, p, path_site + off, path_p, rows_per_pass)

    def _layer_drops(self, l: int, N: int):
        if l < 0:
            return None, None
        p, pp = float(self.cfg.dropout), self._layer_path_p[l]
        return (self._drop(16 + 4 * l, p, 17 + 4 * l, pp, N), self._drop(18 + 4 * l, p, 19 + 4 * l, pp, N))

    def load_state_dict(self, state, strict=True):
        self.store.load(state, strict)
        self._caches_ready = False
        self.generation += 1

    def _build_caches(self):
        t, dev, cfg = self.store.tensors, self.device, self.cfg
        self._frozen16 = {"patch": _W16([t["patch_embed.proj.weight"]], dev, need_t=False)}
        for l in range(cfg.depth):
            p = f"encoder.layers.{l}."
            self._frozen16[p + "qkv"] = _W16([_scaled_copy(t[p + "self_attn.q_proj.weight"], QK_SCALE_LOG2),
                                              t[p + "self_attn.k_proj.weight"], t[p + "self_attn.v_proj.weight"]], dev)
            self._frozen16[p + "out"] = _W16([t[p + "self_attn.out_proj.weight"]], dev)
            self._frozen16[p + "fc1"] = _W16([t[p + "ffn.fc1.weight"]], dev)
            self._frozen16[p + "fc2"] = _W16([t[p + "ffn.fc2.weight"]], dev)
            self._frozen16[p + "bqkv"] = torch.cat([_scaled_copy(t[p + "self_attn.q_proj.bias"], QK_SCALE_LOG2),
                                                    t[p + "self_attn.k_proj.bias"], t[p + "self_attn.v_proj.bias"]]).contiguous()
        self._layer_w = []
        for l in range(cfg.depth):
            p = f"encoder.layers.{l}."
            f16 = self._frozen16
            self._layer_w.append(ops.struct_of(
                ops.MtLongNetLayerWeights, ln1_w=t[p + "self_attn_layer_norm.weight"], ln1_b=t[p + "self_attn_layer_norm.bias"],
                inner_ln_w=t[p + "self_attn.inner_attn_ln.weight"], inner_ln_b=t[p + "self_attn.inner_attn_ln.bias"],
                ln2_w=t[p + "final_layer_norm.weight"], ln2_b=t[p + "final_layer_norm.bias"], ffn_ln_w=t[p + "ffn.ffn_layernorm.weight"],
                ffn_ln_b=t[p + "ffn.ffn_layernorm.bias"], b_qkv=f16[p + "bqkv"], b_out=t[p + "self_attn.out_proj.bias"],
                b_fc1=t[p + "ffn.fc1.bias"], b_fc2=t[p + "ffn.fc2.bias"], w_qkv=f16[p + "qkv"].w, w_out=f16[p + "out"].w, w_fc1=f16[p + "fc1"].w,
                w_fc2=f16[p + "fc2"].w, wt_qkv=f16[p + "qkv"].wt, wt_out=f16[p + "out"].wt, wt_fc1=f16[p + "fc1"].wt, wt_fc2=f16[p + "fc2"].wt))
        self._train16 = {}
        self._pack_table = None
        for pref in self._cross_attn_prefixes():
            self._train16[pref + "q_proj"] = _W16([t[pref + "q_proj.weight"]], dev)
            self._train16[pref + "q_in"] = _W16([t[pref + "multihead_attn.q_proj_weight"]], dev)
            self._train16[pref + "kv"] = _W16([t[pref + "multihead_attn.k_proj_weight"], t[pref + "multihead_attn.v_proj_weight"]], dev)
            self._train16[pref + "out_in"] = _W16([t[pref + "multihead_attn.out_proj.weight"]], dev)
            self._train16[pref + "output_proj"] = _W16([t[pref + "output_proj.weight"]], dev)
        self._caches_ready = True
        self.generation += 1

    def refresh_trainable_caches(self):
        if not self._caches_ready:
# ... 424 lines not shown

    def _injector(self, i: int, c: Var, pe: Param, src: torch.Tensor, src_map, hin: torch.Tensor, first: bool):
        cfg, ctx, tape, P, t = self.cfg, self._ctx, self.tape, self.store.param, self.store.tensors
        B, L, N, Mp, D, E, T = ctx["B"], ctx["L"], ctx["N"], ctx["Mp"], cfg.embed_dim, cfg.adapter_dim, self.T
        pref = f"interactions.{i}.injector."
        ap = pref + "attn."
        pm = ctx["patch_map"]
        w16 = self._train16
        dev = self.device
        chat = tape.layernorm(c, P(ap + "norm_kq.weight"), P(ap + "norm_kq.bias"), add_rows=pe)
        _, Wk, Wv, _, bk, bv = self._mha_in(ap + "multihead_attn.")
        k, v = tape.linear_group([(chat, Wk, bk), (chat, Wv, bv)])
        xhat = torch.empty(Mp, D, dtype=H16, device=dev)
        st = torch.empty(Mp, 2, dtype=F32, device=dev)
        ops.layernorm_fwd(src, t[ap + "norm.weight"], t[ap + "norm.bias"], xhat, st, Mp, D, xmap=src_map)
        q1 = torch.empty(Mp, E, dtype=H16, device=dev)
        ops.gemm_nt(xhat, w16[ap + "q_proj"].w, q1, Mp, E, D, bias=t[ap + "q_proj.bias"])
        q2 = torch.empty(Mp, E, dtype=H16, device=dev)
        bqi = t[ap + "multihead_attn.in_proj_bias"][:E]
        ops.gemm_nt(q1, w16[ap + "q_in"].w, q2, Mp, E, E, bias=bqi)
        a = torch.empty(Mp, E, dtype=H16, device=dev)
        alse = torch.empty(Mp, 12, dtype=F32, device=dev)
        ops.inject_attn_fwd(q2, k.data, v.data, a, Mp, L, T, lse=alse)
        o1 = torch.empty(Mp, E, dtype=H16, device=dev)
        ops.gemm_nt(a, w16[ap + "out_in"].w, o1, Mp, E, E, bias=t[ap + "multihead_attn.out_proj.bias"])
        ops.gemm_nt(o1, w16[ap + "output_proj"].w, hin, Mp, D, E, cmap=pm, epilogue=ops.EPI_INJECT, bias=t[ap + "output_proj.bias"],
                    resid=src, ldr=D, rmap=src_map, colscale=t[pref + "gamma"])
        g = self.store.grads
        ws = ctx["ws"]

        def bwd():
            dh = ws["dh"]
            proj = torch.empty(Mp, D, dtype=H16, device=dev)
            ops.gemm_nt(o1, w16[ap + "output_proj"].w, proj, Mp, D, E, bias=t[ap + "output_proj.bias"])
            dproj = torch.empty(Mp, D, dtype=H16, device=dev)
            ops.inject_resid_bwd(dh, src, proj, t[pref + "gamma"], dh if not first else ws["scratch32"], dproj,
                                 g[pref + "gamma"], Mp, D, dymap=pm, xmap=src_map, dxmap=pm if not first else None)
            self._leaf(lambda: ops.gemm_tn(dproj, o1, g[ap + "output_proj.weight"], Mp, D, E, colsum=g[ap + "output_proj.bias"]), dproj, o1)
            do1 = torch.empty(Mp, E, dtype=H16, device=dev)
            ops.gemm_nt(dproj, w16[ap + "output_proj"].wt, do1, Mp, E, D)
            self._leaf(lambda: ops.gemm_tn(do1, a, g[ap + "multihead_attn.out_proj.weight"], Mp, E, E, colsum=g[ap + "multihead_attn.out_proj.bias"]),
                       do1, a)
            da = torch.empty(Mp, E, dtype=H16, device=dev)
            ops.gemm_nt(do1, w16[ap + "out_in"].wt, da, Mp, E, E)
            dq2 = torch.empty(Mp, E, dtype=H16, device=dev)
            ops.inject_attn_bwd(q2, a, alse, da, k.data, v.data, dq2, k.g(), v.g(), Mp, L, T)
            self._leaf(lambda: ops.gemm_tn(dq2, q1, g[ap + "multihead_attn.q_proj_weight"], Mp, E, E, colsum=g[ap + "multihead_attn.in_proj_bias"][:E]),
                       dq2, q1)
            dq1 = torch.empty(Mp, E, dtype=H16, device=dev)
            ops.gemm_nt(dq2, w16[ap + "q_in"].wt, dq1, Mp, E, E)
            self._leaf(lambda: ops.gemm_tn(dq1, xhat, g[ap + "q_proj.weight"], Mp, E, D, colsum=g[ap + "q_proj.bias"]), dq1, xhat)
            dxhat = torch.empty(Mp, D, dtype=H16, device=dev)
            ops.gemm_nt(dq1, w16[ap + "q_proj"].wt, dxhat, Mp, D, E)
            if first:
                ops.layernorm_bwd(dxhat, src, t[ap + "norm.weight"], st, ws["scratch32"], Mp, D, xmap=src_map,
                                  dw=g[ap + "norm.weight"], db=g[ap + "norm.bias"])
            else:
                ops.layernorm_bwd(dxhat, src, t[ap + "norm.weight"], st, dh, Mp, D, xmap=src_map, dxmap=pm, accumulate=True,
                                  dw=g[ap + "norm.weight"], db=g[ap + "norm.bias"])
        tape.record(bwd)

    def _layer(self, l: int, out: torch.Tensor, pend=None, defer: bool = False):
        cfg, ctx, t = self.cfg, self._ctx, self.store.tensors
        M, D, Fd, ws, plan = ctx["M"], cfg.embed_dim, cfg.ffn_dim, ctx["ws"], ctx["plan"]
        p = f"encoder.layers.{l}."
        f16 = self._frozen16
        hin, hmid, qkv, obr, lsebr, lsetot, a1 = (ws[f"hin{l}"], ws[f"hmid{l}"], ws[f"qkv{l}"], ws[f"obr{l}"], ws[f"lsebr{l}"],
                                                  ws[f"lsetot{l}"], ws[f"a1_{l}"])
        st1, stin, st2, stf = ws[f"st1_{l}"], ws[f"stin_{l}"], ws[f"st2_{l}"], ws[f"stf_{l}"]
        u16, t16 = ws["u16"], ws["t16"]
        N_tok = ctx["N"]
        d_attn, d_ffn = self._layer_drops(l, N_tok)
        br16 = ws["br16"]
        feeds_lower = all(l != a for a, _ in cfg.interaction_indexes)
        d_lower_ffn = self._layer_drops(l - 1, N_tok)[1] if feeds_lower else None
        if ops.TIMER is None:
            cb = ws.get(("_cb", l))
            if cb is None:
                cb = ws[("_cb", l)] = ops.struct_of(
                    ops.MtLongNetLayerBuffers, hin=hin, hmid=hmid, qkv=qkv, o_br=obr, lse_br=lsebr, lse_tot=lsetot, a1=a1, st1=st1, stin=stin,
                    st2=st2, stf=stf, u16=u16, br16=br16, t16=t16, dh=ws["dh"], dy16=ws["dy16"], dh16=ws["dh16"], dt16=ws["dt16"],
                    da1=ws["da1"], dmixed=ws["dmixed"], dqkv16=ws["dqkv16"], delta=ws["delta"], attn_ws=ws["attn_ws"])
            lw = self._layer_w[l]
            ops.longnet_layer_fwd(lw, cb, plan, M, D, Fd, out, pend=pend, defer=defer, drop_attn=d_attn, drop_ffn=d_ffn)

            def bwd_c():
                ops.longnet_layer_bwd(lw, cb, plan, M, D, Fd, bool(ctx.get("dh16_valid")), feeds_lower, drop_attn=d_attn, drop_ffn=d_ffn,
                                      drop_lower_ffn=d_lower_ffn)
                ctx["dh16_valid"] = feeds_lower
            self.tape.record(bwd_c)
            return (hmid, br16, d_ffn) if defer else None
        if pend is None:
            ops.layernorm_fwd(hin, t[p + "self_attn_layer_norm.weight"], t[p + "self_attn_layer_norm.bias"], u16, st1, M, D)
        else:
            ops.add_layernorm_fwd(pend[0], pend[1], t[p + "self_attn_layer_norm.weight"], t[p + "self_attn_layer_norm.bias"],
                                  hin, u16, st1, M, D, drop=pend[2])
        ops.gemm_nt(u16, f16[p + "qkv"].w, qkv, M, 3 * D, D, bias=f16[p + "bqkv"], epilogue=ops.EPI_QKV_HM)
        ops.dilated_attn_fwd(qkv, plan, obr, lsebr)
        ops.dilated_mix_ln_fwd(obr, lsebr, plan, t[p + "self_attn.inner_attn_ln.weight"], t[p + "self_attn.inner_attn_ln.bias"],
                               u16, stin, lsetot)
        ops.gemm_nt(u16, f16[p + "out"].w, br16, M, D, D, bias=t[p + "self_attn.out_proj.bias"])
        ops.add_layernorm_fwd(hin, br16, t[p + "final_layer_norm.weight"], t[p + "final_layer_norm.bias"], hmid, u16, st2, M, D,
                              drop=d_attn)
        ops.gemm_nt(u16, f16[p + "fc1"].w, a1, M, Fd, D, bias=t[p + "ffn.fc1.bias"])
        ops.layernorm_fwd(a1, t[p + "ffn.ffn_layernorm.weight"], t[p + "ffn.ffn_layernorm.bias"], t16, stf, M, Fd, gelu_in=True)
        if defer:
            ops.gemm_nt(t16, f16[p + "fc2"].w, br16, M, D, Fd, bias=t[p + "ffn.fc2.bias"])
            nxt = (hmid, br16, d_ffn)
        else:
            ops.gemm_nt(t16, f16[p + "fc2"].w, out, M, D, Fd, epilogue=ops.EPI_BIAS_RESID, bias=t[p + "ffn.fc2.bias"], resid=hmid, ldr=D,
                        drop=d_ffn)
            nxt = None

        def bwd():
            dh, dy16, dt16, da1 = ws["dh"], ws["dy16"], ws["dt16"], ws["da1"]
            if ctx.get("dh16_valid"):
                src16 = ws["dh16"]
            else:
                ops.cast_f32_to_f16(dh, dy16, drop=d_ffn, D=D)
                src16 = dy16
            ops.gemm_nt(src16, f16[p + "fc2"].wt, dt16, M, Fd, D)
            ops.layernorm_bwd(dt16, a1, t[p + "ffn.ffn_layernorm.weight"], stf, da1, M, Fd, gelu_in=True)
            ops.gemm_nt(da1, f16[p + "fc1"].wt, dy16, M, D, Fd)
            ops.layernorm_bwd(dy16, hmid, t[p + "final_layer_norm.weight"], st2, dh, M, D, accumulate=True, dx16=ws["dh16"],
                              dx16_drop=d_attn)
            ops.gemm_nt(ws["dh16"], f16[p + "out"].wt, u16, M, D, D)
            ops.dilated_mix_ln_bwd(u16, obr, lsebr, lsetot, plan, t[p + "self_attn.inner_attn_ln.weight"], stin, ws["dmixed"], ws["delta"])
            ops.dilated_attn_bwd(qkv, ws["dmixed"], lsetot, ws["delta"], plan, ws["attn_ws"], ws["dqkv16"])
            ops.gemm_nt(ws["dqkv16"], f16[p + "qkv"].wt, dy16, M, D, 3 * D)
            ops.layernorm_bwd(dy16, hin, t[p + "self_attn_layer_norm.weight"], st1, dh, M, D, accumulate=True,
                              dx16=ws["dh16"] if feeds_lower else None, dx16_drop=d_lower_ffn if feeds_lower else None)
            ctx["dh16_valid"] = feeds_lower
        self.tape.record(bwd)
        return nxt

    def _extractor(self, pref: str, c: Var, pe: Param, hout: torch.Tensor) -> Var:
        cfg, ctx, tape, P, t, g = self.cfg, self._ctx, self.tape, self.store.param, self.store.tensors, self.store.grads
        B, L, N, Mp, D, E, T = ctx["B"], ctx["L"], ctx["N"], ctx["Mp"], cfg.embed_dim, cfg.adapter_dim, self.T
        ap = pref + "attn."
        pm, dev, w16, ws = ctx["patch_map"], self.device, self._train16, ctx["ws"]
        xk = torch.empty(Mp, D, dtype=H16, device=dev)
        st = torch.empty(Mp, 2, dtype=F32, device=dev)
        ops.layernorm_fwd(hout, t[ap + "norm_kq.weight"], t[ap + "norm_kq.bias"], xk, st, Mp, D, xmap=pm)
        kv = torch.empty(Mp, 2 * E, dtype=H16, device=dev)
        bkv = t[ap + "multihead_attn.in_proj_bias"][E:]
        ops.gemm_nt(xk, w16[ap + "kv"].w, kv, Mp, 2 * E, D, bias=bkv)
        t2 = tape.layernorm(c, P(ap + "norm.weight"), P(ap + "norm.bias"), add_rows=pe)
        q1 = tape.linear(t2, P(ap + "q_proj.weight"), P(ap + "q_proj.bias"))
        Wq, _, _, bq, _, _ = self._mha_in(ap + "multihead_attn.")
        q2 = tape.linear(q1, Wq, bq)
        out = Var(tape.new(B, T, E))
        lse = tape.new(B, T, 12)
        kps = -(-(-(-L // max(1, min(64, L // 256))) ) // 64) * 64
        nsplit = -(-L // kps)
        pa = tape.new(B * 12 * nsplit * T * 16)
        pml = tape.new(B * 12 * nsplit * T * 2)
        ops.extract_attn_fwd(q2.data, kv, out.data, lse, pa, pml, B, T, L, nsplit)

        def bwd_core():
            if out.grad is None:
                return
            dkv = torch.empty(Mp, 2 * E, dtype=H16, device=dev)
            ops.extract_attn_bwd(q2.data, kv, out.data, lse, out.grad, q2.g(), dkv, B, T, L)
            self._leaf(lambda: ops.gemm_tn(dkv, xk, g[ap + "multihead_attn.k_proj_weight"], Mp, 2 * E, D,
                                           colsum=g[ap + "multihead_attn.in_proj_bias"][E:]), dkv, xk)
            dxk = torch.empty(Mp, D, dtype=H16, device=dev)
            ops.gemm_nt(dkv, w16[ap + "kv"].wt, dxk, Mp, D, 2 * E)
            ops.layernorm_bwd(dxk, hout, t[ap + "norm_kq.weight"], st, ws["dh"], Mp, D, xmap=pm, dxmap=pm, accumulate=True,
                              dw=g[ap + "norm_kq.weight"], db=g[ap + "norm_kq.bias"])
        tape.record(bwd_core)
        o = tape.linear(out, P(ap + "multihead_attn.out_proj.weight"), P(ap + "multihead_attn.out_proj.bias"))
# ... 77 lines not shown
```

modaltune_amd/ops.py:

```python
from __future__ import annotations

import ctypes as C
import os
from typing import Optional, Sequence

import torch

from . import _lib
from ._lib import MtLongNetLayerBuffers, MtLongNetLayerWeights, MtVitBlockBuffers, MtVitBlockWeights
from ._lib import MT_SGEMM_MAX, MtDensePlan, MtDilatedPlan, MtDropout, MtGemmEpilogue, MtRowMap, MtSgemm, check, rowmap

F16, F32 = 0, 1
EPI_BIAS, EPI_BIAS_RESID, EPI_INJECT, EPI_POSEMB, EPI_QKV_HM = 0, 1, 2, 3, 4
ACT_NONE, ACT_RELU, ACT_GELU, ACT_ELU = 0, 1, 2, 3


def _p(t: Optional[torch.Tensor]):
    return None if t is None else t.data_ptr()


_raw_stream = getattr(torch._C, "_cuda_getCurrentRawStream", None)
_raw_device = getattr(torch._C, "_cuda_getDevice", None)


# ... 168 lines not shown

def make_dense_plan(N: int, B: int, H: int, dist=None, nslope=None) -> MtDensePlan:
    p = MtDensePlan()
    p.N, p.B, p.H = N, B, H
    p.dist = dist.data_ptr() if dist is not None else None
    p.nslope = nslope.data_ptr() if nslope is not None else None
    return p


def alibi_dist_halves(N: int) -> int:
    return int(_lib.load().mt_alibi_dist_halves(N))


def alibi_dist(cells, N, table):
    assert table.numel() >= alibi_dist_halves(N) and table.dtype == torch.float16
    check(_lib.load().mt_alibi_dist(_p(cells), N, _p(table), _s()), "alibi_dist")


def dense_attn_fwd(qkv, plan, o, lse):
    check(_lib.load().mt_dense_attn_fwd(_p(qkv), C.byref(plan), _p(o), _p(lse), _s()), "dense_attn_fwd")


def _dense_attn_bwd_phase(qkv, o, d_o, lse, plan, delta, dqkv, phases):
    check(_lib.load().mt_dense_attn_bwd(_p(qkv), _p(o), _p(d_o), _p(lse), C.byref(plan), _p(delta), _p(dqkv), phases, _s()),
          "dense_attn_bwd")


def dense_attn_bwd(qkv, o, d_o, lse, plan, delta, dqkv):
    if TIMER is None:
        return _dense_attn_bwd_phase(qkv, o, d_o, lse, plan, delta, dqkv, DENSE_BWD_ALL)
    for name, ph in (("dense_attn_delta", DENSE_BWD_DELTA), ("dense_attn_bwd_kv", DENSE_BWD_KV), ("dense_attn_bwd_q", DENSE_BWD_Q)):
        e0, e1 = torch.cuda.Event(enable_timing=True), torch.cuda.Event(enable_timing=True)
        e0.record()
        _dense_attn_bwd_phase(qkv, o, d_o, lse, plan, delta, dqkv, ph)
        e1.record()
        TIMER.setdefault(name, []).append((e0, e1))


def gelu_f16_fwd(x, y, n=None):
    check(_lib.load().mt_gelu_f16_fwd(_p(x), _p(y), n if n is not None else x.numel(), _s()), "gelu_f16_fwd")


def gelu_f16_bwd(x, dy, dx, n=None):
    check(_lib.load().mt_gelu_f16_bwd(_p(x), _p(dy), _p(dx), n if n is not None else x.numel(), _s()), "gelu_f16_bwd")


def pool_attn_workspace_floats(B, N, heads, nq) -> int:
    return int(_lib.load().mt_pool_attn_workspace_floats(B, N, heads, nq))


def pool_attn_fwd(q, kv, out, scores, lse, workspace, B, N, E, heads, nq):
    check(_lib.load().mt_pool_attn_fwd(_p(q), _p(kv), B, N, E, heads, nq, _p(out), _p(scores), _p(lse), _p(workspace), _s()), "pool_attn_fwd")


def pool_attn_bwd(q, kv, scores, lse, out, dout, dkv, B, N, E, heads, nq):
    check(_lib.load().mt_pool_attn_bwd(_p(q), _p(kv), _p(scores), _p(lse), _p(out), _p(dout), B, N, E, heads, nq, _p(dkv), _s()), "pool_attn_bwd")


def titan_grid(coords, L, patch, cells, dims, err=None):
    check(_lib.load().mt_titan_grid(_p(coords), L, float(patch), _p(cells), _p(dims), _p(err), _s()), "titan_grid")


def titan_cell_sums(feat, cells, L, Cc, first, nxt, sums, nz, ldf=None):
    check(_lib.load().mt_titan_cell_sums(_p(feat), ldf if ldf is not None else Cc, _p(cells), L, Cc, _p(first), _p(nxt), _p(sums),
                                         _p(nz), _s()), "titan_cell_sums")


def titan_token_order(cells, first, nz, L, pos, cells_tok, count):
    check(_lib.load().mt_titan_token_order(_p(cells), _p(first), _p(nz), L, _p(pos), _p(cells_tok), _p(count), _s()),
          "titan_token_order")


def titan_gather_tokens(sums, pos, L, Cc, x16):
    check(_lib.load().mt_titan_gather_tokens(_p(sums), _p(pos), L, Cc, _p(x16), _s()), "titan_gather_tokens")


def struct_of(cls, **tensors):
    st = cls()
    for k, v in tensors.items():
        setattr(st, k, v.data_ptr() if torch.is_tensor(v) else v)
    return st


def longnet_layer_fwd(w, b, plan, M, D, Fd, out, pend=None, defer=False, drop_attn=None, drop_ffn=None):
    px, pb, pd = (pend[0], pend[1], pend[2]) if pend is not None else (None, None, None)
    check(_lib.load().mt_longnet_layer_fwd(C.byref(w), C.byref(b), C.byref(plan), M, D, Fd, _p(px), _p(pb), _dr(pd), int(defer), _p(out),
                                           _dr(drop_attn), _dr(drop_ffn), _s()), "longnet_layer_fwd")


def longnet_layer_bwd(w, b, plan, M, D, Fd, dh16_valid, feeds_lower, drop_attn=None, drop_ffn=None, drop_lower_ffn=None):
    check(_lib.load().mt_longnet_layer_bwd(C.byref(w), C.byref(b), C.byref(plan), M, D, Fd, int(dh16_valid), int(feeds_lower), _dr(drop_attn),
                                           _dr(drop_ffn), _dr(drop_lower_ffn), _s()), "longnet_layer_bwd")


def vit_block_fwd(w, b, plan, M, D, Fd, out, pend=None, defer=False):
    px, pb = (pend[0], pend[1]) if pend is not None else (None, None)
    check(_lib.load().mt_vit_block_fwd(C.byref(w), C.byref(b), C.byref(plan), M, D, Fd, _p(px), _p(pb), int(defer), _p(out), _s()), "vit_block_fwd")


def vit_block_bwd(w, b, plan, M, D, Fd, dh16_valid, feeds_lower):
    check(_lib.load().mt_vit_block_bwd(C.byref(w), C.byref(b), C.byref(plan), M, D, Fd, int(dh16_valid), int(feeds_lower), _s()), "vit_block_bwd")


def gene_snn_fwd(params, offs, sizes, goff, genes, G, latent, a1, a2, z, alpha_drop=None, passes=1):
    check(_lib.load().mt_gene_snn_fwd(_p(params), _p(offs), _p(sizes), _p(goff), _p(genes), G, latent, passes, _p(a1), _p(a2), _p(z),
                                      _dr(alpha_drop), _s()), "gene_snn_fwd")


def gene_snn_bwd(params, grads, offs, sizes, goff, genes, G, latent, a1, a2, dz, alpha_drop=None, passes=1):
    check(_lib.load().mt_gene_snn_bwd(_p(params), _p(grads), _p(offs), _p(sizes), _p(goff), _p(genes), G, latent, passes, _p(a1),
                                      _p(a2), _p(dz), _dr(alpha_drop), _s()), "gene_snn_bwd")


def inject_attn_fwd(q, k, v, a, M, rows_per_pass, T, lse=None):
    check(_lib.load().mt_inject_attn_fwd(_p(q), M, rows_per_pass, _p(k), _p(v), T, _p(a), _p(lse), _s()), "inject_attn_fwd")


def inject_attn_bwd(q, a, lse, da, k, v, dq, dk, dv, M, rows_per_pass, T):
    check(_lib.load().mt_inject_attn_bwd(_p(q), _p(a), _p(lse), _p(da), M, rows_per_pass, _p(k), _p(v), T, _p(dq), _p(dk),
                                         _p(dv), _s()), "inject_attn_bwd")


def extract_attn_fwd(q, kv, out, lse, part_acc, part_ml, B, T, L, nsplit):
    check(_lib.load().mt_extract_attn_fwd(_p(q), _p(kv), B, T, L, _p(out), _p(lse), _p(part_acc), _p(part_ml), nsplit,
                                          _s()), "extract_attn_fwd")


def extract_attn_bwd(q, kv, out, lse, dout, dq, dkv, B, T, L):
    check(_lib.load().mt_extract_attn_bwd(_p(q), _p(kv), _p(out), _p(lse), _p(dout), B, T, L, _p(dq), _p(dkv), _s()),
          "extract_attn_bwd")


def token_mha_fwd(q, k, v, out, probs, B, T, E, heads):
    check(_lib.load().mt_token_mha_fwd(_p(q), _p(k), _p(v), B, T, E, heads, _p(out), _p(probs), _s()), "token_mha_fwd")


def token_mha_bwd(q, k, v, probs, dout, dq, dk, dv, B, T, E, heads):
    check(_lib.load().mt_token_mha_bwd(_p(q), _p(k), _p(v), _p(probs), _p(dout), B, T, E, heads, _p(dq), _p(dk), _p(dv),
                                       _s()), "token_mha_bwd")


def cast_f32_to_f16(x, y, n=None, drop=None, D=0):
    check(_lib.load().mt_cast_f32_to_f16(_p(x), _p(y), n if n is not None else x.numel(), _dr(drop), D, _s()), "cast")


def rng_advance(rng):
    check(_lib.load().mt_rng_advance(_p(rng), _s()), "rng_advance")


def dropout_f32(x, y, M, D, drop, *, ldx=None, xmap=None):
    check(_lib.load().mt_dropout_f32(_p(x), ldx if ldx is not None else D, _rm(xmap), _p(y), M, D, _dr(drop), _s()), "dropout")


def droppath_rows(x, M, D, drop):
    check(_lib.load().mt_droppath_rows_f32(_p(x), M, D, _dr(drop), _s()), "droppath_rows")


def cast_f16_to_f32(x, y, n=None):
    check(_lib.load().mt_cast_f16_to_f32(_p(x), _p(y), n if n is not None else x.numel(), _s()), "cast")


def pack_weight(src, dst, R, C, transpose=False):
    check(_lib.load().mt_pack_weight_f16(_p(src), R, C, _p(dst), int(transpose), _s()), "pack_weight")


def pack_weights(items, n_items):
    check(_lib.load().mt_pack_weights_f16(_p(items), n_items, _s()), "pack_weights")


def act_fwd(x, y, act, n=None):
    check(_lib.load().mt_act_fwd(_p(x), _p(y), n if n is not None else x.numel(), act, _s()), "act_fwd")


def act_bwd(x, dy, dx, act, n=None):
    check(_lib.load().mt_act_bwd(_p(x), _p(dy), _p(dx), n if n is not None else x.numel(), act, _s()), "act_bwd")
# ... 161 lines not shown
```

Baseline: 24.78 slides/s.

## Skip attention-branch compute for task passes dropped by DropPath

When DropPath zeroes a layer's attention branch for a whole task pass, the QKV GEMM, dilated attention forward/backward, mix-LN and LN backward now skip that pass's rows. The skip is decided on device from the same Philox path mask. The persistent GEMM remaps its tile indices so dead row tiles are never scheduled. This saves real work only on steps where a pass is dropped, and it adds mask checks to every kernel plus new cross-module plumbing and ABI changes.

```diff
diff --git a/include/modaltune_hip.h b/include/modaltune_hip.h
--- a/include/modaltune_hip.h
+++ b/include/modaltune_hip.h
@@ -114,6 +114,7 @@
   int nseg[MT_MAX_BRANCHES];
   int n[MT_MAX_BRANCHES];
   int qlimit[MT_MAX_BRANCHES];
+  MtDropout skip;
 } MtDilatedPlan;
 
 int mt_dilated_attn_fwd(const mt_half* qkv, const MtDilatedPlan* plan, mt_half* o_br, float* lse_br,
@@ -168,10 +169,10 @@
 } MtLongNetLayerBuffers;
 int mt_longnet_layer_fwd(const MtLongNetLayerWeights* w, const MtLongNetLayerBuffers* b, const MtDilatedPlan* plan, int M, int D, int F,
                          const float* pend_x, const mt_half* pend_branch, const MtDropout* pend_drop, int defer, float* out,
-                         const MtDropout* drop_attn, const MtDropout* drop_ffn, mt_stream_t stream);
+                         const MtDropout* drop_attn, const MtDropout* drop_ffn, int skip_dropped, mt_stream_t stream);
 int mt_longnet_layer_bwd(const MtLongNetLayerWeights* w, const MtLongNetLayerBuffers* b, const MtDilatedPlan* plan, int M, int D, int F,
                          int dh16_valid, int feeds_lower, const MtDropout* drop_attn, const MtDropout* drop_ffn,
-                         const MtDropout* drop_lower_ffn, mt_stream_t stream);
+                         const MtDropout* drop_lower_ffn, int skip_dropped, mt_stream_t stream);
 typedef struct {
   const float *n1_w, *n1_b, *n2_w, *n2_b; float n1_eps, n2_eps;
   const float *b_qkv, *b_proj, *b_fc1, *b_fc2;
diff --git a/modaltune_amd/_lib.py b/modaltune_amd/_lib.py
--- a/modaltune_amd/_lib.py
+++ b/modaltune_amd/_lib.py
@@ -38,7 +38,8 @@
 
 class MtDilatedPlan(C.Structure):
     _fields_ = [("nbranch", I), ("N", I), ("B", I), ("seg", I * MT_MAX_BRANCHES), ("ratio", I * MT_MAX_BRANCHES),
-                ("nseg", I * MT_MAX_BRANCHES), ("n", I * MT_MAX_BRANCHES), ("qlimit", I * MT_MAX_BRANCHES)]
+                ("nseg", I * MT_MAX_BRANCHES), ("n", I * MT_MAX_BRANCHES), ("qlimit", I * MT_MAX_BRANCHES),
+                ("skip", MtDropout)]
 
 
 class MtDensePlan(C.Structure):
@@ -121,8 +122,8 @@
     "mt_axpy_dev": [P, P, P, P, L, P],
     "mt_coords_to_grid": [P, I, F, I, P, P, P, P],
     "mt_mfma_probe": [P, I, I, P],
-    "mt_longnet_layer_fwd": [P, P, PL, I, I, I, P, P, DR, I, P, DR, DR, P],
-    "mt_longnet_layer_bwd": [P, P, PL, I, I, I, I, I, DR, DR, DR, P],
+    "mt_longnet_layer_fwd": [P, P, PL, I, I, I, P, P, DR, I, P, DR, DR, I, P],
+    "mt_longnet_layer_bwd": [P, P, PL, I, I, I, I, I, DR, DR, DR, I, P],
     "mt_vit_block_fwd": [P, P, DP, I, I, I, P, P, I, P, P],
     "mt_vit_block_bwd": [P, P, DP, I, I, I, I, I, P],
     "mt_alibi_dist": [P, I, P, P],
diff --git a/modaltune_amd/csrc/attn.hip b/modaltune_amd/csrc/attn.hip
--- a/modaltune_amd/csrc/attn.hip
+++ b/modaltune_amd/csrc/attn.hip
@@ -14,7 +14,7 @@
   const long M = (long)p.B * p.N;
   const int nv = __builtin_amdgcn_readfirstlane(sq.nvalid());
   const int nvq = min(nv, p.qlimit[w.br]);
-  if (w.qt * 128 >= nvq) return;
+  if (w.qt * 128 >= nvq || !p.alive(w.b)) return;
 
   {
     const int buf = tid >> 7, row = (tid >> 1) & 63, which = 6 + (tid & 1);
@@ -222,8 +222,10 @@
 #pragma unroll
   for (int e = 0; e < MIX_CPL; ++e) { w[e] = ln_w[c0 + e]; bb[e] = ln_b[c0 + e]; }
   for (long m2 = ((long)blockIdx.x * 4 + wave) * 2; m2 < M; m2 += (long)gridDim.x * 8) {
-    const bool live = m2 + sub < M;
-    const long m = live ? m2 + sub : M - 1;
+    const bool alive0 = p.alive((int)(m2 / p.N)), alive1 = m2 + 1 < M && p.alive((int)((m2 + 1) / p.N));
+    if (!alive0 && !alive1) continue;
+    const bool live = m2 + sub < M && (sub ? alive1 : alive0);
+    const long m = m2 + sub < M ? m2 + sub : M - 1;
     const int pos = (int)(m % p.N);
     bool cov[NB];
     float lse[NB];
@@ -288,8 +290,10 @@
 #pragma unroll
   for (int e = 0; e < MIX_CPL; ++e) w[e] = ln_w[c0 + e];
   for (long m2 = ((long)blockIdx.x * 4 + wave) * 2; m2 < M; m2 += (long)gridDim.x * 8) {
-    const bool live = m2 + sub < M;
-    const long m = live ? m2 + sub : M - 1;
+    const bool alive0 = p.alive((int)(m2 / p.N)), alive1 = m2 + 1 < M && p.alive((int)((m2 + 1) / p.N));
+    if (!alive0 && !alive1) continue;
+    const bool live = m2 + sub < M && (sub ? alive1 : alive0);
+    const long m = m2 + sub < M ? m2 + sub : M - 1;
     const int pos = (int)(m % p.N);
     const float tot = lse_tot[m * H + h];
     const float mean = stats[2 * m], rstd = stats[2 * m + 1];
diff --git a/modaltune_amd/csrc/attn_bwd_kv.hip b/modaltune_amd/csrc/attn_bwd_kv.hip
--- a/modaltune_amd/csrc/attn_bwd_kv.hip
+++ b/modaltune_amd/csrc/attn_bwd_kv.hip
@@ -17,7 +17,7 @@
   const long M = (long)p.B * p.N;
   const h16x8 zero8 = {0, 0, 0, 0, 0, 0, 0, 0};
   const int nv = __builtin_amdgcn_readfirstlane(sq.nvalid());
-  if (w.qt * 128 >= nv) return;
+  if (w.qt * 128 >= nv || !p.alive(w.b)) return;
 
   {
     const int img = tid >> 6, row = tid & 63;
diff --git a/modaltune_amd/csrc/attn_bwd_q.hip b/modaltune_amd/csrc/attn_bwd_q.hip
--- a/modaltune_amd/csrc/attn_bwd_q.hip
+++ b/modaltune_amd/csrc/attn_bwd_q.hip
@@ -16,7 +16,7 @@
   const h16x8 zero8 = {0, 0, 0, 0, 0, 0, 0, 0};
   const int nv = __builtin_amdgcn_readfirstlane(sq.nvalid());
   const int nvq = min(nv, p.qlimit[w.br]);
-  if (w.qt * 128 >= nvq) return;
+  if (w.qt * 128 >= nvq || !p.alive(w.b)) return;
 
   {
     const int buf = tid >> 7, row = (tid >> 1) & 63, which = 6 + (tid & 1);
diff --git a/modaltune_amd/csrc/attn_combine.hip b/modaltune_amd/csrc/attn_combine.hip
--- a/modaltune_amd/csrc/attn_combine.hip
+++ b/modaltune_amd/csrc/attn_combine.hip
@@ -7,6 +7,7 @@
   const int t = threadIdx.x;
   const int col = t * 12, which = col / DM, h = (col % DM) / HD, d0 = col % HD;
   for (long m = blockIdx.x; m < M; m += gridDim.x) {
+    if (!p.alive((int)(m / p.N))) continue;
     const int pos = (int)(m % p.N);
     float acc[12];
 #pragma unroll
diff --git a/modaltune_amd/csrc/attn_common.h b/modaltune_amd/csrc/attn_common.h
--- a/modaltune_amd/csrc/attn_common.h
+++ b/modaltune_amd/csrc/attn_common.h
@@ -23,6 +23,8 @@
   long ws_off[MT_MAX_BRANCHES + 1];
   float inv_seg[MT_MAX_BRANCHES];
   int qlimit[MT_MAX_BRANCHES];
+  DropArgs skip;
+  MT_DEVINL bool alive(int pass) const { return skip.rng == nullptr || path_alive(skip, pass); }
 };
 
 Plan make_plan(const MtDilatedPlan* p, int qtile) {
@@ -35,6 +37,7 @@
     d.inv_seg[i] = 1.0f / (float)p->seg[i];
     d.qlimit[i] = p->qlimit[i] > 0 ? p->qlimit[i] : p->n[i];
   }
+  d.skip = make_skip(p->skip.rows_per_pass == p->N ? &p->skip : nullptr);
   for (int i = 0; i < d.nbranch; ++i)
     for (int j = i + 1; j < d.nbranch; ++j)
       if (d.n[d.order[j]] > d.n[d.order[i]]) { int t = d.order[i]; d.order[i] = d.order[j]; d.order[j] = t; }
diff --git a/modaltune_amd/csrc/common.h b/modaltune_amd/csrc/common.h
--- a/modaltune_amd/csrc/common.h
+++ b/modaltune_amd/csrc/common.h
@@ -106,6 +106,13 @@
   philox4x32_7((uint32_t)pass, 0x9E3779B9u, d.path_site, d.rng[2], d.rng[0], d.rng[1], r);
   return r[0] >= drop_threshold(d.path_p) ? 1.f / (1.f - d.path_p) : 0.f;
 }
+MT_DEVINL bool path_alive(const DropArgs& d, int pass) { return drop_path_factor(d, pass) != 0.f; }
+static inline DropArgs make_skip(const MtDropout* d) {
+  DropArgs a = make_drop(d);
+  if (!(a.path_p > 0.f)) a = make_drop(nullptr);
+  a.p = 0.f; a.site = 0;
+  return a;
+}
 MT_DEVINL f32x4 drop_elem4(const DropArgs& d, uint64_t idx4, float pf) {
   f32x4 s = {pf, pf, pf, pf};
   if (d.p > 0.f) {
diff --git a/modaltune_amd/csrc/gemm.hip b/modaltune_amd/csrc/gemm.hip
--- a/modaltune_amd/csrc/gemm.hip
+++ b/modaltune_amd/csrc/gemm.hip
@@ -2,8 +2,10 @@
 #include <string.h>
 
 #include "common.h"
-
-int mt_gemm_ps_launch(const void* A, long lda, const void* W, int M, int N, int K, int epilogue, const float* bias, void* C, long ldc, hipStream_t s);
+#include "launchers.h"
+
+int mt_gemm_ps_launch(const void* A, long lda, const void* W, int M, int N, int K, int epilogue, const float* bias, void* C, long ldc, hipStream_t s,
+                      const MtDropout* skip);
 
 namespace {
 
@@ -789,6 +791,12 @@
 extern "C" int mt_gemm_nt_f16(const mt_half* A, long lda, const MtRowMap* amap, const mt_half* W, int M, int N, int K,
                               int epilogue, const MtGemmEpilogue* epi, void* C, long ldc, const MtRowMap* cmap,
                               int out_dtype, mt_stream_t stream) {
+  return mt_gemm_nt_f16_skip(A, lda, amap, W, M, N, K, epilogue, epi, C, ldc, cmap, out_dtype, nullptr, stream);
+}
+
+int mt_gemm_nt_f16_skip(const mt_half* A, long lda, const MtRowMap* amap, const mt_half* W, int M, int N, int K, int epilogue,
+                        const MtGemmEpilogue* epi, void* C, long ldc, const MtRowMap* cmap, int out_dtype, const MtDropout* skip,
+                        mt_stream_t stream) {
   if (!A || !W || !C || M <= 0 || N <= 0 || K <= 0) return MT_ERR_BAD_ARG;
   if (K % BK != 0 || lda % 8 != 0 || (N % 64) != 0 || (ldc % 4) != 0) return MT_ERR_BAD_ARG;
   if (((uintptr_t)A & 15) || ((uintptr_t)W & 15) || ((uintptr_t)C & 7)) return MT_ERR_BAD_ARG;
@@ -811,7 +819,7 @@
   const char* ps_env = getenv("MT_GEMM_PS");
   if (!(ps_env && ps_env[0] == '0') && !f32 && (epilogue == MT_EPI_BIAS || epilogue == MT_EPI_QKV_HM) && a.amap.seg_rows <= 0 &&
       a.cmap.seg_rows <= 0 && (ldc % 8) == 0 && !((uintptr_t)C & 15) && (epilogue != MT_EPI_QKV_HM || a.bias) && !a.drop.active()) {
-    const int rc = mt_gemm_ps_launch(A, lda, W, M, N, K, epilogue, a.bias, C, ldc, s);
+    const int rc = mt_gemm_ps_launch(A, lda, W, M, N, K, epilogue, a.bias, C, ldc, s, skip);
     if (rc != MT_ERR_UNSUPPORTED) return rc;
   }
   switch (epilogue) {
diff --git a/modaltune_amd/csrc/gemm_ps.hip b/modaltune_amd/csrc/gemm_ps.hip
--- a/modaltune_amd/csrc/gemm_ps.hip
+++ b/modaltune_amd/csrc/gemm_ps.hip
@@ -24,7 +24,45 @@
   int M, N, K;
   int nbm, nbn;
   int gc;
+  DropArgs skip;
 };
+constexpr int PS_MAX_PASSES = 4;
+
+struct DeadTiles {
+  int lo0, len0, lo1, len1;
+  MT_DEVINL int row_tile(int live) const {
+    if (live >= lo0) live += len0;
+    if (live >= lo1) live += len1;
+    return live;
+  }
+};
+MT_DEVINL DeadTiles dead_tiles(const GemmPsArgs& g, int& ndead) {
+  DeadTiles d{1 << 30, 0, 1 << 30, 0};
+  ndead = 0;
+  if (!g.skip.rng) return d;
+  const int R = g.skip.rows_per_pass, np = min((g.M + R - 1) / R, PS_MAX_PASSES);
+  unsigned dead = 0;
+  for (int b = 0; b < np; ++b)
+    if (!path_alive(g.skip, b)) dead |= 1u << b;
+  int nrun = 0;
+  for (int b = 0; b < np;) {
+    if (!((dead >> b) & 1u)) { ++b; continue; }
+    int e = b;
+    while (e + 1 < np && ((dead >> (e + 1)) & 1u)) ++e;
+    const int r0 = b * R, r1 = min((e + 1) * R, g.M);
+    const int t0 = (r0 + PS_BM - 1) / PS_BM, t1 = r1 == g.M ? g.nbm : r1 / PS_BM;
+    if (t1 > t0) {
+      if (nrun == 0) { d.lo0 = t0; d.len0 = t1 - t0; } else { d.lo1 = t0; d.len1 = t1 - t0; }
+      ndead += t1 - t0;
+      ++nrun;
+    }
+    b = e + 1;
+  }
+  d.lo0 = __builtin_amdgcn_readfirstlane(d.lo0); d.len0 = __builtin_amdgcn_readfirstlane(d.len0);
+  d.lo1 = __builtin_amdgcn_readfirstlane(d.lo1); d.len1 = __builtin_amdgcn_readfirstlane(d.len1);
+  ndead = __builtin_amdgcn_readfirstlane(ndead);
+  return d;
+}
 
 #ifdef PS_STAMP
 __device__ unsigned long long* ps_stamp_buf;
@@ -74,6 +112,9 @@
   const int wr = wave >> 1, wc = wave & 1;
   const int fr = lane & 15, fq = lane >> 4;
 
+  int ndead;
+  const DeadTiles dt = dead_tiles(g, ndead);
+  g.nbm -= ndead;
   const int ntiles = g.nbm * g.nbn;
   const int xcd = blockIdx.x & 7, slot_id = blockIdx.x >> 3, nslot = gridDim.x >> 3;
   const int tq = ntiles / 8, trm = ntiles % 8;
@@ -94,6 +135,7 @@
   auto dma_tile_setup = [&](int t) {
     const int idx = t_begin + slot_id + min(t, my_tiles - 1) * nslot;
     int mt, nt; tile_of(g, idx, mt, nt);
+    mt = dt.row_tile(mt);
 #pragma unroll
     for (int p = 0; p < 3; ++p) voffA[p] = (unsigned)min(mt * PS_BM + wave * 48 + p * 16 + prow, g.M - 1) * lda2 + lchunk * 16;
     soffW = (unsigned)(nt * PS_BN + wave * 64) * K2;
@@ -267,6 +309,7 @@
     {
       const int idx = t_begin + slot_id + t * nslot;
       int mt, nt; tile_of(g, idx, mt, nt);
+      mt = dt.row_tile(mt);
       const int m = mt * PS_BM + wr * 96 + fq, n = nt * PS_BN + wc * 128 + fr * 8;
       held_rows_left = g.M - m;
       held_off = EPI == MT_EPI_QKV_HM ? (unsigned)(((n / 48) * g.M + m) * 48 + n % 48) * 2u
@@ -298,16 +341,17 @@
 
 }
 
-int mt_gemm_ps_launch(const void* A, long lda, const void* W, int M, int N, int K, int epilogue, const float* bias, void* C, long ldc, hipStream_t s);
+int mt_gemm_ps_launch(const void* A, long lda, const void* W, int M, int N, int K, int epilogue, const float* bias, void* C, long ldc, hipStream_t s,
+                      const MtDropout* skip);
 #ifdef PS_STAMP
 extern "C" int mt_gemm_ps_set_stamps(void* buf) { return hipMemcpyToSymbol(HIP_SYMBOL(ps_stamp_buf), &buf, sizeof(buf)) == hipSuccess ? 0 : -1; }
 extern "C" int mt_gemm_ps_stamp_launch(const void* A, long lda, const void* W, int M, int N, int K, const float* bias, void* C, long ldc) {
-  return mt_gemm_ps_launch(A, lda, W, M, N, K, MT_EPI_BIAS, bias, C, ldc, nullptr);
+  return mt_gemm_ps_launch(A, lda, W, M, N, K, MT_EPI_BIAS, bias, C, ldc, nullptr, nullptr);
 }
 #endif
 
 int mt_gemm_ps_launch(const void* A, long lda, const void* W, int M, int N, int K, int epilogue, const float* bias, void* C, long ldc,
-                      hipStream_t s) {
+                      hipStream_t s, const MtDropout* skip) {
   if (N % 256 != 0 || K % 64 != 0 || K < 768 || M < 256) return MT_ERR_UNSUPPORTED;
   static int ncu = 0;
   if (!ncu) {
@@ -319,6 +363,8 @@
   g.A = (const h16*)A; g.lda = lda; g.W = (const h16*)W; g.bias = bias; g.C = (h16*)C; g.ldc = ldc;
   g.M = M; g.N = N; g.K = K;
   g.nbm = cdiv(M, PS_BM); g.nbn = N / PS_BN;
+  g.skip = make_skip(skip);
+  if (g.skip.rng && (g.skip.rows_per_pass < 1 || cdiv(M, g.skip.rows_per_pass) > PS_MAX_PASSES)) g.skip = make_skip(nullptr);
   {
     const char* e = getenv("MT_GEMM_GC");
     const int want = e ? atoi(e) : 0;
diff --git a/modaltune_amd/csrc/launchers.h b/modaltune_amd/csrc/launchers.h
--- /dev/null
+++ b/modaltune_amd/csrc/launchers.h
@@ -0,0 +1,12 @@
+#pragma once
+#include "../../include/modaltune_hip.h"
+
+
+int mt_layernorm_bwd_skip(const void* dy, long lddy, const MtRowMap* dymap, int dy_dtype, const void* x, long ldx, const MtRowMap* xmap,
+                          int in_dtype, int gelu_in, const float* w, const float* stats, void* dx, long lddx, const MtRowMap* dxmap,
+                          int dx_dtype, int accumulate, float* dw, float* db, mt_half* dx_f16, const MtDropout* dx_f16_drop,
+                          const MtDropout* skip, int M, int D, mt_stream_t stream);
+
+int mt_gemm_nt_f16_skip(const mt_half* A, long lda, const MtRowMap* amap, const mt_half* W, int M, int N, int K, int epilogue,
+                        const MtGemmEpilogue* epi, void* C, long ldc, const MtRowMap* cmap, int out_dtype, const MtDropout* skip,
+                        mt_stream_t stream);
diff --git a/modaltune_amd/csrc/layer.hip b/modaltune_amd/csrc/layer.hip
--- a/modaltune_amd/csrc/layer.hip
+++ b/modaltune_amd/csrc/layer.hip
@@ -1,4 +1,5 @@
 #include "common.h"
+#include "launchers.h"
 
 namespace {
 
@@ -13,22 +14,31 @@
     if (st__ != MT_OK) return st__; \
   } while (0)
 
+MtDilatedPlan branch_plan(const MtDilatedPlan* plan, const MtDropout* drop_attn, int skip_dropped) {
+  MtDilatedPlan p = *plan;
+  p.skip = MtDropout{};
+  if (skip_dropped && drop_attn && drop_attn->rng && drop_attn->path_p > 0.f && drop_attn->rows_per_pass == plan->N) p.skip = *drop_attn;
+  return p;
+}
+
 }
 
 extern "C" int mt_longnet_layer_fwd(const MtLongNetLayerWeights* w, const MtLongNetLayerBuffers* b, const MtDilatedPlan* plan, int M,
                                     int D, int F, const float* pend_x, const mt_half* pend_branch, const MtDropout* pend_drop, int defer,
-                                    float* out, const MtDropout* drop_attn, const MtDropout* drop_ffn, mt_stream_t s) {
+                                    float* out, const MtDropout* drop_attn, const MtDropout* drop_ffn, int skip_dropped, mt_stream_t s) {
   if (!w || !b || !plan || M < 1 || D != 768 || (!defer && !out)) return MT_ERR_BAD_ARG;
+  const MtDilatedPlan bp = branch_plan(plan, drop_attn, skip_dropped);
   if (!pend_x)
     MT_TRY(mt_layernorm_fwd(b->hin, D, nullptr, MT_OUT_F32, 0, w->ln1_w, w->ln1_b, nullptr, 0, b->u16, D, nullptr, MT_OUT_F16, b->st1, M, D, s));
   else
     MT_TRY(mt_add_layernorm_fwd(pend_x, pend_branch, pend_drop, w->ln1_w, w->ln1_b, b->hin, b->u16, b->st1, M, D, s));
   MtGemmEpilogue e = epi_bias(w->b_qkv);
-  MT_TRY(mt_gemm_nt_f16(b->u16, D, nullptr, w->w_qkv, M, 3 * D, D, MT_EPI_QKV_HM, &e, b->qkv, 3 * D, nullptr, MT_OUT_F16, s));
-  MT_TRY(mt_dilated_attn_fwd(b->qkv, plan, b->o_br, b->lse_br, s));
-  MT_TRY(mt_dilated_mix_ln_fwd(b->o_br, b->lse_br, plan, w->inner_ln_w, w->inner_ln_b, b->u16, b->stin, b->lse_tot, s));
+  const MtDropout* skip = bp.skip.rng ? &bp.skip : nullptr;
+  MT_TRY(mt_gemm_nt_f16_skip(b->u16, D, nullptr, w->w_qkv, M, 3 * D, D, MT_EPI_QKV_HM, &e, b->qkv, 3 * D, nullptr, MT_OUT_F16, skip, s));
+  MT_TRY(mt_dilated_attn_fwd(b->qkv, &bp, b->o_br, b->lse_br, s));
+  MT_TRY(mt_dilated_mix_ln_fwd(b->o_br, b->lse_br, &bp, w->inner_ln_w, w->inner_ln_b, b->u16, b->stin, b->lse_tot, s));
   e = epi_bias(w->b_out);
-  MT_TRY(mt_gemm_nt_f16(b->u16, D, nullptr, w->w_out, M, D, D, MT_EPI_BIAS, &e, b->br16, D, nullptr, MT_OUT_F16, s));
+  MT_TRY(mt_gemm_nt_f16_skip(b->u16, D, nullptr, w->w_out, M, D, D, MT_EPI_BIAS, &e, b->br16, D, nullptr, MT_OUT_F16, skip, s));
   MT_TRY(mt_add_layernorm_fwd(b->hin, b->br16, drop_attn, w->ln2_w, w->ln2_b, b->hmid, b->u16, b->st2, M, D, s));
   e = epi_bias(w->b_fc1);
   MT_TRY(mt_gemm_nt_f16(b->u16, D, nullptr, w->w_fc1, M, F, D, MT_EPI_BIAS, &e, b->a1, F, nullptr, MT_OUT_F16, s));
@@ -42,8 +52,9 @@
 
 extern "C" int mt_longnet_layer_bwd(const MtLongNetLayerWeights* w, const MtLongNetLayerBuffers* b, const MtDilatedPlan* plan, int M,
                                     int D, int F, int dh16_valid, int feeds_lower, const MtDropout* drop_attn, const MtDropout* drop_ffn,
-                                    const MtDropout* drop_lower_ffn, mt_stream_t s) {
+                                    const MtDropout* drop_lower_ffn, int skip_dropped, mt_stream_t s) {
   if (!w || !b || !plan || M < 1 || D != 768) return MT_ERR_BAD_ARG;
+  const MtDilatedPlan bp = branch_plan(plan, drop_attn, skip_dropped);
   const MtGemmEpilogue none{};
   const mt_half* src16 = b->dh16;
   if (!dh16_valid) {
@@ -56,12 +67,14 @@
   MT_TRY(mt_gemm_nt_f16(b->da1, F, nullptr, w->wt_fc1, M, D, F, MT_EPI_BIAS, &none, b->dy16, D, nullptr, MT_OUT_F16, s));
   MT_TRY(mt_layernorm_bwd(b->dy16, D, nullptr, MT_OUT_F16, b->hmid, D, nullptr, MT_OUT_F32, 0, w->ln2_w, b->st2, b->dh, D, nullptr, MT_OUT_F32,
                           1, nullptr, nullptr, b->dh16, drop_attn, M, D, s));
-  MT_TRY(mt_gemm_nt_f16(b->dh16, D, nullptr, w->wt_out, M, D, D, MT_EPI_BIAS, &none, b->u16, D, nullptr, MT_OUT_F16, s));
-  MT_TRY(mt_dilated_mix_ln_bwd(b->u16, b->o_br, b->lse_br, b->lse_tot, plan, w->inner_ln_w, b->stin, b->dmixed, b->delta, s));
-  MT_TRY(mt_dilated_attn_bwd(b->qkv, b->dmixed, b->lse_tot, b->delta, plan, b->attn_ws, b->dqkv16, MT_ATTN_BWD_ALL, s));
-  MT_TRY(mt_gemm_nt_f16(b->dqkv16, 3 * D, nullptr, w->wt_qkv, M, D, 3 * D, MT_EPI_BIAS, &none, b->dy16, D, nullptr, MT_OUT_F16, s));
-  return mt_layernorm_bwd(b->dy16, D, nullptr, MT_OUT_F16, b->hin, D, nullptr, MT_OUT_F32, 0, w->ln1_w, b->st1, b->dh, D, nullptr, MT_OUT_F32, 1,
-                          nullptr, nullptr, feeds_lower ? b->dh16 : nullptr, feeds_lower ? drop_lower_ffn : nullptr, M, D, s);
+  const MtDropout* skip = bp.skip.rng ? &bp.skip : nullptr;
+  MT_TRY(mt_gemm_nt_f16_skip(b->dh16, D, nullptr, w->wt_out, M, D, D, MT_EPI_BIAS, &none, b->u16, D, nullptr, MT_OUT_F16, skip, s));
+  MT_TRY(mt_dilated_mix_ln_bwd(b->u16, b->o_br, b->lse_br, b->lse_tot, &bp, w->inner_ln_w, b->stin, b->dmixed, b->delta, s));
+  MT_TRY(mt_dilated_attn_bwd(b->qkv, b->dmixed, b->lse_tot, b->delta, &bp, b->attn_ws, b->dqkv16, MT_ATTN_BWD_ALL, s));
+  MT_TRY(mt_gemm_nt_f16_skip(b->dqkv16, 3 * D, nullptr, w->wt_qkv, M, D, 3 * D, MT_EPI_BIAS, &none, b->dy16, D, nullptr, MT_OUT_F16, skip, s));
+  return mt_layernorm_bwd_skip(b->dy16, D, nullptr, MT_OUT_F16, b->hin, D, nullptr, MT_OUT_F32, 0, w->ln1_w, b->st1, b->dh, D, nullptr,
+                               MT_OUT_F32, 1, nullptr, nullptr, feeds_lower ? b->dh16 : nullptr, feeds_lower ? drop_lower_ffn : nullptr,
+                               skip, M, D, s);
 }
 
 extern "C" int mt_vit_block_fwd(const MtVitBlockWeights* w, const MtVitBlockBuffers* b, const MtDensePlan* plan, int M, int D, int F,
diff --git a/modaltune_amd/csrc/norm.hip b/modaltune_amd/csrc/norm.hip
--- a/modaltune_amd/csrc/norm.hip
+++ b/modaltune_amd/csrc/norm.hip
@@ -1,4 +1,5 @@
 #include "common.h"
+#include "launchers.h"
 
 namespace {
 
@@ -98,13 +99,14 @@
       bv[c] = Vec4<h16>::load(bp + c * 256 + lane * 4);
     }
     const float pf = dropping ? drop_path_factor(a.drop, m / a.drop.rows_per_pass) : 1.f;
+    const bool add = pf != 0.f;
     float s = 0.f;
     float* hrow = a.h + (long)m * D;
 #pragma unroll
     for (int c = 0; c < NC; ++c) {
       const int col = c * 256 + lane * 4;
-      if (dropping) bv[c] *= drop_elem4(a.drop, ((uint64_t)m * D + col) >> 2, pf);
-      v[c] += bv[c];
+      if (dropping && add) bv[c] *= drop_elem4(a.drop, ((uint64_t)m * D + col) >> 2, pf);
+      if (add) v[c] += bv[c];
       Vec4<float>::store(hrow + col, v[c]);
       s += v[c][0] + v[c][1] + v[c][2] + v[c][3];
     }
@@ -133,6 +135,7 @@
   const float* w; const float* stats;
   void* dx; long lddx; RowMap dxmap; int accumulate;
   float* dw; float* db; h16* dx16; DropArgs drop16; int M;
+  DropArgs skip;
 };
 
 template <int D, typename DyT, typename InT, typename DxT, bool GELU, bool PARAM>
@@ -147,6 +150,19 @@
 #pragma unroll
   for (int c = 0; c < NC; ++c) wr[c] = Vec4<float>::load(a.w + c * 256 + lane * 4);
   for (int m = blockIdx.x * 4 + wave; m < a.M; m += gridDim.x * 4) {
+    if (a.skip.rng && !path_alive(a.skip, m / a.skip.rows_per_pass)) {
+      if (a.dx16) {
+        const DxT* dx = reinterpret_cast<const DxT*>(a.dx) + a.dxmap.map(m) * a.lddx;
+#pragma unroll
+        for (int c = 0; c < NC; ++c) {
+          const int col = c * 256 + lane * 4;
+          f32x4 o = Vec4<DxT>::load(dx + col);
+          if (a.drop16.active()) o *= drop_scale4(a.drop16, ((uint64_t)m * D + col) >> 2, m);
+          Vec4<h16>::store(a.dx16 + (long)m * D + col, o);
+        }
+      }
+      continue;
+    }
     const DyT* dy = reinterpret_cast<const DyT*>(a.dy) + a.dymap.map(m) * a.lddy;
     const InT* x = reinterpret_cast<const InT*>(a.x) + a.xmap.map(m) * a.ldx;
     const float mean = a.stats[2 * (long)m], rstd = a.stats[2 * (long)m + 1];
@@ -656,15 +672,16 @@
   return MT_ERR_UNSUPPORTED;
 }
 
-extern "C" int mt_layernorm_bwd(const void* dy, long lddy, const MtRowMap* dymap, int dy_dtype, const void* x,
-                                long ldx, const MtRowMap* xmap, int in_dtype, int gelu_in, const float* w,
-                                const float* stats, void* dx, long lddx, const MtRowMap* dxmap, int dx_dtype,
-                                int accumulate, float* dw, float* db, mt_half* dx_f16, const MtDropout* dx_f16_drop, int M,
-                                int D, mt_stream_t stream) {
+int mt_layernorm_bwd_skip(const void* dy, long lddy, const MtRowMap* dymap, int dy_dtype, const void* x, long ldx, const MtRowMap* xmap,
+                          int in_dtype, int gelu_in, const float* w, const float* stats, void* dx, long lddx, const MtRowMap* dxmap,
+                          int dx_dtype, int accumulate, float* dw, float* db, mt_half* dx_f16, const MtDropout* dx_f16_drop,
+                          const MtDropout* skip, int M, int D, mt_stream_t stream) {
   if (!dy || !x || !w || !stats || !dx || M <= 0 || (!dw) != (!db)) return MT_ERR_BAD_ARG;
   if (dx_f16 && gelu_in) return MT_ERR_UNSUPPORTED;
+  const DropArgs sk = make_skip(skip);
+  if (sk.rng && (!accumulate || dw || gelu_in)) return MT_ERR_UNSUPPORTED;
   LnBwdArgs a{dy, lddy, make_rowmap(dymap), x, ldx, make_rowmap(xmap), w, stats, dx, lddx, make_rowmap(dxmap), accumulate, dw, db,
-              (h16*)dx_f16, make_drop(dx_f16 ? dx_f16_drop : nullptr), M};
+              (h16*)dx_f16, make_drop(dx_f16 ? dx_f16_drop : nullptr), M, sk};
   hipStream_t s = (hipStream_t)stream;
   switch (D) {
     case 256: return ln_bwd_types<256>(a, dy_dtype, in_dtype, dx_dtype, gelu_in, s);
@@ -673,6 +690,15 @@
     case 3072: return ln_bwd_types<3072>(a, dy_dtype, in_dtype, dx_dtype, gelu_in, s);
     default: return MT_ERR_UNSUPPORTED;
   }
+}
+
+extern "C" int mt_layernorm_bwd(const void* dy, long lddy, const MtRowMap* dymap, int dy_dtype, const void* x,
+                                long ldx, const MtRowMap* xmap, int in_dtype, int gelu_in, const float* w,
+                                const float* stats, void* dx, long lddx, const MtRowMap* dxmap, int dx_dtype,
+                                int accumulate, float* dw, float* db, mt_half* dx_f16, const MtDropout* dx_f16_drop, int M,
+                                int D, mt_stream_t stream) {
+  return mt_layernorm_bwd_skip(dy, lddy, dymap, dy_dtype, x, ldx, xmap, in_dtype, gelu_in, w, stats, dx, lddx, dxmap, dx_dtype, accumulate,
+                               dw, db, dx_f16, dx_f16_drop, nullptr, M, D, stream);
 }
 
 extern "C" int mt_cast_f32_to_f16(const float* x, mt_half* y, long n, const MtDropout* drop, int D, mt_stream_t stream) {
diff --git a/modaltune_amd/engine.py b/modaltune_amd/engine.py
--- a/modaltune_amd/engine.py
+++ b/modaltune_amd/engine.py
@@ -171,6 +171,7 @@
         self._fresh_pool: Dict[int, list] = {}
         dpr = np.linspace(0.0, float(cfg.drop_path_rate), cfg.depth) if cfg.depth > 1 else np.zeros(1)
         self._layer_path_p = [float(v) for v in dpr]
+        self.droppath_skip = os.environ.get("MT_DROPPATH_SKIP", "1") != "0"
         self.leaf_stream = os.environ.get("MT_LEAF_STREAM", "0") == "1"
         self._side, self._side_refs, self._side_busy = None, [], False
 
@@ -761,11 +762,12 @@
                     st2=st2, stf=stf, u16=u16, br16=br16, t16=t16, dh=ws["dh"], dy16=ws["dy16"], dh16=ws["dh16"], dt16=ws["dt16"],
                     da1=ws["da1"], dmixed=ws["dmixed"], dqkv16=ws["dqkv16"], delta=ws["delta"], attn_ws=ws["attn_ws"])
             lw = self._layer_w[l]
-            ops.longnet_layer_fwd(lw, cb, plan, M, D, Fd, out, pend=pend, defer=defer, drop_attn=d_attn, drop_ffn=d_ffn)
+            skip = self.droppath_skip
+            ops.longnet_layer_fwd(lw, cb, plan, M, D, Fd, out, pend=pend, defer=defer, drop_attn=d_attn, drop_ffn=d_ffn, skip_dropped=skip)
 
             def bwd_c():
                 ops.longnet_layer_bwd(lw, cb, plan, M, D, Fd, bool(ctx.get("dh16_valid")), feeds_lower, drop_attn=d_attn, drop_ffn=d_ffn,
-                                      drop_lower_ffn=d_lower_ffn)
+                                      drop_lower_ffn=d_lower_ffn, skip_dropped=skip)
                 ctx["dh16_valid"] = feeds_lower
             self.tape.record(bwd_c)
             return (hmid, br16, d_ffn) if defer else None
diff --git a/modaltune_amd/ops.py b/modaltune_amd/ops.py
--- a/modaltune_amd/ops.py
+++ b/modaltune_amd/ops.py
@@ -274,15 +274,15 @@
     return st
 
 
-def longnet_layer_fwd(w, b, plan, M, D, Fd, out, pend=None, defer=False, drop_attn=None, drop_ffn=None):
+def longnet_layer_fwd(w, b, plan, M, D, Fd, out, pend=None, defer=False, drop_attn=None, drop_ffn=None, skip_dropped=False):
     px, pb, pd = (pend[0], pend[1], pend[2]) if pend is not None else (None, None, None)
     check(_lib.load().mt_longnet_layer_fwd(C.byref(w), C.byref(b), C.byref(plan), M, D, Fd, _p(px), _p(pb), _dr(pd), int(defer), _p(out),
-                                           _dr(drop_attn), _dr(drop_ffn), _s()), "longnet_layer_fwd")
-
-
-def longnet_layer_bwd(w, b, plan, M, D, Fd, dh16_valid, feeds_lower, drop_attn=None, drop_ffn=None, drop_lower_ffn=None):
+                                           _dr(drop_attn), _dr(drop_ffn), int(skip_dropped), _s()), "longnet_layer_fwd")
+
+
+def longnet_layer_bwd(w, b, plan, M, D, Fd, dh16_valid, feeds_lower, drop_attn=None, drop_ffn=None, drop_lower_ffn=None, skip_dropped=False):
     check(_lib.load().mt_longnet_layer_bwd(C.byref(w), C.byref(b), C.byref(plan), M, D, Fd, int(dh16_valid), int(feeds_lower), _dr(drop_attn),
-                                           _dr(drop_ffn), _dr(drop_lower_ffn), _s()), "longnet_layer_bwd")
+                                           _dr(drop_ffn), _dr(drop_lower_ffn), int(skip_dropped), _s()), "longnet_layer_bwd")
 
 
 def vit_block_fwd(w, b, plan, M, D, Fd, out, pend=None, defer=False):
```

After: 25.10 slides/s, median of 6. 1.01x the previous value.
